# tansey/functionalmf

Measured on AMD Instinct MI355X. Metric: Gibbs sweeps/sec (full W+V update) at (512,256,64) K=5; % HBM roofline, higher is better.
Workload: dtype f64; 1 GPU; gaussian_btf c3 (512,256,64,4) nembeds=5 tf_order=2 complete data, W+V update, rng=device; burn_in_sweeps=10, step_loop=C side (btf_wv_steps: one call queues the K steps), v_sampler=spectral, likelihood_form=complete, parallelism=rows(W)/cols(V) x1

## Files before the change

### functionalmf_amd/_native.py

```python
import ctypes as C
import os
import subprocess
import sys

import numpy as np

HERE = os.path.dirname(os.path.abspath(__file__))
ROOT = os.path.dirname(HERE)
CSRC = os.path.join(HERE, "csrc")
LIB_PATH = os.environ.get("BTF_LIB_PATH") or os.path.join(HERE, "libbtf_hip.so")
SOURCES = [os.path.join(CSRC, "btf_abi.hip"), os.path.join(CSRC, "btf_criteria.hip"), os.path.join(CSRC, "btf_nmf.hip"),
           os.path.join(CSRC, "btf_gass_ep.hip"), os.path.join(CSRC, "btf_gamma_grid.hip"), os.path.join(CSRC, "btf_diag.hip"),
           os.path.join(CSRC, "btf_predict.hip"), os.path.join(CSRC, "btf_functionals.hip"), os.path.join(CSRC, "btf_fold_in.hip"),
           os.path.join(CSRC, "btf_loo.hip")]
HEADERS = sorted(os.path.join(CSRC, f) for f in os.listdir(CSRC) if f.endswith(".h")) + \
    [os.path.join(ROOT, "include", "btf.h")]

BTF_OK, BTF_EINVAL, BTF_EHIP, BTF_ENOTPD, BTF_ESTATE = 0, 1, 2, 3, 4
COMPAT = {"reference": 0, "exact": 1}
KERNEL_NAMES = ["stats", "w_accum", "w_solve", "v_accum", "v_banded", "gram", "products", "sse", "pg_draw", "nb_loglik",
                "prior_band", "gram_eig", "hyper", "ess", "criteria"]
COMM_ID_BYTES = 128
PEER_DESC_BYTES = 256
OPT_SAMPLER, OPT_NB_HISTOGRAMS, OPT_FUSE_GRAM, OPT_PG_EXACT, OPT_CURVE_COUNTS, OPT_SPLIT_ACCUM, OPT_FUSED_SWEEP, OPT_FUSED_STEP, OPT_FUSED_DATAFLOW = 0, 1, 2, 3, 4, 5, 6, 7, 8
# ... 3 lines not shown
SAMPLERS = {"banded": 0, "spectral": 1, "chain": 2, "generic": 3, "banded_nopanel": 4}

_c_dp = C.POINTER(C.c_double)
_c_ip = C.POINTER(C.c_int32)
_ctx = C.c_void_p
SIGNATURES = {
    "btf_create": (C.c_int, [C.POINTER(_ctx), C.c_int, C.c_int, C.c_int, C.c_int, C.c_int, C.c_int, C.c_void_p]),
    "btf_destroy": (None, [_ctx]),
    "btf_last_error": (C.c_char_p, [_ctx]),
    "btf_fail_index": (C.c_int, [_ctx]),
    "btf_set_shard": (C.c_int, [_ctx, C.c_int, C.c_int, C.c_int, C.c_int]),
    "btf_stream": (C.c_void_p, [_ctx]),
    "btf_dev_W": (C.c_void_p, [_ctx]),
    "btf_dev_V": (C.c_void_p, [_ctx]),
    "btf_set_data_gaussian": (C.c_int, [_ctx, _c_dp, _c_dp, C.c_int]),
    "btf_set_data_binomial": (C.c_int, [_ctx, _c_dp, _c_dp, _c_dp, _c_dp]),
    "btf_set_stale_sources": (C.c_int, [_ctx, _c_ip, _c_ip]),
    "btf_set_shard_halo": (C.c_int, [_ctx, C.c_int, C.c_int]),
    "btf_set_W": (C.c_int, [_ctx, _c_dp]),
    "btf_get_W": (C.c_int, [_ctx, _c_dp]),
    "btf_set_V": (C.c_int, [_ctx, _c_dp]),
    "btf_get_V": (C.c_int, [_ctx, _c_dp]),
    "btf_set_hyper": (C.c_int, [_ctx, _c_dp, C.c_double, C.c_double]),
    "btf_set_tau_chain": (C.c_int, [_ctx, _c_dp, _c_dp, _c_dp]),
    "btf_get_tau": (C.c_int, [_ctx, _c_dp, _c_dp, _c_dp, _c_dp]),
    "btf_resample_Tau2": (C.c_int, [_ctx, C.c_uint64, C.c_double, C.c_double, _c_dp]),
    "btf_set_nu2": (C.c_int, [_ctx, C.c_double]),
    "btf_set_omega": (C.c_int, [_ctx, _c_dp, _c_dp]),
    "btf_get_omega": (C.c_int, [_ctx, _c_dp]),
    "btf_w_accum": (C.c_int, [_ctx, C.c_int]),
    "btf_resample_W": (C.c_int, [_ctx, _c_dp, C.c_uint64, C.c_int]),
    "btf_resample_V": (C.c_int, [_ctx, _c_dp, C.c_uint64, C.c_int, C.c_double, C.c_int]),
    "btf_get_V_attempts": (C.c_int, [_ctx, _c_ip]),
    "btf_get_V_order": (C.c_int, [_ctx, _c_ip]),
    "btf_sse": (C.c_int, [_ctx, _c_dp, _c_dp]),
    "btf_sse_begin": (C.c_int, [_ctx]),
    "btf_set_data_counts": (C.c_int, [_ctx, _c_dp, C.c_int]),
    "btf_nb_loglik": (C.c_int, [_ctx, _c_dp, _c_dp, _c_ip, _c_dp]),
    "btf_nb_set_rate": (C.c_int, [_ctx, _c_dp, _c_ip]),
    "btf_nb_mh": (C.c_int, [_ctx, C.c_uint64, C.c_int, C.c_double, C.c_double, _c_ip, _c_dp]),
    "btf_nb_get_rate": (C.c_int, [_ctx, _c_dp, _c_ip]),
    "btf_dev_hyp": (C.c_void_p, [_ctx]),
    "btf_set_global_nobs": (C.c_int, [_ctx, C.c_double]),
    "btf_set_scalar_slot": (C.c_int, [_ctx, C.c_int, C.c_double]),
    "btf_device_scalars": (C.c_int, [_ctx, C.c_int]),
    "btf_set_scalars": (C.c_int, [_ctx, C.c_double, C.c_double, C.c_double, C.c_double]),
    "btf_get_scalars": (C.c_int, [_ctx, _c_dp]),
    "btf_draw_scalars": (C.c_int, [_ctx, C.c_uint64, C.c_int, C.c_double, C.c_double, C.c_double, C.c_double]),
    "btf_draw_lam2": (C.c_int, [_ctx, C.c_uint64, C.c_int]),
    "btf_sse_end": (C.c_int, [_ctx, _c_dp, _c_dp, _c_dp]),
    "btf_pg_draw": (C.c_int, [_ctx, C.c_uint64]),
    "btf_pg_batch": (C.c_int, [C.c_int, C.c_int64, _c_dp, _c_dp, C.c_uint64, _c_dp]),
    "btf_pg_batch_mode": (C.c_int, [C.c_int, C.c_int64, _c_dp, _c_dp, C.c_uint64, C.c_int, _c_dp]),
    "btf_posterior_summary": (C.c_int, [C.c_int, C.c_int, C.c_int, C.c_int, C.c_int, C.c_int, _c_dp, _c_dp, C.c_int, _c_dp,
                                        C.c_int, _c_dp, _c_dp]),
    "btf_posterior_functionals": (C.c_int, [C.c_int] * 6 + [_c_dp, _c_dp, C.c_int, _c_ip, C.c_int, _c_dp, C.c_double, C.c_double, _c_dp,
                                            C.c_int, _c_ip, C.c_int] + [_c_dp] * 7),
    "btf_collect_functionals": (C.c_int, [_ctx, C.c_int, C.c_int, _c_ip, C.c_int, _c_dp, C.c_double, C.c_double, _c_dp, C.c_int, _c_ip,
                                          C.c_int] + [_c_dp] * 7),
    "btf_fold_in_rows": (C.c_int, [C.c_int] * 7 + [_c_dp] * 7 + [C.c_uint64, C.c_int, C.c_int64, _c_dp, _c_dp, C.c_int, _c_dp, C.c_int,
                                   _c_dp, _c_dp]),
    "btf_collect_fold_in": (C.c_int, [_ctx, C.c_int, C.c_int, C.c_int] + [_c_dp] * 4 + [C.c_uint64, C.c_int, C.c_int64, _c_dp, _c_dp,
                                                                                       C.c_int, _c_dp, C.c_int, _c_dp, _c_dp]),
    "btf_diag_eval": (C.c_int, [C.c_int, C.c_int, C.c_int, C.c_int, C.c_int, C.c_int, C.c_int, C.POINTER(_c_dp), C.POINTER(_c_dp),
                                C.POINTER(_ctx), C.c_int, _c_dp]),
    "btf_collect_begin": (C.c_int, [_ctx, C.c_int]),
    "btf_collect": (C.c_int, [_ctx, C.c_int]),
    "btf_collect_schedule": (C.c_int, [_ctx, C.c_int, C.c_int, C.c_int]),
    "btf_collect_end": (C.c_int, [_ctx, C.c_int, _c_dp, _c_dp, _c_dp, _c_dp]),
    "btf_collect_summary": (C.c_int, [_ctx, C.c_int, C.c_int, _c_dp, C.c_int, _c_dp, _c_dp]),
    "btf_crit_set_data": (C.c_int, [_ctx, C.c_int, _c_dp, _c_dp, _c_dp, _c_dp]),
    "btf_crit_eval": (C.c_int, [_ctx, C.c_int, C.c_int, C.c_double, C.c_int, _c_dp, _c_dp, _c_dp, C.c_int, _c_dp, _c_dp, _c_dp]),
    "btf_crit_loo": (C.c_int, [_ctx, C.c_int, C.c_int, C.c_double, C.c_int, _c_dp, _c_dp, _c_dp, C.c_int, _c_dp, C.c_int, _c_dp, _c_dp,
                               _c_dp]),
    "btf_predict_batch": (C.c_int, [C.c_int, C.c_int, C.c_int64, _c_dp, _c_dp, C.c_uint64, _c_dp]),
    "btf_predict_eval": (C.c_int, [_ctx, C.c_int, C.c_double, C.c_int, _c_dp, _c_dp, _c_dp, C.c_int, _c_dp, _c_dp, C.c_int, C.c_int,
                                   C.c_uint64, _c_dp, C.c_int, _c_ip, C.c_int] + [_c_dp] * 11),
    "btf_nmf_create": (C.c_int, [C.POINTER(C.c_void_p), C.c_int, C.c_int, C.c_int, C.c_int, C.c_int, C.c_int, _c_dp,
                                 C.POINTER(C.c_uint8), C.c_double]),
    "btf_nmf_run": (C.c_int, [C.c_void_p, _c_dp, _c_dp, C.c_int, C.c_int, C.c_int, C.c_int, C.c_double, C.c_int, _c_ip, _c_dp,
                              _c_dp]),
    "btf_nmf_destroy": (None, [C.c_void_p]),
    "btf_nmf_pav": (C.c_int, [C.c_int, C.c_int, C.c_int, C.c_int, C.c_int, _c_dp, _c_dp]),
    "btf_sync": (C.c_int, [_ctx]),
    "btf_ess_begin": (C.c_int, [_ctx, C.c_int, _c_dp, C.c_uint64, C.c_double, C.c_int]),
    "btf_ess_eval": (C.c_int, [_ctx, C.c_int, C.c_double, C.c_int, C.c_int, _c_dp]),
    "btf_ess_run": (C.c_int, [_ctx, C.c_int, C.c_int, C.c_int, _c_dp, C.c_uint64, C.c_int, C.c_double, C.c_int]),
    "btf_ess_info": (C.c_int, [_ctx, _c_ip, _c_dp]),
    "btf_mvn_banded": (C.c_int, [C.c_int, C.c_int, C.c_int, C.c_int, _c_dp, _c_dp, _c_dp, C.c_uint64,
                                 C.c_double, C.c_int, _c_dp, _c_ip]),
    "btf_set_profiling": (C.c_int, [_ctx, C.c_int]),
    "btf_kernel_times": (C.c_int, [_ctx, _c_dp, C.POINTER(C.c_int64)]),
    "btf_set_tuning": (C.c_int, [_ctx, C.c_int, C.c_int]),
    "btf_set_option": (C.c_int, [_ctx, C.c_int, C.c_int]),
    "btf_sym_eig": (C.c_int, [C.c_int, C.c_int, C.c_int, _c_dp, _c_dp, _c_dp]),
    "btf_read_probe": (C.c_int, [C.c_int, C.c_size_t, C.c_int, _c_dp]),
    "btf_queue_Tau2": (C.c_int, [_ctx, C.c_uint64, C.c_double]),
    "btf_queue_lam2": (C.c_int, [_ctx, C.c_uint64, C.c_int]),
    "btf_gibbs_sweeps": (C.c_int, [_ctx, C.c_int, C.c_uint64, C.c_uint64, C.c_int, C.c_double, C.c_double, C.c_double,
                                   C.c_double, C.c_double, C.c_double, C.c_int]),
    "btf_wv_steps": (C.c_int, [_ctx, C.c_int, C.c_uint64, C.c_uint64, C.c_int, C.c_double, C.c_int]),
    "btf_gass_set_constraints": (C.c_int, [_ctx, _c_dp, C.c_int, _c_dp, C.c_int]),
    "btf_gass_begin": (C.c_int, [_ctx, C.c_int, C.c_int, _c_dp, _c_dp, C.c_uint64, C.c_double, C.c_int, C.c_int]),
    "btf_gass_grid": (C.c_int, [_ctx, C.c_int, _c_ip, C.POINTER(C.c_uint8), _c_dp, _c_dp]),
    "btf_gass_eval": (C.c_int, [_ctx, C.c_int, _c_dp, _c_ip, _c_dp]),
    "btf_gass_commit": (C.c_int, [_ctx, C.c_int, _c_dp, _c_ip]),
    "btf_gass_select": (C.c_int, [_ctx, C.c_int, C.c_uint64, _c_ip]),
    "btf_gass_run": (C.c_int, [_ctx, C.c_int, C.c_int, C.c_uint64, C.c_int, C.c_double, C.c_int]),
    "btf_gass_set_ep": (C.c_int, [_ctx, _c_dp, _c_dp]),
    "btf_mvn_dense": (C.c_int, [C.c_int, C.c_int, C.c_int, _c_dp, C.c_int, _c_dp, _c_dp, _c_dp, C.c_uint64, C.c_double, C.c_int,
                                _c_dp, _c_ip]),
    "btf_get_likelihood_form": (C.c_int, [_ctx, _c_ip]),
    "btf_get_draw_counters": (C.c_int, [_ctx, C.POINTER(C.c_uint64), C.POINTER(C.c_uint64)]),
    "btf_set_draw_counters": (C.c_int, [_ctx, C.c_uint64, C.c_uint64]),
    "btf_get_accum_bytes_per_cell": (C.c_int, [_ctx, _c_dp]),
    "btf_get_V_sampler": (C.c_int, [_ctx, _c_ip]),
    "btf_queue_scalars": (C.c_int, [_ctx, C.c_uint64, C.c_int, C.c_double, C.c_double, C.c_double, C.c_double, _c_ip]),
    "btf_host_selftest": (C.c_int, []),
    "btf_set_likelihood_param": (C.c_int, [_ctx, C.c_int, C.c_double]),
    "btf_set_likelihood_table": (C.c_int, [_ctx, C.c_int, _c_dp, _c_dp, _c_dp, C.c_int]),
    "btf_set_data_logsum": (C.c_int, [_ctx, _c_dp, _c_dp, C.c_int]),
    "btf_comm_fork": (C.c_int, [_ctx, C.c_void_p]),
    "btf_comm_join": (C.c_int, [_ctx, C.c_void_p]),
    "btf_comm_unique_id": (C.c_int, [C.POINTER(C.c_ubyte), C.c_int]),
    "btf_comm_block": (C.c_int, [C.c_int, C.c_int, C.c_int, _c_ip, _c_ip]),
    "btf_comm_init": (C.c_int, [_ctx, C.c_int, C.c_int, C.POINTER(C.c_ubyte), C.c_int]),
    "btf_comm_rehearse": (C.c_int, [_ctx, C.c_int, C.c_int]),
    "btf_peer_export": (C.c_int, [_ctx, C.POINTER(C.c_ubyte), C.c_int]),
    "btf_peer_init": (C.c_int, [_ctx, C.c_int, C.c_int, C.POINTER(C.c_ubyte), C.c_int]),
    "btf_comm_destroy": (C.c_int, [_ctx]),
    "btf_comm_info": (C.c_int, [_ctx, _c_ip]),
    "btf_allgather_W": (C.c_int, [_ctx]),
    "btf_allgather_V": (C.c_int, [_ctx]),
    "btf_allreduce_sse": (C.c_int, [_ctx]),
    "btf_allreduce_sum": (C.c_int, [_ctx, _c_dp, C.c_int]),
    "btf_set_gathered_W": (C.c_int, [_ctx, _c_dp]),
    "btf_set_gathered_V": (C.c_int, [_ctx, _c_dp]),
}


class BTFError(RuntimeError):
    def __init__(self, code, msg, index=-1):
        super().__init__("btf error %d: %s" % (code, msg))
        self.code = code
        self.index = index


class NotPositiveDefiniteError(BTFError, np.linalg.LinAlgError):
    """Raised where the reference raises LinAlgError (W step, factor.py:357) and
    where it would loop forever after the jitter retries (fast_mvn.py:69-72)."""


INST_SOURCE = os.path.join(CSRC, "btf_instances.hip")
INST_PARTS = 9
OBJ_DIR = os.path.join(ROOT, "build", "obj")


def build(force=False, verbose=False, jobs=None):
    deps = SOURCES + [INST_SOURCE] + HEADERS
    if not force and os.path.exists(LIB_PATH) and \
            os.path.getmtime(LIB_PATH) >= max(os.path.getmtime(p) for p in deps):
        return LIB_PATH
    from concurrent.futures import ThreadPoolExecutor
    os.makedirs(OBJ_DIR, exist_ok=True)
    tag = os.path.splitext(os.path.basename(LIB_PATH))[0]
    base = ["hipcc", "--offload-arch=gfx950", "-O3", "-std=c++17", "-fPIC", "-Wno-unused-function",
            "-mllvm", "-amdgpu-kernarg-preload-count=16",
            "-I", os.path.join(ROOT, "include")] + os.environ.get("BTF_BUILD_DEFS", "").split()
    units = [(SOURCES[0], os.path.join(OBJ_DIR, tag + "_abi.o"), []), (SOURCES[1], os.path.join(OBJ_DIR, tag + "_crit.o"), [])]
    units += [(SOURCES[2], os.path.join(OBJ_DIR, tag + "_nmf.o"), []), (SOURCES[3], os.path.join(OBJ_DIR, tag + "_gass_ep.o"), [])]
    units += [(SOURCES[4], os.path.join(OBJ_DIR, tag + "_gamma_grid.o"), []), (SOURCES[5], os.path.join(OBJ_DIR, tag + "_diag.o"), [])]
    units += [(SOURCES[6], os.path.join(OBJ_DIR, tag + "_predict.o"), []), (SOURCES[7], os.path.join(OBJ_DIR, tag + "_functionals.o"), [])]
    units += [(SOURCES[8], os.path.join(OBJ_DIR, tag + "_fold_in.o"), []), (SOURCES[9], os.path.join(OBJ_DIR, tag + "_loo.o"), [])]
    units += [(INST_SOURCE, os.path.join(OBJ_DIR, "%s_inst%d.o" % (tag, p)), ["-DBTF_INST_PART=%d" % p])
              for p in range(INST_PARTS)]

    def compile_unit(u):
        src, obj, defs = u
        cmd = base + defs + ["-c", src, "-o", obj]
        if verbose:
            print(" ".join(cmd), file=sys.stderr)
        subprocess.run(cmd, check=True, cwd=CSRC)
        return obj

    jobs = jobs or max(1, min(len(units), os.cpu_count() or 1))
    with ThreadPoolExecutor(max_workers=jobs) as pool:
        objs = list(pool.map(compile_unit, units))
    cmd = ["hipcc", "--offload-arch=gfx950", "-fPIC", "-shared", "-o", LIB_PATH] + objs + os.environ.get("BTF_LINK_FLAGS", "").split()
    if verbose:
        print(" ".join(cmd), file=sys.stderr)
    subprocess.run(cmd, check=True, cwd=CSRC)
    return LIB_PATH


_lib = None


def load():
    global _lib
    if _lib is not None:
        return _lib
    if not os.path.exists(LIB_PATH):
        raise ImportError("functionalmf_amd: %s is missing - run `python -c 'import __graft_entry__ as g; g.build()'` "
                          "(there is no CPU fallback)" % LIB_PATH)
    if "torch" not in sys.modules and os.environ.get("BTF_NO_TORCH", "0") != "1":
        try:
            import torch
        except Exception:
            pass
    lib = C.CDLL(LIB_PATH)
    for name, (res, args) in SIGNATURES.items():
        fn = getattr(lib, name)
        fn.restype = res
        fn.argtypes = args
    _lib = lib
    return lib


def check(rc, lib, handle=None, fail_index=True):
    if rc == BTF_OK:
        return
    msg = lib.btf_last_error(handle).decode()
    if rc == BTF_ENOTPD:
        raise NotPositiveDefiniteError(rc, msg, lib.btf_fail_index(handle) if fail_index else -1)
    raise BTFError(rc, msg)


def dptr(a):
    return a.ctypes.data_as(_c_dp) if a is not None else None


def as_f64(a):
    return np.ascontiguousarray(a, dtype=np.float64)


class Context:

    def __init__(self, nrows, ncols, ndepth, nembeds, tf_order, device=0, stream=None):
        self.lib = load()
        self.h = _ctx()
        check(self.lib.btf_create(C.byref(self.h), nrows, ncols, ndepth, nembeds, tf_order, device,
                                  C.c_void_p(stream) if stream else None), self.lib)
        self.dims = (nrows, ncols, ndepth, nembeds, tf_order)
        self.device = device
        self.stream_handle = self.lib.btf_stream(self.h)

    def close(self):
        if getattr(self, "h", None):
            self.lib.btf_destroy(self.h)
            self.h = None

    def __del__(self):
        try:
            self.close()
        except Exception:
            pass

    def check(self, rc):
        check(rc, self.lib, self.h)

    def call(self, name, *args):
        self.check(getattr(self.lib, name)(self.h, *args))

    def kernel_times(self):
        ms = np.zeros(len(KERNEL_NAMES))
        n = np.zeros(len(KERNEL_NAMES), dtype=np.int64)
        self.check(self.lib.btf_kernel_times(self.h, dptr(ms), n.ctypes.data_as(C.POINTER(C.c_int64))))
        return {k: (float(ms[i]), int(n[i])) for i, k in enumerate(KERNEL_NAMES)}
```

### functionalmf_amd/csrc/btf_abi.hip

```cpp
#include "../../include/btf.h"
#include "btf_kernels.h"
#include "btf_banded_fast.h"
#include "btf_banded_twist.h"
#include "btf_banded_chunk.h"
#include "btf_spectral.h"
#include "btf_gass.h"
#include "btf_gass_ep.h"
#include "btf_gamma_grid.h"
#include "btf_fused.h"
#include "btf_diag.h"
#include "btf_criteria.h"
#include "btf_loo.h"
#include "btf_predict.h"
#include "btf_functionals.h"
#include "btf_fold_in.h"
#include "btf_instances.h"
#include "btf_comm.h"
#include "btf_scratch.h"
#include <hip/hip_ext.h>
#include <unistd.h>

#include <algorithm>
#include <atomic>
#include <climits>
// ... 319 lines not shown
  }
  for (int r = 0; r < nD; ++r) {
    int lo = T, hi = -1;
    for (int t = 0; t < T; ++t)
      if (Delta[(size_t)r * T + t] != 0.0) { lo = std::min(lo, t); hi = std::max(hi, t); }
    if (hi - lo > tf + 1) return fail(c, BTF_EINVAL, "penalty row wider than the band");
  }
  int rc;
  if ((rc = dev_alloc(c, &c->st_ptr, ptr.size()))) return rc;
  if ((rc = dev_alloc(c, &c->st_row, row.size()))) return rc;
  if ((rc = dev_alloc(c, &c->st_coef, coef.size()))) return rc;
  HIPCHK(c, hipMemcpy(c->st_ptr, ptr.data(), ptr.size() * sizeof(int), hipMemcpyHostToDevice));
  HIPCHK(c, hipMemcpy(c->st_row, row.data(), row.size() * sizeof(int), hipMemcpyHostToDevice));
  HIPCHK(c, hipMemcpy(c->st_coef, coef.data(), coef.size() * sizeof(double), hipMemcpyHostToDevice));
  {
    const size_t ne = (size_t)T * D1;
    std::vector<int> drow(ne * VS_MAXE, 0);
    std::vector<double> dcoef(ne * VS_MAXE, 0.0);
    c->st_dense_ok = true;
    for (size_t e = 0; e < ne; ++e) {
      const int cnt = ptr[e + 1] - ptr[e];
      if (cnt > VS_MAXE) { c->st_dense_ok = false; break; }
      for (int u = 0; u < cnt; ++u) { drow[e * VS_MAXE + u] = row[ptr[e] + u]; dcoef[e * VS_MAXE + u] = coef[ptr[e] + u]; }
    }
    if ((rc = dev_alloc(c, &c->st_drow, drow.size()))) return rc;
    if ((rc = dev_alloc(c, &c->st_dcoef, dcoef.size()))) return rc;
    HIPCHK(c, hipMemcpy(c->st_drow, drow.data(), drow.size() * sizeof(int), hipMemcpyHostToDevice));
    HIPCHK(c, hipMemcpy(c->st_dcoef, dcoef.data(), dcoef.size() * sizeof(double), hipMemcpyHostToDevice));
  }
  return BTF_OK;
}

inline int unr3_min_rpb() {
  static const int v = [] { const char* e = std::getenv("BTF_UNR3_RPB"); return e ? std::atoi(e) : 2048; }();
  return v;
}
inline bool lean_on() {
  static const bool v = [] { const char* e = std::getenv("BTF_ACC_LEAN"); return !e || std::atoi(e) != 0; }();
  return v;
}
template <int K>
void launch_accum(btf_ctx* c, int kid, int mode, const double* X, const double* Cx, const unsigned char* C8, const double* U,
                  const int* srcmap, int Rdim, int ld, int rpb, int nch, EigSide side = EigSide{nullptr, 0, 0, nullptr},
                  EigSideCols sidec = EigSideCols{nullptr, 0, CurveLists{nullptr, nullptr, nullptr}, nullptr, 0.0, nullptr},
                  TauSide tau = TauSide{}, GramSide gram = GramSide{},
                  ChunkMap cm = ChunkMap{0, 0, INT_MAX, 0, 0, 0}, SweepSide sw = SweepSide{},
                  const FuseW* fw = nullptr, const FuseV* fv = nullptr) {
  if (cm.row_end == 0) cm.row_end = Rdim;
  {
    static const double min_mb = [] { const char* e = std::getenv("BTF_NT_MIN_MB"); return e ? std::atof(e) : 100.0; }();
    cm.nt = (double)Rdim * (double)ld * 8.0 >= min_mb * 1048576.0 ? 1 : 0;
  }
#ifdef BTF_ACC_STAMPS
  cm.stamps = c->acc_stamps;
#endif
  Prof p(c, kid);
  const int cpw = TAU_SIDE_CPW;
  cm.nside = (sw.sc.hyp ? 1 : 0) + (sw.lam.hyp ? 1 : 0) + (side.out ? 1 + eig_side_groups(sidec.ncols, acc_waves(K, mode)) : 0) +
             (tau.Tau2 ? (tau.M + cpw - 1) / cpw : 0) + (gram.gpart ? gram.nblocks : 0) + (gram.sum_src ? 1 : 0) + (fw ? fw->owners : 0);
  dim3 grid((ld / ACC_TILE) * nch + cm.nside);
  if (fw || fv) {
    const bool unr3 = rpb >= unr3_min_rpb();
    if constexpr (K == 8) {
      if (unr3 && fw) { p.launch(accum_kernel<K, 0, 16, double, double, 3, 2, FUSE_W>, grid, dim3(16 * WAVE), 0, X, Cx, U, srcmap, c->part, Rdim, ld, rpb, side, sidec, tau, gram, cm, sw, *fw); return; }
      if (unr3 && fv) { p.launch(accum_kernel<K, 0, 16, double, double, 3, 2, FUSE_V>, grid, dim3(16 * WAVE), 0, X, Cx, U, srcmap, c->part, Rdim, ld, rpb, side, sidec, tau, gram, cm, sw, *fv); return; }
    }
    if constexpr (K <= 8) {
      if (fw) p.launch(accum_kernel<K, 0, 16, double, double, 0, 2, FUSE_W>, grid, dim3(16 * WAVE), 0, X, Cx, U, srcmap, c->part, Rdim, ld, rpb, side, sidec, tau, gram, cm, sw, *fw);
      else {
        const bool df_on = c->fused_dataflow != 0;
        FuseV f2 = *fv;
        constexpr int RG = K < 4 ? 4 : (K > 6 ? 6 : K);
        f2.dataflow = (df_on && f2.a.pband && f2.pimg && !f2.cnt && !f2.hp.flag && K <= 6 &&
                       vf_df_fits(f2.a.T, K, f2.a.TF, f2.a.nD, 16, RG)) ? 1 : 0;

        if constexpr (K <= 6) {
          if (f2.dataflow) { p.launch(accum_kernel<K, 0, 16, double, double, 0, 2, FUSE_VDF>, grid, dim3(16 * WAVE), 0, X, Cx, U, srcmap, c->part, Rdim, ld, rpb, side, sidec, tau, gram, cm, sw, f2); return; }
        }
        p.launch(accum_kernel<K, 0, 16, double, double, 0, 2, FUSE_V>, grid, dim3(16 * WAVE), 0, X, Cx, U, srcmap, c->part, Rdim, ld, rpb, side, sidec, tau, gram, cm, sw, f2);
      }
    }
    return;
  }
  const signed char* A8 = (mode >= 1 && !C8 && X == c->A_wT) ? c->A8_wT : ((mode >= 1 && !C8 && X == c->A_v) ? c->A8_v : nullptr);
  if (A8) {
    if (mode == 2) p.launch(accum_kernel<K, 2, acc_waves(K, 2), double, signed char>, grid, dim3(acc_waves(K, 2) * WAVE), 0, A8, Cx, U, srcmap, c->part, Rdim, ld, rpb, side, sidec, tau, gram, cm, sw, FuseNone{});
    else p.launch(accum_kernel<K, 1, acc_waves(K, 1), double, signed char>, grid, dim3(acc_waves(K, 1) * WAVE), 0, A8, Cx, U, srcmap, c->part, Rdim, ld, rpb, side, sidec, tau, gram, cm, sw, FuseNone{});
    return;
  }
  if (mode >= 1 && C8) {
    if (mode == 2) p.launch(accum_kernel<K, 2, acc_waves(K, 2), unsigned char>, grid, dim3(acc_waves(K, 2) * WAVE), 0, X, C8, U, srcmap, c->part, Rdim, ld, rpb, side, sidec, tau, gram, cm, sw, FuseNone{});
    else p.launch(accum_kernel<K, 1, acc_waves(K, 1), unsigned char>, grid, dim3(acc_waves(K, 1) * WAVE), 0, X, C8, U, srcmap, c->part, Rdim, ld, rpb, side, sidec, tau, gram, cm, sw, FuseNone{});
  } else if (mode == 2) p.launch(accum_kernel<K, 2>, grid, dim3(acc_waves(K, 2) * WAVE), 0, X, Cx, U, srcmap, c->part, Rdim, ld, rpb, side, sidec, tau, gram, cm, sw, FuseNone{});
  else if (mode == 1) p.launch(accum_kernel<K, 1>, grid, dim3(acc_waves(K, 1) * WAVE), 0, X, Cx, U, srcmap, c->part, Rdim, ld, rpb, side, sidec, tau, gram, cm, sw, FuseNone{});
  else if (K <= 8 && acc_waves(K, 0) == 16 && rpb < unr3_min_rpb() && !tau.Tau2 && !sw.sc.hyp && !sw.lam.hyp && lean_on()) {
    if constexpr (K <= 8) p.launch(accum_kernel<K, 0, 16, double, double, 0, 2, FUSE_LEAN>, grid, dim3(16 * WAVE), 0, X, Cx, U, srcmap, c->part, Rdim, ld, rpb, side, sidec, tau, gram, cm, sw, FuseNone{});
  }
  else if (K >= 10 && ACC_WAVES != acc_waves(10, 0) && !side.out && rpb < unr3_min_rpb()) {
    if constexpr (K >= 10) p.launch(accum_kernel<K, 0, ACC_WAVES>, grid, dim3(ACC_WAVES * WAVE), 0, X, Cx, U, srcmap, c->part, Rdim, ld, rpb, side, sidec, tau, gram, cm, sw, FuseNone{});
  }
  else if (rpb >= unr3_min_rpb()) p.launch(accum_kernel<K, 0, acc_waves(K, 0), double, double, 3>, grid, dim3(acc_waves(K, 0) * WAVE), 0, X, Cx, U, srcmap, c->part, Rdim, ld, rpb, side, sidec, tau, gram, cm, sw, FuseNone{});
  else p.launch(accum_kernel<K, 0>, grid, dim3(acc_waves(K, 0) * WAVE), 0, X, Cx, U, srcmap, c->part, Rdim, ld, rpb, side, sidec, tau, gram, cm, sw, FuseNone{});
}
struct PgPasses { bool flat, series, frac; int mode; };
PgPasses pg_passes(const btf_ctx* c) {
  PgPasses p{false, false, false, c->pg_mode};
  if (c->counts && p.mode == PG_MODE_DEFAULT) p.mode = PG_MODE_SERIES_ALL;
  if (p.mode == PG_MODE_SERIES_ALL) { p.series = true; return p; }
  if (p.mode == PG_MODE_EXACT_ALL) { p.flat = c->pg_has_small || c->pg_has_big; p.frac = c->pg_has_frac; }
  else { p.flat = c->pg_has_small; p.series = c->pg_has_big || c->pg_has_frac; }
  if (!p.flat && !p.series && !p.frac) p.series = true;
  return p;
}
template <int K>
void launch_pg(btf_ctx* c, const double* B, double* out, const double* Lf, const double* Uf, int nl, int ld, int Rdim,
               unsigned long long base, unsigned long long stride_r, unsigned long long stride_l, unsigned long long seed) {
  const int gx = (nl + PG_THREADS - 1) / PG_THREADS;
  int nrb = std::max(1, std::min(Rdim, 4096 / std::max(1, gx)));
  const int rpb = (Rdim + nrb - 1) / nrb;
  nrb = (Rdim + rpb - 1) / rpb;
  const PgPasses ps = pg_passes(c);
  int fill = 1;
  if (ps.flat) {
    Prof p(c, BTF_K_PG);
    const int rpx = round_up(rpb, PGX_CPL);
    p.launch(pgx_kernel<K, PGX_CPL>, dim3(gx, (Rdim + rpx - 1) / rpx), dim3(256), pgx_rows_lds(PGX_CPL), B, out, Lf, Uf, nl, ld, Rdim,
             rpx, base, stride_r, stride_l, seed, ps.mode, fill);
    fill = 0;
  }
  if (ps.series) {
    Prof p(c, BTF_K_PG);
    p.launch(pg_kernel<K, PG_PATH_SERIES>, dim3(gx, nrb), dim3(PG_THREADS), 0, B, out, Lf, Uf, nl, ld, Rdim, rpb, base, stride_r, stride_l, seed, ps.mode, fill);
    fill = 0;
  }
  if (ps.frac) {
    Prof p(c, BTF_K_PG);
    p.launch(pg_kernel<K, PG_PATH_EXACT>, dim3(gx, nrb), dim3(PG_THREADS), 0, B, out, Lf, Uf, nl, ld, Rdim, rpb, base, stride_r, stride_l, seed, ps.mode, fill);
  }
}
template <int K>
void launch_gram(btf_ctx* c, const double* U, int Rdim) {
  Prof p(c, BTF_K_GRAM);
  c->ngp_gram = gram_blocks(Rdim);
  p.launch(gram_kernel<K>, dim3(c->ngp_gram), dim3(GRAM_THREADS), 0, U, Rdim, c->gpart);
}
template <int K>
void launch_wsolve(btf_ctx* c, const WSolveArgs& a0) {
  Prof p(c, BTF_K_W_SOLVE);
  WSolveArgs a = a0;
  const int rw = ws_rows_for(a.nl);
  a.nside = (a.lam.hyp ? 1 : 0) + (a.band.pband ? a.band.ml : 0);
  const dim3 grid((a.nl + rw - 1) / rw + a.nside);
#define WS_LAUNCH(WT, RWV) p.launch(w_solve_kernel<K, WT, RWV>, grid, dim3(WS_ROWS * ws_split_of(K, WT)), 0, a)
#define WS_PICK(WT) do { if (rw == 8) WS_LAUNCH(WT, 8); else if (rw == 16) WS_LAUNCH(WT, 16); else if (rw == 32) WS_LAUNCH(WT, 32); else WS_LAUNCH(WT, 64); } while (0)
  if (a.weighted) WS_PICK(true); else WS_PICK(false);
#undef WS_PICK
#undef WS_LAUNCH
}
template <int K>
hipError_t launch_vbanded(btf_ctx* c, const VBandArgs& a, size_t lds_bytes) {
  static std::atomic<unsigned long long> attr_set{0};
  if (!dev_flag_is_set(attr_set, c->dev)) {
    hipError_t e = hipFuncSetAttribute((const void*)v_banded_kernel<K>, hipFuncAttributeMaxDynamicSharedMemorySize, 160 * 1024);
    if (e != hipSuccess) return e;
    dev_flag_set(attr_set, c->dev);
  }
  Prof p(c, BTF_K_V_BANDED);
  p.launch(v_banded_kernel<K>, dim3(a.ml), dim3(WAVE), lds_bytes, a);
  return hipSuccess;
}
template <int NPL, bool ROW16>
hipError_t launch_vbanded_fast(btf_ctx* c, const VBandArgs& a, size_t lds_bytes) {
  static std::atomic<unsigned long long> attr_set{0};
  if (!dev_flag_is_set(attr_set, c->dev)) {
    hipError_t e = hipFuncSetAttribute((const void*)v_banded_fast_kernel<NPL, ROW16>,
                                       hipFuncAttributeMaxDynamicSharedMemorySize, 160 * 1024);
    if (e != hipSuccess) return e;
    dev_flag_set(attr_set, c->dev);
  }
  Prof p(c, BTF_K_V_BANDED);
  p.launch(v_banded_fast_kernel<NPL, ROW16>, dim3(a.ml), dim3(VB_THREADS), lds_bytes, a, c->K);
  return hipSuccess;
}
hipError_t dispatch_vbanded_fast(btf_ctx* c, const VBandArgs& a, int bw, size_t lds_bytes, bool* handled) {
  const int npairs = bw * (bw - 1) / 2;
  const int npl = std::max(1, (npairs + WAVE - 1) / WAVE);
  *handled = true;
  if (bw <= 15) {
    if (npl == 1) return launch_vbanded_fast<1, true>(c, a, lds_bytes);
    if (npl == 2) return launch_vbanded_fast<2, true>(c, a, lds_bytes);
  } else {
    switch (npl) {
      case 2: return launch_vbanded_fast<2, false>(c, a, lds_bytes);
      case 3: return launch_vbanded_fast<3, false>(c, a, lds_bytes);
      case 4: return launch_vbanded_fast<4, false>(c, a, lds_bytes);
      case 5: return launch_vbanded_fast<5, false>(c, a, lds_bytes);
      case 6: return launch_vbanded_fast<6, false>(c, a, lds_bytes);
      case 7: return launch_vbanded_fast<7, false>(c, a, lds_bytes);
      case 8: return launch_vbanded_fast<8, false>(c, a, lds_bytes);
      default: break;
    }
  }
  *handled = false;
  return hipSuccess;
}
template <int NPL>
hipError_t launch_vbanded_chunk(btf_ctx* c, const VBandArgs& a, size_t lds_bytes, int CH) {
  static std::atomic<unsigned long long> attr_set{0};
  if (!dev_flag_is_set(attr_set, c->dev)) {
    hipError_t e = hipFuncSetAttribute((const void*)v_banded_chunk_kernel<NPL>, hipFuncAttributeMaxDynamicSharedMemorySize, 160 * 1024);
    if (e != hipSuccess) return e;
    dev_flag_set(attr_set, c->dev);
  }
  Prof p(c, BTF_K_V_BANDED);
  p.launch(v_banded_chunk_kernel<NPL>, dim3(a.ml), dim3(VB_THREADS), lds_bytes, a, c->K, CH);
  return hipSuccess;
}
constexpr size_t VC_LDS_BUDGET = 158 * 1024;
inline int vc_npl(int bw) { return std::max(1, ((bw - 1) * (bw - 2) / 2 + WAVE - 1) / WAVE); }
inline int vc_chunk_for(const btf_ctx* c, bool wt) {
  const int bw = (c->TF + 1) * c->K;
  if (bw < 3 || vc_npl(bw) > 8) return 0;
  return vc_pick_chunk(c->T, c->K, c->TF, wt ? 1 : 0, VC_LDS_BUDGET);
}
hipError_t dispatch_vbanded_chunk(btf_ctx* c, const VBandArgs& a, int bw, int CH, bool wt, bool* handled) {
  const size_t lds_bytes = vc_lds_bytes(c->T, c->K, c->TF, wt ? 1 : 0, CH);
  *handled = true;
  switch (vc_npl(bw)) {
    case 1: return launch_vbanded_chunk<1>(c, a, lds_bytes, CH);
    case 2: return launch_vbanded_chunk<2>(c, a, lds_bytes, CH);
    case 3: return launch_vbanded_chunk<3>(c, a, lds_bytes, CH);
    case 4: return launch_vbanded_chunk<4>(c, a, lds_bytes, CH);
    case 5: return launch_vbanded_chunk<5>(c, a, lds_bytes, CH);
    case 6: return launch_vbanded_chunk<6>(c, a, lds_bytes, CH);
    case 7: return launch_vbanded_chunk<7>(c, a, lds_bytes, CH);
    case 8: return launch_vbanded_chunk<8>(c, a, lds_bytes, CH);
    default: break;
  }
  *handled = false;
  return hipSuccess;
}
template <int NPL, bool ROW16, int KC = 0, int TFC = 0, int TC = 0>
hipError_t launch_vbanded_twist(btf_ctx* c, const VBandArgs& a, size_t lds_bytes) {
  static std::atomic<unsigned long long> attr_set{0};
  if (!dev_flag_is_set(attr_set, c->dev)) {
    hipError_t e = hipFuncSetAttribute((const void*)v_banded_twist_kernel<NPL, ROW16, KC, TFC, TC>,
                                       hipFuncAttributeMaxDynamicSharedMemorySize, 160 * 1024);
    if (e != hipSuccess) return e;
    dev_flag_set(attr_set, c->dev);
  }
  Prof p(c, BTF_K_V_BANDED);
  p.launch(v_banded_twist_kernel<NPL, ROW16, KC, TFC, TC>, dim3(a.ml), dim3(VT_THREADS), lds_bytes, a, c->K);
  return hipSuccess;
}
void fill_table_host(int T, int K, int TF, int wmode, std::vector<int>& tab) {
  const int KK = tri(K), D1 = TF + 2, n = T * K;
  const bool weighted = wmode != 0;
  const TwLayout W = tw_layout(T, K, TF, wmode);
  auto qsrc = [&](int t, int q) { return wmode == 2 ? -2 - (q * T + t) : W.Ql + (weighted ? t * KK : 0) + q; };
  const int R1 = W.L.R1, nl = W.nl, nr = W.nr, nL = W.nL;
  tab.clear();
  auto put = [&](int dst, int src, int dia) { tab.push_back(dst); tab.push_back(src); tab.push_back(dia); tab.push_back(0); };
  for (int i = 0; i < nL; ++i) {
    const int t = i / K, k = i - t * K;
    for (int aa = 0; aa < K - k; ++aa)
      if (i + aa < nL) put(W.L.band + i * R1 + aa, qsrc(t, lidx(k + aa, k)), aa == 0 ? W.P + t * D1 : -1);
    for (int d = 1; d < D1; ++d)
      if (t + d < T && i + d * K < nL) put(W.L.band + i * R1 + d * K, W.P + t * D1 + d, -1);
  }
  for (int m = 0; m < nr; ++m) {
    const int gc = n - 1 - m, tc = gc / K, kc = gc - tc * K;
    for (int aa = 0; aa <= kc; ++aa)
      if (gc - aa >= nl) put(W.R.band + m * R1 + aa, qsrc(tc, lidx(kc, kc - aa)), aa == 0 ? W.P + tc * D1 : -1);
    for (int d = 1; d < D1; ++d)
      if (gc - d * K >= nl) put(W.R.band + m * R1 + d * K, W.P + (tc - d) * D1 + d, -1);
  }
  while ((tab.size() / 4) % VT_THREADS) put(W.L.dummy + 1, W.P, -1);
}
inline int twist_wmode(const btf_ctx* c, bool wt) {
  if (tw_lds_bytes(c->T, c->K, c->TF, wt ? 1 : 0) <= 160 * 1024) return wt ? 1 : 0;
  if (wt && tw_lds_bytes(c->T, c->K, c->TF, 2) <= 160 * 1024) return 2;
  return -1;
}
int make_fill_table(btf_ctx* c, bool weighted) {
  const int key = twist_wmode(c, weighted);
  if (c->fill_tab && c->fill_key == key) return BTF_OK;
  std::vector<int> tab;
  fill_table_host(c->T, c->K, c->TF, key, tab);
  std::vector<int> packed(tab.size() / 2);
  for (size_t e = 0; e + 3 < tab.size(); e += 4) {
    const int dst = tab[e], src = tab[e + 1], dia = tab[e + 2];
    if (dst < 0 || dst >= 0xffff || dia >= 0xffff) return fail(c, BTF_EINVAL, "band assembly program: LDS offset beyond 16 bits");
    packed[e / 2] = (int)((unsigned)dst | ((unsigned)(dia < 0 ? 0xffff : dia) << 16));
    packed[e / 2 + 1] = src;
  }
  int rc;
  if ((rc = dev_alloc(c, &c->fill_tab, packed.size()))) return rc;
  HIPCHK(c, hipMemcpy(c->fill_tab, packed.data(), packed.size() * sizeof(int), hipMemcpyHostToDevice));
  c->fill_n = (int)(tab.size() / 4);
  c->fill_key = key;
  return BTF_OK;
}
hipError_t dispatch_vbanded_twist(btf_ctx* c, const VBandArgs& a, int bw, size_t lds_bytes, bool* handled) {
  const int npairs = (bw - 1) * (bw - 2) / 2;
  const int npl = std::max(1, (npairs + WAVE - 1) / WAVE);
  *handled = true;
  if (c->TF == 2 && c->T == 64 && (c->K == 5 || c->K == 8)) {
    if (c->K == 5) return launch_vbanded_twist<tw_npl(5, 2), tw_row16(5, 2), 5, 2, 64>(c, a, lds_bytes);
    return launch_vbanded_twist<tw_npl(8, 2), tw_row16(8, 2), 8, 2, 64>(c, a, lds_bytes);
  }
// ... 136 lines not shown
  if (st[0] != 0) {
    c->fail_index = st[1];
    int zero[2] = {0, -1};
    HIPCHK(c, hipMemcpy(c->status, zero, sizeof(zero), hipMemcpyHostToDevice));
    if (st[0] == 2) return fail(c, BTF_EHIP, "a hand-off inside a fused launch timed out (btf_fused.h): its producer workgroup never published");
    if (st[0] == 3) return fail(c, BTF_EHIP, "the peer-window exchange timed out waiting for rank " + std::to_string(st[1]) + " (btf_comm.h; BTF_PEER_TIMEOUT_MS)");
    return fail(c, BTF_ENOTPD, "conditional precision not positive definite at index " + std::to_string(st[1]));
  }
  return BTF_OK;
}

int ensure_part(btf_ctx* c, size_t elems) {
  if (elems > c->part_elems) {
    int rc = dev_alloc(c, &c->part, elems);
    if (rc) return rc;
    c->part_elems = elems;
  }
  return BTF_OK;
}

int ensure_z(btf_ctx* c, size_t elems) {
  if (elems > c->z_elems) {
    int rc = dev_alloc(c, &c->zbuf, elems);
    if (rc) return rc;
    c->z_elems = elems;
  }
  return BTF_OK;
}

int pick_rpb(int Rdim, int tiles, int user, bool weighted, int slots = 0, int reserve = 0) {
  if (user > 0) return std::max(64, round_up(user, 64));
  const long long want_wgs = tiles >= 32 ? 512 : 256;
  long long rpb = ((long long)Rdim * tiles + want_wgs - 1) / want_wgs;
  rpb = std::max<long long>(rpb, weighted ? 256 : 512);
  rpb = std::min<long long>(rpb, std::max(Rdim, 1));
  rpb = std::max(128, round_up((int)rpb, 64));
  static const bool fit = [] { const char* e = std::getenv("BTF_FIT_ROUND"); return !e || std::atoi(e) != 0; }();
  if (fit && slots > 0) {
    const long long nch = (Rdim + rpb - 1) / rpb, total = nch * tiles + reserve;
    const long long rounds = (total + slots - 1) / slots;
    const long long nch1 = (slots - reserve) / std::max(tiles, 1);
    if (rounds >= 2 && rounds <= 3 && nch1 >= 1) {
      const long long r1 = round_up((int)((Rdim + nch1 - 1) / nch1), 64);
      if (r1 < rounds * rpb) rpb = r1;
    }
  }
  return (int)rpb;
}
inline int slab_rows(const btf_ctx* c) { return c->nl + (c->hrow >= 0 ? 1 : 0); }
inline int slab_cols(const btf_ctx* c) { return c->ml + (c->hcol >= 0 ? 1 : 0); }
inline int acc_slots(const btf_ctx* c, int K, int mode, bool w_launch = false) {
  const int waves = (w_launch && mode == 0 && K >= 10) ? ACC_WAVES : acc_waves(K, mode);
  return c->ncu * std::max(1, 16 / waves);
}
inline int w_side_reserve(const btf_ctx* c, bool wt) {
  const bool whole = c->nl == c->N && c->ml == c->M;
  const bool gram_side = !wt && !(whole && c->fuse_gram && c->ngp_v > 0) && !c->weighted;
  return (gram_side ? 32 : 0) + (c->tau_pending && c->dev_scalars && c->have_chain ? (c->ml + TAU_SIDE_CPW - 1) / TAU_SIDE_CPW : 0) +
         (c->sc_pending ? 1 : 0);
}
inline int v_side_reserve(const btf_ctx* c, bool wt) {
  const bool spectral = banded_choice(c) == 3;
  return (spectral ? 1 + (c->weighted && !wt ? (c->cv_ndef + 3) / 4 : 0) : 0) + (c->lam_pending ? 1 : 0);
}

struct Uploaded { const double* h = nullptr; const double* h2 = nullptr; double* d = nullptr; double* d2 = nullptr; };
int make_stats(btf_ctx* c, const double* hY, const double* hY2, int rows, int cols, int R, bool transposed,
               double** A, double** C, double** B, int ld, size_t out_rows, bool want_sums, Uploaded* keep, bool last, int sum_rows = -1) {
  const size_t cells = (size_t)rows * cols;
  double* dY = nullptr; double* dY2 = nullptr;
  int rc;
  const bool reuse = keep && keep->d && keep->h == hY && keep->h2 == hY2;
  if (reuse) { dY = keep->d; dY2 = keep->d2; }
  else {
    if ((rc = dev_alloc(c, &dY, cells * R))) return rc;
    HIPCHK(c, hipMemcpy(dY, hY, cells * R * sizeof(double), hipMemcpyHostToDevice));
    if (hY2) {
      if ((rc = dev_alloc(c, &dY2, cells))) return rc;
      HIPCHK(c, hipMemcpy(dY2, hY2, cells * sizeof(double), hipMemcpyHostToDevice));
    }
  }
  const size_t out_elems = out_rows * (size_t)ld;
  if ((rc = dev_alloc(c, A, out_elems))) return rc;
  HIPCHK(c, hipMemsetAsync(*A, 0, out_elems * sizeof(double), c->stream));
  if ((rc = dev_alloc(c, C, out_elems))) return rc;
  HIPCHK(c, hipMemsetAsync(*C, 0, out_elems * sizeof(double), c->stream));
  int* dflag = c->status + 2;
  const int blocks = (int)std::min<size_t>(4096, (cells + 255) / 256);
  if (want_sums) {
    if ((size_t)blocks * 3 > c->bsum_elems) {
      if ((rc = dev_alloc(c, &c->bsum, (size_t)blocks * 3))) return rc;
      c->bsum_elems = (size_t)blocks * 3;
    }
  }
  StatsArgs a{dY, dY2, rows, cols, R, ld, transposed ? 1 : 0, *A, *C, want_sums ? c->bsum : nullptr, dflag, sum_rows < 0 ? rows : sum_rows};
  {
    Prof p(c, BTF_K_STATS);
    p.launch(stats_kernel, dim3(blocks), dim3(256), 0, a);
  }
  HIPCHK(c, hipGetLastError());
  if (B && hY2) {
    if ((rc = dev_alloc(c, B, out_elems))) return rc;
    HIPCHK(c, hipMemcpyAsync(*B, *C, out_elems * sizeof(double), hipMemcpyDeviceToDevice, c->stream));
  }
  HIPCHK(c, hipStreamSynchronize(c->stream));
  if (want_sums) {
    std::vector<double> h((size_t)blocks * 3);
    HIPCHK(c, hipMemcpy(h.data(), c->bsum, h.size() * sizeof(double), hipMemcpyDeviceToHost));
    double ssw = 0.0, nobs = 0.0, sa2 = 0.0;
    for (int b = 0; b < blocks; ++b) { ssw += h[3 * b]; nobs += h[3 * b + 1]; sa2 += h[3 * b + 2]; }
    c->ssw = ssw;
    c->nobs = nobs;
    c->sa2 = sa2;
  }
  if (keep && !last) { keep->h = hY; keep->h2 = hY2; keep->d = dY; keep->d2 = dY2; }
  else {
    (void)hipFree(dY);
    if (dY2) (void)hipFree(dY2);
    if (keep) *keep = Uploaded{};
  }
  return BTF_OK;
}

int upload_relayout(btf_ctx* c, const double* h, int rows, int cols, double* dst, int ld, bool transposed) {
  const size_t cells = (size_t)rows * cols;
  double* d = nullptr;
  int rc;
  if ((rc = dev_alloc(c, &d, cells))) return rc;
  HIPCHK(c, hipMemcpy(d, h, cells * sizeof(double), hipMemcpyHostToDevice));
  const int blocks = (int)std::min<size_t>(4096, (cells + 255) / 256);
  hipLaunchKernelGGL(relayout_kernel, dim3(blocks), dim3(256), 0, c->stream, d, rows, cols, dst, ld, transposed ? 1 : 0, 1);
  HIPCHK(c, hipStreamSynchronize(c->stream));
  (void)hipFree(d);
  return BTF_OK;
}

}

extern "C" {

int btf_create(btf_ctx** out, int nrows, int ncols, int ndepth, int nembeds, int tf_order, int device, void* stream) {
  if (!out) return BTF_EINVAL;
  *out = nullptr;
  if (nrows < 1 || ncols < 1 || ndepth < 2 || nembeds < 1 || nembeds > MAX_K || tf_order < 0 || tf_order > 3)
    return fail(nullptr, BTF_EINVAL, "unsupported dims (need 1<=nembeds<=10, 0<=tf_order<=3, ndepth>=2)");
  if ((tf_order + 1) * nembeds > 63) return fail(nullptr, BTF_EINVAL, "half-bandwidth (tf_order+1)*nembeds must be <= 63");
  btf_ctx* c = new btf_ctx();
  c->N = nrows; c->M = ncols; c->T = ndepth; c->K = nembeds; c->TF = tf_order; c->KK = tri(nembeds);
  c->dev = device;
  c->row0 = 0; c->nl = nrows; c->col0 = 0; c->ml = ncols;
  hipError_t e = hipSetDevice(device);
  if (e != hipSuccess) { g_err = std::string("hipSetDevice: ") + hipGetErrorString(e); delete c; return BTF_EHIP; }
  { int n = 0; if (hipDeviceGetAttribute(&n, hipDeviceAttributeMultiprocessorCount, device) == hipSuccess && n > 0) c->ncu = n; }
  { const char* e = std::getenv("BTF_FUSED_STEP"); if (e) c->fused_step = std::max(0, std::min(2, std::atoi(e))); }
  { const char* e = std::getenv("BTF_LAM_IN_WSOLVE"); if (e) c->lam_in_wsolve = std::atoi(e) != 0; }
  { const char* e = std::getenv("BTF_BAND_IN_WSOLVE"); if (e) c->band_in_wsolve = std::atoi(e) != 0; }
  { const char* e = std::getenv("BTF_VF_DATAFLOW"); if (e) c->fused_dataflow = std::atoi(e) != 0 ? 1 : 0; }
  if (stream) { c->stream = (hipStream_t)stream; }
  else {
    e = hipStreamCreateWithFlags(&c->stream, hipStreamNonBlocking);
    if (e != hipSuccess) { g_err = std::string("hipStreamCreate: ") + hipGetErrorString(e); delete c; return BTF_EHIP; }
    c->own_stream = true;
  }
  int rc = BTF_OK;
  auto A = [&](int r) { if (rc == BTF_OK) rc = r; };
  A(dev_alloc(c, &c->W, (size_t)(nrows + 64) * nembeds));
  A(dev_alloc(c, &c->V, (size_t)(ncols + 64) * ndepth * nembeds));
  A(dev_alloc(c, &c->gpart, (size_t)GRAM_BLOCKS * c->KK));
  A(dev_alloc(c, &c->status, 4));
  if (rc == BTF_OK) {
    int init[4] = {0, -1, 0, 0};
    if (hipMemcpy(c->status, init, sizeof(init), hipMemcpyHostToDevice) != hipSuccess) rc = BTF_EHIP;
  }
  if (rc == BTF_OK) rc = build_stencil(c);
  A(dev_alloc(c, &c->Tau2, (size_t)ncols * c->nD));
  A(dev_alloc(c, &c->tries, (size_t)ncols));
  if (rc != BTF_OK) { std::string m = c->err; btf_destroy(c); g_err = m; return rc; }
  *out = c;
  return BTF_OK;
}

void btf_destroy(btf_ctx* c) {
  if (!c) return;
  (void)hipSetDevice(c->dev);
  if (c->stream) (void)hipStreamSynchronize(c->stream);
  void* ptrs[] = {c->A_wT, c->C_wT, c->A_v, c->C_v, c->B_wT, c->B_v, c->W, c->V, c->Tau2, c->part,
                  c->gpart, c->zbuf, c->bsum, c->gband, c->status, c->tries, c->st_ptr, c->st_row, c->st_coef,
                  c->srcmap_w, c->srcmap_v, c->pband, c->pimg, c->dbg, c->gpart_w, c->gpart_v, c->gsum_v, c->eig, c->cv_cptr, c->cv_crow, c->cv_cdef, c->cv_rptr, c->cv_rcol, c->cv_rdef, c->eig_cols, c->cv_dcols, c->A8_wT, c->A8_v, c->gs_cons, c->gs_cc, c->gs_rc, c->gs_av, c->gs_mask, c->gs_info, c->gs_thetas, c->gs_ntheta, c->gs_ll, c->gs_llp, c->gs_hh, c->gs_cur, c->gs_nacc, c->gs_u, c->st_drow, c->st_dcoef, c->essX0, c->essNu, c->ess_st, c->ess_theta, c->ess_done, c->ess_part, c->Ta, c->Tb, c->Tc, c->lsum, c->dr_ptr, c->dr_col, c->dr_val, c->sse_cols, c->vs_rec, c->vc_scratch, c->gs_cptr, c->gs_cidx, c->gs_cval,
                  c->ep_rows, c->ep_cols, c->ep_crow, c->ep_ccol, c->ep_mu, c->ep_corr, c->ep_pband, c->ep_envg, c->ep_f, c->ep_off,
                  c->gg_tab, c->gg_Lw, c->gg_Lv};
  for (void* p : ptrs) if (p) (void)hipFree(p);
  if (c->pin) (void)hipHostFree(c->pin);
  if (c->pin_lsum) (void)hipHostFree(c->pin_lsum);
  if (c->pin_hyp) (void)hipHostFree(c->pin_hyp);
  for (void* p : {(void*)c->nb_data, (void*)c->nb_S, (void*)c->nb_cnt, (void*)c->nb_R, (void*)c->nb_C, (void*)c->nb_tmp, (void*)c->nb_out, (void*)c->nb_H, (void*)c->nb_Hd, (void*)c->nb_Hs, (void*)c->nb_G, (void*)c->nb_L, (void*)c->nb_optr, (void*)c->nb_oval, (void*)c->fill_tab, (void*)c->C8_wT, (void*)c->C8_v, (void*)c->smp_W, (void*)c->smp_V, (void*)c->smp_T, (void*)c->smp_s})
    if (p) (void)hipFree(p);
  for (int sl = 0; sl < 2; ++sl)
    for (void* p : {(void*)c->crit_S1[sl], (void*)c->crit_cnt[sl], (void*)c->crit_c0[sl], (void*)c->crit_c1[sl]})
      if (p) (void)hipFree(p);
  if (c->hyp) (void)hipFree(c->hyp);
  if (c->fz_words) (void)hipFree(c->fz_words);
  if (c->fz_pub) (void)hipFree(c->fz_pub);
  for (auto& e : c->ev_pool) { (void)hipEventDestroy(e.a); (void)hipEventDestroy(e.b); }
  if (c->ev_draw) (void)hipEventDestroy(c->ev_draw);
  if (c->ev_join) (void)hipEventDestroy(c->ev_join);
  (void)btf_comm_destroy(c);

  if (c->own_stream && c->stream) (void)hipStreamDestroy(c->stream);
  delete c;
}

const char* btf_last_error(const btf_ctx* c) { return c ? c->err.c_str() : g_err.c_str(); }
int fold_fail_index();
int btf_fail_index(const btf_ctx* c) { return c ? c->fail_index : fold_fail_index(); }

int btf_set_shard(btf_ctx* c, int row0, int nrows_local, int col0, int ncols_local) {
  if (!c) return BTF_EINVAL;
  if (c->have_data) return fail(c, BTF_ESTATE, "btf_set_shard must precede btf_set_data_*");
  if (row0 < 0 || nrows_local < 0 || row0 + nrows_local > c->N || col0 < 0 || ncols_local < 0 || col0 + ncols_local > c->M)
    return fail(c, BTF_EINVAL, "shard out of range");
  c->row0 = row0; c->nl = nrows_local; c->col0 = col0; c->ml = ncols_local;
  c->hrow = c->hcol = -1;
  ++c->prior_version;
  if (c->pband) { (void)hipFree(c->pband); c->pband = nullptr; c->pband_version = 0; }
  if (c->pimg) { (void)hipFree(c->pimg); c->pimg = nullptr; c->pimg_version = 0; }
  c->v_wants_band = false;
  c->nb_bwt_written = false;
  return BTF_OK;
}
int btf_set_shard_halo(btf_ctx* c, int halo_row, int halo_col) {
  if (!c) return BTF_EINVAL;
  if (halo_row < -1 || halo_row >= c->N || halo_col < -1 || halo_col >= c->M) return fail(c, BTF_EINVAL, "halo source out of range");
  if ((halo_row >= c->row0 && halo_row < c->row0 + c->nl) || (halo_col >= c->col0 && halo_col < c->col0 + c->ml))
    return fail(c, BTF_EINVAL, "halo source inside the shard's own block");
  if (halo_row != c->hrow || halo_col != c->hcol) {
    c->have_data = false;
    c->nb_bwt_written = false;
  }
  c->hrow = halo_row; c->hcol = halo_col;
  return BTF_OK;
}
void* btf_stream(btf_ctx* c) { return c ? (void*)c->stream : nullptr; }
void* btf_dev_W(btf_ctx* c) { return c ? c->W : nullptr; }
void* btf_dev_V(btf_ctx* c) { return c ? c->V : nullptr; }

static int detect_curve_counts(btf_ctx* c) {
  c->curve = false;
  c->cv_cij.clear();
  if (!c->C8_v || c->nl != c->N || c->ml != c->M) return BTF_OK;
  const int N = c->N, M = c->M, T = c->T;
  std::vector<unsigned char> h((size_t)N * c->ldv);
  HIPCHK(c, hipMemcpy(h.data(), c->C8_v, h.size(), hipMemcpyDeviceToHost));
  std::vector<unsigned char> cij((size_t)N * M);
  for (int i = 0; i < N; ++i)
    for (int j = 0; j < M; ++j) {
      const unsigned char* p = h.data() + (size_t)i * c->ldv + (size_t)j * T;
      const unsigned char v = p[0];
      for (int t = 1; t < T; ++t) if (p[t] != v) return BTF_OK;
      cij[(size_t)i * M + j] = v;
    }
  std::vector<int> cptr(M + 1, 0), rptr(N + 1, 0);
  size_t nnz = 0;
  for (int i = 0; i < N; ++i)
    for (int j = 0; j < M; ++j) if (cij[(size_t)i * M + j] < c->R) { ++cptr[j + 1]; ++rptr[i + 1]; ++nnz; }
  if (nnz == 0 || nnz > (size_t)N * M / 4) return BTF_OK;
  for (int j = 0; j < M; ++j) cptr[j + 1] += cptr[j];
  for (int i = 0; i < N; ++i) rptr[i + 1] += rptr[i];
  std::vector<int> crow(nnz), rcol(nnz), cfill(cptr.begin(), cptr.end() - 1), rfill(rptr.begin(), rptr.end() - 1);
  std::vector<double> cdef(nnz), rdef(nnz);
  for (int i = 0; i < N; ++i)
    for (int j = 0; j < M; ++j) {
      const int v = cij[(size_t)i * M + j];
      if (v >= c->R) continue;
      const double d = (double)(c->R - v);
      crow[cfill[j]] = i; cdef[cfill[j]++] = d;
      rcol[rfill[i]] = j; rdef[rfill[i]++] = d;
    }
  int rc;
  if ((rc = dev_alloc(c, &c->cv_cptr, cptr.size()))) return rc;
  if ((rc = dev_alloc(c, &c->cv_crow, nnz))) return rc;
  if ((rc = dev_alloc(c, &c->cv_cdef, nnz))) return rc;
  if ((rc = dev_alloc(c, &c->cv_rptr, rptr.size()))) return rc;
  if ((rc = dev_alloc(c, &c->cv_rcol, nnz))) return rc;
  if ((rc = dev_alloc(c, &c->cv_rdef, nnz))) return rc;
  HIPCHK(c, hipMemcpy(c->cv_cptr, cptr.data(), cptr.size() * sizeof(int), hipMemcpyHostToDevice));
  HIPCHK(c, hipMemcpy(c->cv_crow, crow.data(), nnz * sizeof(int), hipMemcpyHostToDevice));
  HIPCHK(c, hipMemcpy(c->cv_cdef, cdef.data(), nnz * sizeof(double), hipMemcpyHostToDevice));
  HIPCHK(c, hipMemcpy(c->cv_rptr, rptr.data(), rptr.size() * sizeof(int), hipMemcpyHostToDevice));
  HIPCHK(c, hipMemcpy(c->cv_rcol, rcol.data(), nnz * sizeof(int), hipMemcpyHostToDevice));
  HIPCHK(c, hipMemcpy(c->cv_rdef, rdef.data(), nnz * sizeof(double), hipMemcpyHostToDevice));
  std::vector<int> dcols;
  for (int j = 0; j < M; ++j) if (cptr[j + 1] > cptr[j]) dcols.push_back(j);
  if ((rc = dev_alloc(c, &c->cv_dcols, dcols.size()))) return rc;
  HIPCHK(c, hipMemcpy(c->cv_dcols, dcols.data(), dcols.size() * sizeof(int), hipMemcpyHostToDevice));
  c->cv_ndef = (int)dcols.size();
  const size_t ne = (size_t)M * (c->K + c->K * c->K + 8);
  if ((rc = dev_alloc(c, &c->eig_cols, ne))) return rc;
  HIPCHK(c, hipMemset(c->eig_cols, 0, ne * sizeof(double)));
  c->cv_cij.swap(cij);
  c->curve = true;
  return BTF_OK;
}

static int finish_data(btf_ctx* c) {
  int flag = 0;
  HIPCHK(c, hipMemcpy(&flag, c->status + 2, sizeof(int), hipMemcpyDeviceToHost));
  c->weighted = c->binomial || flag != 0;
// ... 192 lines not shown
  if (!c) return BTF_EINVAL;
  HIPCHK(c, hipSetDevice(c->dev));
  if (Tau2) {
    HIPCHK(c, hipMemcpyAsync(c->Tau2, Tau2, (size_t)c->M * c->nD * sizeof(double), hipMemcpyHostToDevice, c->stream));
    HIPCHK(c, hipStreamSynchronize(c->stream));
    c->have_hyper = true;
  }
  if (Tau2 || lam2 != c->lam2) ++c->prior_version;
  c->lam2 = lam2; c->sigma2 = sigma2;
  return BTF_OK;
}
int btf_set_tau_chain(btf_ctx* c, const double* Ta, const double* Tb, const double* Tc) {
  if (!c || !Ta || !Tb || !Tc) return BTF_EINVAL;
  HIPCHK(c, hipSetDevice(c->dev));
  const size_t n = (size_t)c->M * c->nD;
  int rc;
  if (!c->Ta) {
    if ((rc = dev_alloc(c, &c->Ta, n))) return rc;
    if ((rc = dev_alloc(c, &c->Tb, n))) return rc;
    if ((rc = dev_alloc(c, &c->Tc, n))) return rc;
    if ((rc = dev_alloc(c, &c->lsum, (size_t)c->M))) return rc;
  }
  HIPCHK(c, hipMemcpyAsync(c->Ta, Ta, n * sizeof(double), hipMemcpyHostToDevice, c->stream));
  HIPCHK(c, hipMemcpyAsync(c->Tb, Tb, n * sizeof(double), hipMemcpyHostToDevice, c->stream));
  HIPCHK(c, hipMemcpyAsync(c->Tc, Tc, n * sizeof(double), hipMemcpyHostToDevice, c->stream));
  HIPCHK(c, hipStreamSynchronize(c->stream));
  c->have_chain = true;
  return BTF_OK;
}

int btf_get_tau(btf_ctx* c, double* Tau2, double* Ta, double* Tb, double* Tc) {
  if (!c || !Tau2) return BTF_EINVAL;
  HIPCHK(c, hipSetDevice(c->dev));
  const size_t n = (size_t)c->M * c->nD * sizeof(double);
  HIPCHK(c, hipMemcpyAsync(Tau2, c->Tau2, n, hipMemcpyDeviceToHost, c->stream));
  if (Ta && c->Ta) {
    HIPCHK(c, hipMemcpyAsync(Ta, c->Ta, n, hipMemcpyDeviceToHost, c->stream));
    HIPCHK(c, hipMemcpyAsync(Tb, c->Tb, n, hipMemcpyDeviceToHost, c->stream));
    HIPCHK(c, hipMemcpyAsync(Tc, c->Tc, n, hipMemcpyDeviceToHost, c->stream));
  }
  HIPCHK(c, hipStreamSynchronize(c->stream));
  return BTF_OK;
}

static TauSide tau_side_of(btf_ctx* c, uint64_t seed, double lam2, double stability) {
  TauSide t{};
  ++c->prior_version;
  t.V = c->V; t.T = c->T; t.nD = c->nD; t.M = c->M;
  t.dr_ptr = c->dr_ptr; t.dr_col = c->dr_col; t.dr_val = c->dr_val;
  t.lam2 = lam2; t.lo = stability; t.hi = 1.0 / stability;
  t.Tau2 = c->Tau2; t.Ta = c->Ta; t.Tb = c->Tb; t.Tc = c->Tc; t.lsum = c->lsum;
  t.seed = (unsigned long long)seed; t.hyp = c->dev_scalars ? c->hyp : nullptr;
  return t;
}

int btf_queue_Tau2(btf_ctx* c, uint64_t seed, double stability) {
  if (!c || !(stability > 0.0)) return fail(c, BTF_EINVAL, "bad Tau2 update arguments");
  if (!c->dev_scalars) return fail(c, BTF_ESTATE, "btf_queue_Tau2 needs device-resident scalars");
  if (!c->have_V || !c->have_hyper || !c->have_chain) return fail(c, BTF_ESTATE, "set V, Tau2 and the horseshoe+ chain first");
  c->tau_pending = true; c->tau_seed = seed; c->tau_stability = stability;
  return BTF_OK;
}

int btf_resample_Tau2(btf_ctx* c, uint64_t seed, double lam2, double stability, double* lsum_out) {
  if (!c || !(stability > 0.0)) return fail(c, BTF_EINVAL, "bad Tau2 update arguments");
  if (c->dev_scalars) lam2 = 1.0;
  if (!(lam2 > 0.0)) return fail(c, BTF_EINVAL, "bad Tau2 update arguments");
  if (!c->have_V || !c->have_hyper || !c->have_chain) return fail(c, BTF_ESTATE, "set V, Tau2 and the horseshoe+ chain first");
  HIPCHK(c, hipSetDevice(c->dev));
  c->tau_pending = false;
  {
    Prof p(c, BTF_K_HYPER);
    p.launch(tau2_kernel, dim3(c->M), dim3(256), 0, tau_side_of(c, seed, lam2, stability), c->K);
  }
  HIPCHK(c, hipGetLastError());
  if (lsum_out) {
    if (!c->pin_lsum) HIPCHK(c, hipHostMalloc((void**)&c->pin_lsum, (size_t)c->M * sizeof(double), hipHostMallocDefault));
    HIPCHK(c, hipMemcpyAsync(c->pin_lsum, c->lsum, (size_t)c->M * sizeof(double), hipMemcpyDeviceToHost, c->stream));
    HIPCHK(c, hipStreamSynchronize(c->stream));
    std::memcpy(lsum_out, c->pin_lsum, (size_t)c->M * sizeof(double));
  }
  return BTF_OK;
}

int btf_set_nu2(btf_ctx* c, double nu2) {
  if (!c || !(nu2 > 0.0)) return fail(c, BTF_EINVAL, "nu2 must be positive");
  c->nu2 = nu2;
  return BTF_OK;
}
int btf_set_omega(btf_ctx* c, const double* omega_rows, const double* omega_cols) {
  if (c) { c->w_part_valid = false; c->w_local_done = c->v_local_done = false; c->sse_cols_valid = false; }
  if (!c || !omega_rows || !omega_cols) return BTF_EINVAL;
  if (!c->have_data || !c->binomial) return fail(c, BTF_ESTATE, "btf_set_omega needs binomial data");
  HIPCHK(c, hipSetDevice(c->dev));
  int rc;
  const int MT = c->M * c->T;
  HIPCHK(c, hipMemsetAsync(c->C_wT, 0, (size_t)MT * c->ldw * sizeof(double), c->stream));
  HIPCHK(c, hipMemsetAsync(c->C_v, 0, (size_t)c->N * c->ldv * sizeof(double), c->stream));
  if ((rc = upload_relayout(c, omega_rows, slab_rows(c), MT, c->C_wT, c->ldw, true))) return rc;
  if ((rc = upload_relayout(c, omega_cols, c->N, slab_cols(c) * c->T, c->C_v, c->ldv, false))) return rc;
  hipLaunchKernelGGL(mask_kernel, dim3(1024), dim3(256), 0, c->stream, c->C_wT, c->B_wT, (size_t)MT * c->ldw);
  hipLaunchKernelGGL(mask_kernel, dim3(1024), dim3(256), 0, c->stream, c->C_v, c->B_v, (size_t)c->N * c->ldv);
  HIPCHK(c, hipStreamSynchronize(c->stream));
  return BTF_OK;
}
int btf_get_omega(btf_ctx* c, double* omega_rows) {
  if (!c || !omega_rows) return BTF_EINVAL;
  if (!c->have_data || !c->C_wT) return fail(c, BTF_ESTATE, "no weights on this context");
  HIPCHK(c, hipSetDevice(c->dev));
  const int MT = c->M * c->T;
  std::vector<double> h((size_t)MT * c->ldw);
  HIPCHK(c, hipMemcpyAsync(h.data(), c->C_wT, h.size() * sizeof(double), hipMemcpyDeviceToHost, c->stream));
  HIPCHK(c, hipStreamSynchronize(c->stream));
  for (int i = 0; i < c->nl; ++i)
    for (int jt = 0; jt < MT; ++jt) omega_rows[(size_t)i * MT + jt] = h[(size_t)jt * c->ldw + i];
  return BTF_OK;
}

namespace {
struct SplitGeom { bool ok; int lo, hi, rpb_l, nch_l, nch_r; };
SplitGeom split_geom(int lo, int hi, int Rdim, int rpb, int tiles) {
  SplitGeom g{false, lo, hi, 0, 0, 0};
  if (hi <= lo || hi - lo >= Rdim || rpb <= 0 || lo % rpb != 0) return g;
  g.ok = true;
  g.nch_r = (Rdim - (hi - lo) + rpb - 1) / rpb;
  long long rl = ((long long)(hi - lo) * tiles + 255) / 256;
  g.rpb_l = std::min(rpb, std::max(64, round_up((int)rl, 64)));
  g.nch_l = (hi - lo + g.rpb_l - 1) / g.rpb_l;
  return g;
}
bool split_applies(const btf_ctx* c) {
  return c->split_accum && !c->binomial && !c->counts && !(c->nl == c->N && c->ml == c->M) && c->nl > 0 && c->ml > 0;
}
enum { ACC_ALL = 2, ACC_LOCAL = 0 };

enum { FZ_EIG = 0, FZ_SC = 32, FZ_LAM = 64, FZ_GRAM = 96, FZ_GSUM = 128, FZ_TICKETS = 160 };
constexpr int FZ_PUB_EIG = 0, FZ_PUB_HYP = 128, FZ_PUB_GSUM = 136, FZ_PUB_GRAN = 200, FZ_PUB_DOUBLES = 224;
int ensure_fused(btf_ctx* c) {
  const int tw = c->ldw / ACC_TILE, tv = c->ldv / ACC_TILE;
  if (c->fz_words && c->fz_tiles_w == tw && c->fz_tiles_v == tv) return BTF_OK;
  int rc;
  const size_t nwords = (size_t)((FZ_TICKETS + tw + tv + 31) / 32) * 32;
  if ((rc = dev_alloc(c, &c->fz_words, nwords))) return rc;
  HIPCHK(c, hipMemsetAsync(c->fz_words, 0, nwords * sizeof(unsigned), c->stream));
  if (!c->fz_pub) {
    if ((rc = dev_alloc(c, &c->fz_pub, (size_t)FZ_PUB_DOUBLES))) return rc;
    HIPCHK(c, hipMemsetAsync(c->fz_pub, 0, (size_t)FZ_PUB_DOUBLES * sizeof(double), c->stream));
  }
  c->fz_tiles_w = tw; c->fz_tiles_v = tv;
  c->fz_gram_total = 0; c->fz_w_total = 0;
  return BTF_OK;
}
bool fuse_w_applies(const btf_ctx* c, bool wt, bool cv, int mode, int rpb) {
  if (c->fused_step < 2 || wt || cv || mode != 0 || c->nl <= 0 || c->K > 8) return false;
  if (split_applies(c)) return false;
  if (rpb >= unr3_min_rpb() && c->K != 8) return false;
  return true;
}
struct WFuseReq { const double* dz; uint64_t seed; bool done; };
int w_accum_phase(btf_ctx* c, int compat, int part = ACC_ALL, WFuseReq* wf = nullptr) {
  const int K = c->K, KK = c->KK, MT = c->M * c->T;
  const bool wt = lik_weighted(c), cv = c->weighted && !wt;
  const int mode = !wt ? 0 : (compat == BTF_COMPAT_REFERENCE && c->stale_w && c->srcmap_w ? 2 : 1);
  const int NV = wt ? K + KK : K;
  const int tiles = c->ldw / ACC_TILE;
  const int rpb = pick_rpb(MT, tiles, c->rpb_w, wt, acc_slots(c, K, mode, true), w_side_reserve(c, wt));
  const int nch = (MT + rpb - 1) / rpb;
  int rc;
  if ((rc = ensure_part(c, (size_t)round_up(nch, 32) * NV * c->ldw))) return rc;
  const SplitGeom sg = split_applies(c) ? split_geom(c->col0 * c->T, (c->col0 + c->ml) * c->T, MT, rpb, tiles) : SplitGeom{};
  if (sg.ok) { if ((rc = ensure_part(c, (size_t)(sg.nch_r + sg.nch_l) * NV * c->ldw))) return rc; }
  if (part == ACC_LOCAL) {
    c->w_local_done = false;
    if (!sg.ok || mode == 2) return BTF_OK;
    K_SWITCH(K, launch_accum<KT>(c, BTF_K_W_ACCUM, mode, c->A_wT, c->C_wT, c->C8_wT, c->V, c->srcmap_w, MT, c->ldw, sg.rpb_l, sg.nch_l,
                                 EigSide{nullptr, 0, 0, nullptr}, EigSideCols{nullptr, 0, CurveLists{nullptr, nullptr, nullptr}, nullptr, 0.0, nullptr},
                                 TauSide{}, GramSide{}, ChunkMap{sg.nch_r, sg.lo, INT_MAX, 0, sg.hi, 0}));
    HIPCHK(c, hipGetLastError());
    c->w_local_done = true; c->w_local_rpb = rpb; c->w_local_mode = mode;
    return BTF_OK;
  }
  const bool rest_only = c->w_local_done && sg.ok && c->w_local_rpb == rpb && c->w_local_mode == mode;
  c->w_local_done = false;
  const ChunkMap cm = rest_only ? ChunkMap{0, 0, sg.lo, sg.hi - sg.lo, MT, 0} : ChunkMap{0, 0, INT_MAX, 0, MT, 0};
  const int nch_launch = rest_only ? sg.nch_r : nch;
  const int nch_total = rest_only ? sg.nch_r + sg.nch_l : nch;
  const bool whole = c->nl == c->N && c->ml == c->M;
  bool use_gv = !wt && whole && c->fuse_gram && c->ngp_v > 0;
  if (cv && c->nl > 0) {
    if (c->ngp_v != c->ml) {
      if (!c->gpart_v) { if ((rc = dev_alloc(c, &c->gpart_v, (size_t)c->M * KK))) return rc; }
      Prof p(c, BTF_K_GRAM);
      K_SWITCH(K, p.launch(colgram_kernel<KT>, dim3(c->ml), dim3(WAVE), 0, (const double*)c->V, c->T, c->ml, c->gpart_v));
      c->ngp_v = c->ml;
    }
    use_gv = true;
  }
  if (c->nl > 0) {
    GramSide gram{nullptr, 0, nullptr, 0};
    if (!wt && !use_gv) {
      c->ngp_gram = std::min(gram_blocks(MT), 32);
      gram = GramSide{c->V, MT, c->gpart, c->ngp_gram, nullptr, nullptr, 0, nullptr, 0};
    }
    bool gsum = false;
    c->w_part_gsum = false;
    if (!wt && use_gv && part == ACC_ALL && c->ngp_v > 8 * std::min(32, (WS_ROWS * ws_split_of(K, false)) / KK)) {
      if (!c->gsum_v) { if ((rc = dev_alloc(c, &c->gsum_v, (size_t)tri(MAX_K)))) return rc; }
      gram.sum_src = c->gpart_v; gram.sum_n = c->ngp_v; gram.sum_out = c->gsum_v; gram.sum_threads = WS_ROWS * ws_split_of(K, false);
      gsum = true;
    }
    c->w_part_gsum = gsum;
    TauSide tau{};
    if (c->tau_pending && c->dev_scalars && c->have_chain) tau = tau_side_of(c, c->tau_seed, 1.0, c->tau_stability);
    SweepSide sw{};
    if (c->sc_pending) {
      const int h = std::min(c->K, c->N);
      const double nfree = (double)c->N * c->K - (double)h * (h - 1) / 2.0 - (double)(c->K - h) * c->N;
      sw.sc = ScalarSide{c->sse_cols, c->M, c->ssw + c->sa2, c->nobs_global >= 0.0 ? c->nobs_global : c->nobs, c->W, c->N * c->K, nfree,
                         c->sc_prior[0], c->sc_prior[1], c->sc_prior[2], c->sc_prior[3], c->sc_which, c->sc_seed, c->hyp};
      c->sc_pending = false;
    }
    FuseW fw{};
    int own_rows = 0;
    if (wf && !rest_only && fuse_w_applies(c, wt, cv, mode, rpb)) {
      const long long others = (long long)tiles * nch + (tau.Tau2 ? (tau.M + TAU_SIDE_CPW - 1) / TAU_SIDE_CPW : 0) + (gram.gpart ? gram.nblocks : 0) + (sw.sc.hyp ? 1 : 0);
      static const int min_rows = [] { const char* e = std::getenv("BTF_OWNER_ROWS"); return e ? std::atoi(e) : 32; }();
      for (int r = std::max(ws_rows_for(c->nl), min_rows); r <= ACC_TILE; r *= 2) {
        if (others + (long long)tiles * (ACC_TILE / r) <= (long long)c->ncu && w_owner_lds_doubles(K, r, nch) <= w_owner_lds_budget(K)) { own_rows = r; break; }
      }
    }
    const bool fuse = own_rows > 0;
    if (fuse) {
      if ((rc = ensure_fused(c))) return rc;
      ++c->fz_epoch;
      WSolveArgs& a = fw.a;
      a.part = c->part; a.nch = nch_total; a.ld = c->ldw; a.weighted = 0;
      a.gpart = use_gv ? c->gpart_v : c->gpart; a.ngp = use_gv ? c->ngp_v : c->ngp_gram;
      if (whole && c->fuse_gram) {
        if (!c->gpart_w) { if ((rc = dev_alloc(c, &c->gpart_w, (size_t)std::max(64, (c->N + WS_ROWS - 1) / WS_ROWS) * KK))) return rc; }
        a.gout = c->gpart_w;
      }
      a.s = c->binomial ? 1.0 : 1.0 / c->nu2;
      a.sR = a.s * c->R;
      a.inv_sigma2 = 1.0 / c->sigma2;
      a.hyp = c->dev_scalars ? c->hyp : nullptr; a.Rrep = c->R; a.hyp_noise = c->binomial ? 0 : 1;
      a.W = c->W; a.row0 = c->row0; a.nl = c->nl;
#ifdef BTF_WS_STAMPS
      a.dbg = c->dbg;
#endif
      a.z = wf->dz; a.seed = wf->seed; a.stream = 2 * c->sweep_w + 0x10000ULL;
      a.status = c->status;
      fw.cnt = c->fz_words + FZ_TICKETS;
      fw.rw = ws_rows_for(c->nl);
      if (sw.sc.hyp) {
        sw.sc.pub = c->fz_pub + FZ_PUB_HYP; sw.sc.flag = c->fz_words + FZ_SC; sw.sc.epoch = c->fz_epoch;
        fw.hp = HypPub{c->fz_pub + FZ_PUB_HYP, c->fz_words + FZ_SC, c->fz_epoch, sw.sc.which & 3};
      }
      if (gram.gpart) {
        gram.cnt = c->fz_words + FZ_GRAM;
        c->fz_gram_total += (unsigned)gram.nblocks;
        fw.gram_cnt = gram.cnt; fw.gram_expected = c->fz_gram_total;
      }
      c->fz_w_total += (unsigned)nch_total;
      fw.expected = c->fz_w_total;
      fw.rows = own_rows;
      fw.owners = tiles * (ACC_TILE / own_rows);
    }
    K_SWITCH(K, launch_accum<KT>(c, BTF_K_W_ACCUM, mode, c->A_wT, c->C_wT, c->C8_wT, c->V, c->srcmap_w, MT, c->ldw, rpb, nch_launch,
                                 EigSide{nullptr, 0, 0, nullptr}, EigSideCols{nullptr, 0, CurveLists{nullptr, nullptr, nullptr}, nullptr, 0.0, nullptr}, tau, gram, cm, sw,
                                 fuse ? &fw : nullptr));
    if (fuse) {
      wf->done = true;
      const int wrows = ws_rows_for(c->nl);
      c->ngp_w = fw.a.gout ? (c->nl + wrows - 1) / wrows : 0;
      c->ngp_v = 0;
    }
    c->tau_pending = false;
  } else if (c->tau_pending && c->dev_scalars && c->have_chain) {
    Prof p(c, BTF_K_HYPER);
    p.launch(tau2_kernel, dim3(c->M), dim3(256), 0, tau_side_of(c, c->tau_seed, 1.0, c->tau_stability), c->K);
    c->tau_pending = false;
  }
  HIPCHK(c, hipGetLastError());
  c->w_part_valid = true; c->w_part_mode = mode; c->w_part_nch = nch_total; c->w_part_rpb = rpb; c->w_part_gv = use_gv;
  c->w_part_curve = cv;
  return BTF_OK;
}
}

namespace {
int v_accum_local(btf_ctx* c, int compat);
int mark_draw(btf_ctx* c);
}

int btf_w_accum(btf_ctx* c, int compat) {
  if (!c) return BTF_EINVAL;
  if (!c->have_data || !c->have_V || !c->have_W) return fail(c, BTF_ESTATE, "set data, W and V first");
  HIPCHK(c, hipSetDevice(c->dev));
  return w_accum_phase(c, compat);
}

int btf_resample_W(btf_ctx* c, const double* z, uint64_t seed, int compat) {
  if (!c) return BTF_EINVAL;
  if (!c->have_data || !c->have_V || !c->have_W) return fail(c, BTF_ESTATE, "set data, W and V first");
  HIPCHK(c, hipSetDevice(c->dev));
  const int K = c->K, KK = c->KK;
  const bool wt = lik_weighted(c), cv = c->weighted && !wt;
  const int want_mode = !wt ? 0 : (compat == BTF_COMPAT_REFERENCE && c->stale_w && c->srcmap_w ? 2 : 1);
  int rc;
  c->v_local_done = false;
  const double* dz = nullptr;
  if (z) {
    const size_t nz = (size_t)w_z_offset(c->N, K);
    if ((rc = ensure_z(c, nz))) return rc;
    HIPCHK(c, hipMemcpyAsync(c->zbuf, z, nz * sizeof(double), hipMemcpyHostToDevice, c->stream));
    dz = c->zbuf;
  }
  WFuseReq wf{dz, seed, false};
  if (!(c->w_part_valid && c->w_part_mode == want_mode && c->w_part_curve == cv)) { if ((rc = w_accum_phase(c, compat, ACC_ALL, &wf))) return rc; }
  if (c->sc_pending) return fail(c, BTF_ESTATE, "btf_queue_scalars must be followed by the W accumulation that carries it");
  const int nch = c->w_part_nch;
  const bool use_gv = c->w_part_gv;
  c->w_part_valid = false;
  if (c->nl > 0 && !wf.done) {
    const bool whole = c->nl == c->N && c->ml == c->M;
    WSolveArgs a{};
    a.part = c->part; a.nch = nch; a.ld = c->ldw; a.weighted = wt ? 1 : 0;
    a.gsrc = (wt && want_mode == 2) ? c->srcmap_w : nullptr;
    a.gpart = use_gv ? c->gpart_v : c->gpart; a.ngp = use_gv ? c->ngp_v : c->ngp_gram;
    if (use_gv && c->w_part_gsum) { a.gpart = c->gsum_v; a.ngp = 1; }
    const int wrows = ws_rows_for(c->nl);
    const int wblocks = (c->nl + wrows - 1) / wrows;
    if (whole && c->fuse_gram) {
      if (!c->gpart_w) { if ((rc = dev_alloc(c, &c->gpart_w, (size_t)std::max(64, (c->N + WS_ROWS - 1) / WS_ROWS) * KK))) return rc; }
      a.gout = c->gpart_w;
    }
    a.s = c->binomial ? 1.0 : 1.0 / c->nu2;
    a.sR = a.s * c->R;
    a.inv_sigma2 = 1.0 / c->sigma2;
    a.hyp = c->dev_scalars ? c->hyp : nullptr; a.Rrep = c->R; a.hyp_noise = c->binomial ? 0 : 1;
    a.W = c->W; a.row0 = c->row0; a.nl = c->nl;
#ifdef BTF_WS_STAMPS
    a.dbg = c->dbg;
#endif
    a.z = dz; a.seed = seed; a.stream = 2 * c->sweep_w + 0x10000ULL;
    a.status = c->status;
    if (cv) { a.cv = CurveLists{c->cv_rptr, c->cv_rcol, c->cv_rdef}; a.cv_blocks = c->gpart_v; }
    if (c->lam_in_wsolve && c->lam_pending && c->dev_scalars && c->lsum && c->have_chain) {
      a.lam = LamSide{c->lsum, c->M, (double)c->nD * c->M * c->K + 1.0, c->lam_exact, c->lam_seed, c->hyp, nullptr, nullptr, 0u};
      c->lam_pending = false;
      ++c->prior_version;
      const int TD1 = c->T * (c->TF + 2);
      if (c->band_in_wsolve && c->v_wants_band && c->pband && (!c->band_img || c->pimg) && TD1 <= 2 * WS_ROWS * ws_split_of(K, wt) &&
          c->nD <= 2 * WS_ROWS * ws_split_of(K, wt)) {
        if ((rc = ensure_fused(c))) return rc;
        ++c->fz_epoch;
        a.lam.pub = c->fz_pub + FZ_PUB_HYP; a.lam.flag = c->fz_words + FZ_LAM; a.lam.epoch = c->fz_epoch;
        a.band = BandSide{c->Tau2, c->nD, c->st_ptr, c->st_row, c->st_coef, TD1, c->col0, c->ml, c->pband,
                          c->band_img ? c->pimg : nullptr, c->T, c->TF + 2, c->band_PB, nullptr, 0.0,
                          c->fz_pub + FZ_PUB_HYP, c->fz_words + FZ_LAM, c->fz_epoch, c->status};
        c->pband_version = c->prior_version;
        c->pimg_version = c->band_img ? c->prior_version : 0;
      }
    }
    K_SWITCH(K, launch_wsolve<KT>(c, a));
    c->ngp_w = a.gout ? wblocks : 0;
    c->ngp_v = 0;
  }
  c->sweep_w++;
  c->nb_L_valid = false;
  c->sse_cols_valid = false;
  HIPCHK(c, hipGetLastError());
  if (split_applies(c)) {
    if ((rc = mark_draw(c))) return rc;
    return v_accum_local(c, compat);
  }
  return BTF_OK;
}

static int v_banded_dispatch(btf_ctx* c, int choice, const double* dz, uint64_t seed, int nch, bool use_gw, double eps0,
                             int attempts, double* out, bool prior_only) {
  const int K = c->K, KK = c->KK, T = c->T, n = T * K;
  const bool wt = lik_weighted(c), cv = c->weighted && !wt && !prior_only;
  const bool whole = c->nl == c->N && c->ml == c->M;
  int rc;
  const int bw = (c->TF + 1) * K, R1 = bw + 1, D1 = c->TF + 2;
  size_t lds_fixed = (size_t)(3 * n + T * D1 + (wt ? T * KK : KK) + (bw * (bw + 1) / 2 + 3) / 4) * sizeof(double);
  size_t lds_band = std::max((size_t)n * R1, (size_t)(GRAM_BLOCKS + 16) * KK) * sizeof(double);
  size_t lds_bytes = lds_fixed + lds_band;
  VBandArgs a{};
  if (lds_bytes > 150 * 1024) {
    if (wt) lds_fixed -= (size_t)T * KK * sizeof(double);
    if (lds_fixed > 150 * 1024) return fail(c, BTF_EINVAL, "ndepth*nembeds too large for the on-chip vectors");
    const size_t stride = (size_t)n * R1 + (wt ? (size_t)T * KK : 0);
    if (!c->gband || c->gband_stride != stride) {
      if ((rc = dev_alloc(c, &c->gband, (size_t)c->ml * stride))) return rc;
      c->gband_stride = stride;
    }
    a.gband = c->gband; a.gband_stride = c->gband_stride;
    lds_bytes = lds_fixed;
  }
  a.part = c->part; a.nch = nch; a.ld = c->ldv; a.weighted = wt ? 1 : 0;
  a.gsrc = (wt && c->v_part_mode == 2) ? c->srcmap_v : nullptr;
  a.gpart = use_gw ? c->gpart_w : c->gpart; a.ngp = use_gw ? c->ngp_w : c->ngp_gram;
  a.s = c->binomial ? 1.0 : 1.0 / c->nu2;
  a.sR = a.s * c->R;
  a.Tau2 = c->Tau2; a.lam2 = c->lam2; a.nD = c->nD;
  a.hyp = c->dev_scalars ? c->hyp : nullptr; a.Rrep = c->R; a.hyp_noise = c->binomial ? 0 : 1;
  a.panel4 = c->sampler == BTF_SAMPLER_BANDED_NOPANEL ? 0 : 1;
  a.st_ptr = c->st_ptr; a.st_row = c->st_row; a.st_coef = c->st_coef;
  a.T = T; a.TF = c->TF; a.col0 = c->col0; a.ml = c->ml;
  a.V = c->V; a.z = dz; a.seed = seed; a.stream = 2 * c->sweep_v + 0x10001ULL;
  a.eps0 = eps0; a.attempts = attempts; a.status = c->status; a.tries = c->tries; a.dbg = c->dbg;
  if (prior_only) { a.nch = 0; a.ngp = 0; a.s = 0.0; a.sR = 0.0; a.hyp_noise = 0; }
  if (cv) { a.cv = CurveLists{c->cv_cptr, c->cv_crow, c->cv_cdef}; a.cv_W = c->W; }
  a.V = out;
  hipError_t e = hipSuccess;
  bool handled = false;
  const bool fast = choice >= 0;
  const int tw_npl = std::max(1, ((bw - 1) * (bw - 2) / 2 + WAVE - 1) / WAVE);
  const bool tw_handles = bw <= 15 ? tw_npl <= 2 : (tw_npl >= 2 && tw_npl <= 8);
  const bool own_prior = choice == 2 && tw_handles && c->st_dense_ok && c->st_drow && (c->TF + 2) * T >= c->nD;
  if (own_prior) {
    a.st_drow = c->st_drow; a.st_dcoef = c->st_dcoef; a.pband = nullptr;
    const int TD1 = T * D1;
    static const bool lazy_band = [] { const char* e = std::getenv("BTF_TWIST_PBAND"); return !e || std::atoi(e) != 0; }();
    if (!lazy_band) {  }
    else if (c->pband && c->pband_version == c->prior_version) a.pband = c->pband;
    else if (c->last_v_prior_version == c->prior_version) {
      if (!c->pband) { if ((rc = dev_alloc(c, &c->pband, (size_t)c->ml * TD1))) return rc; }
      Prof p(c, BTF_K_PRIOR);
      p.launch(prior_band_kernel, dim3((c->ml * TD1 + 255) / 256), dim3(256), 0, (const double*)c->Tau2, c->lam2, c->nD,
               (const int*)c->st_ptr, (const int*)c->st_row, (const double*)c->st_coef, TD1, c->col0, c->ml, c->pband,
               (const double*)(c->dev_scalars ? c->hyp : nullptr), 1, (double*)nullptr, 0, 0, 0);
      c->pband_version = c->prior_version;
      a.pband = c->pband;
    }
    c->last_v_prior_version = c->prior_version;
  }
  if (fast && !own_prior) {
    const int TD1 = T * D1;
    if (!c->pband) { if ((rc = dev_alloc(c, &c->pband, (size_t)c->ml * TD1))) return rc; }
    {
      Prof p(c, BTF_K_PRIOR);
      p.launch(prior_band_kernel, dim3((c->ml * TD1 + 255) / 256), dim3(256), 0, (const double*)c->Tau2, c->lam2, c->nD,
               (const int*)c->st_ptr, (const int*)c->st_row, (const double*)c->st_coef, TD1, c->col0, c->ml, c->pband,
               (const double*)(c->dev_scalars ? c->hyp : nullptr), 0, (double*)nullptr, 0, 0, 0);
    }
    c->pband_version = 0;
    a.pband = c->pband;
  }
  const bool emit_gv = !prior_only && fast && whole && c->fuse_gram && !wt &&
                       (size_t)c->ml * KK + 16 * KK <= ws_gram_stage(K, false);
  if (emit_gv) {
    if (!c->gpart_v) { if ((rc = dev_alloc(c, &c->gpart_v, (size_t)c->M * KK))) return rc; }
    a.gout = c->gpart_v;
  }
  if (!prior_only) { c->ngp_v = emit_gv ? c->ml : 0; c->ngp_w = 0; }
  if (choice == 2) {
    if ((rc = make_fill_table(c, wt))) return rc;
    a.fill = c->fill_tab; a.nfill = c->fill_n;
    a.ql_global = twist_wmode(c, wt) == 2 ? 1 : 0;
    e = dispatch_vbanded_twist(c, a, bw, tw_lds_bytes(T, K, c->TF, twist_wmode(c, wt)), &handled);
  }
  HIPCHK(c, e);
  if (fast && !handled && vb_fast_lds_bytes(T, K, c->TF, wt ? 1 : 0) <= 158 * 1024)
    e = dispatch_vbanded_fast(c, a, bw, vb_fast_lds_bytes(T, K, c->TF, wt ? 1 : 0), &handled);
  HIPCHK(c, e);
  if (fast && !handled) {
    const int CH = vc_chunk_for(c, wt);
    if (CH > 0) {
      const size_t stride = vc_scratch_stride(T, K, c->TF);
      if (!c->vc_scratch || c->vc_scratch_elems < (size_t)c->ml * stride) {
        if ((rc = dev_alloc(c, &c->vc_scratch, (size_t)c->ml * stride))) return rc;
        c->vc_scratch_elems = (size_t)c->ml * stride;
      }
      VBandArgs ac = a;
      ac.gband = c->vc_scratch; ac.gband_stride = stride;
      e = dispatch_vbanded_chunk(c, ac, bw, CH, wt, &handled);
      HIPCHK(c, e);
    }
  }
  if (!handled) { a.gout = nullptr; if (!prior_only) c->ngp_v = 0; }
  if (!handled) { K_SWITCH(K, e = launch_vbanded<KT>(c, a, lds_bytes)); }
  HIPCHK(c, e);
  return BTF_OK;
}
// ... 2237 lines not shown

int btf_mvn_banded(int device, int batch, int n, int bw, const double* band, const double* mu_part, const double* z,
                   uint64_t seed, double eps0, int attempts, double* x_out, int32_t* tries_out) {
  if (batch < 1 || n < 1 || bw < 0 || bw > 63 || !band || !x_out) return fail(nullptr, BTF_EINVAL, "bad mvn arguments");
  hipError_t e = hipSetDevice(device);
  if (e != hipSuccess) return fail(nullptr, BTF_EHIP, std::string("hipSetDevice: ") + hipGetErrorString(e));
  const int R1 = bw + 1;
  const size_t nb = (size_t)batch * n * R1, nv = (size_t)batch * n;
  const int st0[2] = {0, 0};
  Scratch s(nullptr, nullptr);
  const double* dband = s.upload(band, nb);
  const double* dmu = mu_part ? s.upload(mu_part, nv) : nullptr;
  const double* dz = z ? s.upload(z, nv) : nullptr;
  double *dx = s.alloc<double>(nv), *dwork = s.alloc<double>(nb + 2 * nv);
  int *dtries = s.alloc<int>((size_t)batch), *dstatus = s.upload(st0, 2);
  MvnArgs a{dband, dmu, dz, dx, dwork, n, bw, seed, eps0, attempts < 0 ? 0 : attempts, dtries, dstatus};
  const size_t lds = ((size_t)(bw * (bw + 1) / 2 + 3) / 4 + 1) * sizeof(double);
  s.launch(mvn_banded_kernel, dim3(batch), dim3(WAVE), lds, a);
  int st[2] = {0, 0};
  s.download(st, dstatus, 2);
  s.download(x_out, dx, nv);
  s.download(tries_out, dtries, (size_t)batch);
  const int rc = s.finish();
  if (rc) return rc;
  if (st[0]) return fail(nullptr, BTF_ENOTPD, "precision not positive definite in batch item " + std::to_string(st[1]));
  return BTF_OK;
}

int btf_mvn_dense(int device, int batch, int n, const double* A, int form, const double* mu, const double* mu_part,
                  const double* z, uint64_t seed, double eps0, int attempts, double* x_out, int32_t* tries_out) {
  if (batch < 1 || n < 1 || n > 1024 || !A || !x_out || (form & ~3) || (mu && mu_part))
    return fail(nullptr, BTF_EINVAL, "bad dense mvn arguments (1 <= n <= 1024; mu and mu_part are mutually exclusive)");
  hipError_t e = hipSetDevice(device);
  if (e != hipSuccess) return fail(nullptr, BTF_EHIP, std::string("hipSetDevice: ") + hipGetErrorString(e));
  const size_t nm = (size_t)batch * n * n, nv = (size_t)batch * n;
  const int st0[2] = {0, 0};
  Scratch s(nullptr, nullptr);
  const double* dA = s.upload(A, nm);
  const double* dmu = mu ? s.upload(mu, nv) : nullptr;
  const double* dmp = mu_part ? s.upload(mu_part, nv) : nullptr;
  const double* dz = z ? s.upload(z, nv) : nullptr;
  double *dx = s.alloc<double>(nv), *dwork = s.alloc<double>(nm);
  int *dtries = s.alloc<int>((size_t)batch), *dstatus = s.upload(st0, 2);
  MvnDenseArgs a{dA, dmu, dmp, dz, dx, dwork, n, form, (unsigned long long)seed, eps0, attempts < 0 ? 0 : attempts, dtries, dstatus};
  s.launch(mvn_dense_kernel, dim3(batch), dim3(MVD_THREADS), 2 * (size_t)n * sizeof(double), a);
  int st[2] = {0, 0};
  s.download(st, dstatus, 2);
  s.download(x_out, dx, nv);
  s.download(tries_out, dtries, (size_t)batch);
  const int rc = s.finish();
  if (rc) return rc;
  if (st[0]) return fail(nullptr, BTF_ENOTPD, "matrix not positive definite in batch item " + std::to_string(st[1]));
  return BTF_OK;
}

int btf_set_profiling(btf_ctx* c, int on) {
  if (!c) return BTF_EINVAL;
  HIPCHK(c, hipSetDevice(c->dev));
  if (on && c->ev_pool.empty()) {
    c->ev_pool.resize(MAX_EVENTS);
    for (auto& e : c->ev_pool) {
      HIPCHK(c, hipEventCreate(&e.a));
      HIPCHK(c, hipEventCreate(&e.b));
    }
  }
  c->profiling = on != 0;
  return BTF_OK;
}

int btf_kernel_times(btf_ctx* c, double* ms_total, int64_t* launches) {
  if (!c || !ms_total || !launches) return BTF_EINVAL;
  HIPCHK(c, hipSetDevice(c->dev));
  HIPCHK(c, hipStreamSynchronize(c->stream));
  int64_t timed[BTF_K_COUNT] = {0};
  for (size_t i = 0; i < c->ev_used; ++i) {
    float ms = 0.f;
    if (hipEventElapsedTime(&ms, c->ev_pool[i].a, c->ev_pool[i].b) == hipSuccess) {
      c->ms_total[c->ev_pool[i].kid] += ms;
      timed[c->ev_pool[i].kid]++;
    }
  }
  for (int k = 0; k < BTF_K_COUNT; ++k) {
    ms_total[k] = c->ms_total[k];
    launches[k] = c->profiling ? timed[k] : c->launches[k];
    c->ms_total[k] = 0.0;
    c->launches[k] = 0;
  }
  c->ev_used = 0;
  return BTF_OK;
}

extern "C" int btf_debug_eig(btf_ctx* c, double* out) {
  if (!c || !out) return BTF_EINVAL;
  if (!c->eig) return fail(c, BTF_ESTATE, "no eigen-system yet");
  HIPCHK(c, hipSetDevice(c->dev));
  HIPCHK(c, hipStreamSynchronize(c->stream));
  HIPCHK(c, hipMemcpy(out, c->eig, ((size_t)c->K + c->K * c->K + 8) * sizeof(double), hipMemcpyDeviceToHost));
  return BTF_OK;
}
#ifdef BTF_ACC_STAMPS
extern "C" int btf_debug_acc_stamps(btf_ctx* c, long long* out) {
  if (!c) return BTF_EINVAL;
  HIPCHK(c, hipSetDevice(c->dev));
  HIPCHK(c, hipStreamSynchronize(c->stream));
  if (!c->acc_stamps) {
    int rc = dev_alloc(c, &c->acc_stamps, (size_t)8192 * 8);
    if (rc) return rc;
  }
  HIPCHK(c, hipMemcpy(out, c->acc_stamps, sizeof(long long) * 8192 * 8, hipMemcpyDeviceToHost));
  HIPCHK(c, hipMemset(c->acc_stamps, 0, sizeof(long long) * 8192 * 8));
  return BTF_OK;
}
#endif
extern "C" int btf_debug_stamps(btf_ctx* c, long long* out) {
  if (!c) return BTF_EINVAL;
  HIPCHK(c, hipSetDevice(c->dev));
  if (!c->dbg) {
    int rc = dev_alloc(c, &c->dbg, (size_t)c->M * 6);
    if (rc) return rc;
    HIPCHK(c, hipMemset(c->dbg, 0, (size_t)c->M * 6 * sizeof(long long)));
    return BTF_OK;
  }
  HIPCHK(c, hipStreamSynchronize(c->stream));
  HIPCHK(c, hipMemcpy(out, c->dbg, (size_t)c->ml * 6 * sizeof(long long), hipMemcpyDeviceToHost));
  return BTF_OK;
}

int btf_set_tuning(btf_ctx* c, int rows_per_block_w, int rows_per_block_v) {
  if (!c || rows_per_block_w < 0 || rows_per_block_v < 0) return fail(c, BTF_EINVAL, "rows per workgroup must be >= 0 (0 = default)");
  c->rpb_w = rows_per_block_w; c->rpb_v = rows_per_block_v;
  return BTF_OK;
}

int btf_set_option(btf_ctx* c, int option, int value) {
  if (!c) return BTF_EINVAL;
  switch (option) {
    case BTF_OPT_SAMPLER:
      if (value < BTF_SAMPLER_BANDED || value > BTF_SAMPLER_BANDED_NOPANEL) return fail(c, BTF_EINVAL, "unknown sampler");
      c->sampler = value;
      c->ngp_v = 0;
      return BTF_OK;
    case BTF_OPT_NB_HISTOGRAMS:
      c->nb_hist = value != 0;
      return BTF_OK;
    case BTF_OPT_PG_EXACT:
      if (value < PG_MODE_DEFAULT || value > PG_MODE_SERIES_ALL) return fail(c, BTF_EINVAL, "unknown Polya-Gamma mode");
      c->pg_mode = value;
      return BTF_OK;
    case BTF_OPT_FUSE_GRAM:
      c->fuse_gram = value != 0;
      c->ngp_v = c->ngp_w = 0;
      return BTF_OK;
    case BTF_OPT_FUSED_STEP:
      if (value < 0 || value > 2) return fail(c, BTF_EINVAL, "BTF_OPT_FUSED_STEP: 0, 1 or 2");
      c->fused_step = value;
      return BTF_OK;
    case BTF_OPT_FUSED_DATAFLOW:
      c->fused_dataflow = value != 0 ? 1 : 0;
      return BTF_OK;
    case BTF_OPT_FUSED_SWEEP:
      c->fused_sweep = value != 0;
      c->sse_cols_valid = false;
      return BTF_OK;
    case BTF_OPT_SPLIT_ACCUM:
      c->split_accum = value != 0;
      c->w_local_done = c->v_local_done = false; c->sse_cols_valid = false;
      return BTF_OK;
    case BTF_OPT_CURVE_COUNTS:
      c->curve_opt = value != 0;
      c->ngp_v = c->ngp_w = 0;
      c->w_part_valid = false; c->w_local_done = c->v_local_done = false; c->sse_cols_valid = false;
      return BTF_OK;
    default:
      return fail(c, BTF_EINVAL, "unknown option");
  }
}

int btf_get_likelihood_form(btf_ctx* c, int32_t* form) {
  if (!c || !form) return BTF_EINVAL;
  if (!c->have_data) return fail(c, BTF_ESTATE, "set data first");
  *form = !c->weighted ? BTF_LIK_COMPLETE : (curve_on(c) ? BTF_LIK_CURVE_COUNTS : BTF_LIK_WEIGHTED);
  return BTF_OK;
}

int btf_get_draw_counters(btf_ctx* c, uint64_t* w, uint64_t* v) {
  if (!c || !w || !v) return BTF_EINVAL;
  *w = c->sweep_w; *v = c->sweep_v;
  return BTF_OK;
}

int btf_set_draw_counters(btf_ctx* c, uint64_t w, uint64_t v) {
  if (!c) return BTF_EINVAL;
  c->sweep_w = w; c->sweep_v = v;
  c->sse_cols_valid = false;
  HIPCHK(c, hipSetDevice(c->dev));
  const size_t rec = (size_t)c->K + (size_t)c->K * c->K + 8;
  if (c->eig) HIPCHK(c, hipMemsetAsync(c->eig, 0, rec * sizeof(double), c->stream));
  if (c->eig_cols) HIPCHK(c, hipMemsetAsync(c->eig_cols, 0, (size_t)c->M * rec * sizeof(double), c->stream));
  return BTF_OK;
}

int btf_comm_fork(btf_ctx* c, void* comm_stream) {
  if (!c || !comm_stream) return BTF_EINVAL;
  HIPCHK(c, hipSetDevice(c->dev));
  int rc;
  if (!(c->ev_draw && split_applies(c))) { if ((rc = mark_draw(c))) return rc; }
  HIPCHK(c, hipStreamWaitEvent((hipStream_t)comm_stream, c->ev_draw, 0));
  return BTF_OK;
}
int btf_comm_join(btf_ctx* c, void* comm_stream) {
  if (!c || !comm_stream) return BTF_EINVAL;
  HIPCHK(c, hipSetDevice(c->dev));
  if (!c->ev_join) HIPCHK(c, hipEventCreateWithFlags(&c->ev_join, hipEventDisableTiming));
  HIPCHK(c, hipEventRecord(c->ev_join, (hipStream_t)comm_stream));
  HIPCHK(c, hipStreamWaitEvent(c->stream, c->ev_join, 0));
  return BTF_OK;
}

namespace {
#define RCCLCHK(ctx, api, call)                                                                     \
  do {                                                                                              \
    ncclResult_t r__ = (call);                                                                      \
    if (r__ != ncclSuccess)                                                                         \
      return fail(ctx, BTF_EHIP, std::string(#call) + ": " + (api)->GetErrorString(r__));           \
  } while (0)

int comm_ready(btf_ctx* c, RcclApi** api) {
  if (!c) return BTF_EINVAL;
  *api = nullptr;
  if (c->peer_on) { HIPCHK(c, hipSetDevice(c->dev)); return BTF_OK; }
  if (!c->comm) return fail(c, BTF_ESTATE, "no communicator: btf_comm_init (or btf_peer_init) first");
  std::string why;
  if (!(*api = rccl_api(&why))) return fail(c, BTF_EHIP, why);
  HIPCHK(c, hipSetDevice(c->dev));
  return BTF_OK;
}
int comm_blocks_match(btf_ctx* c) {
  const int r = c->gather_rank, w = c->gather_world;
  if (c->row0 != comm_block_lo(c->N, r, w) || c->nl != comm_block_len(c->N, r, w) ||
      c->col0 != comm_block_lo(c->M, r, w) || c->ml != comm_block_len(c->M, r, w))
    return fail(c, BTF_ESTATE, "btf_set_shard blocks are not rank " + std::to_string(r) + " of " + std::to_string(w) +
                                   "'s equal chunks ceil(n / world) (btf_comm_block)");
  return BTF_OK;
}
int peer_collective(btf_ctx* c, int which, size_t off, size_t len, const double* red_src, double* red_dst, int red_n, hipStream_t s) {
  if (c->gather_world <= 1) {
    if (red_n && red_dst != red_src) HIPCHK(c, hipMemcpyAsync(red_dst, red_src, (size_t)red_n * sizeof(double), hipMemcpyDeviceToDevice, s));
    return BTF_OK;
  }
  PeerArgs a{};
  a.tab = c->peer_tab; a.rank = c->gather_rank; a.world = c->gather_world; a.which = which;
  static const int wpp_cap = [] { const char* e = std::getenv("BTF_PEER_WPP"); const int v = e && *e ? std::atoi(e) : 64; return std::min(64, std::max(1, v)); }();
  static const int wg_bytes = [] { const char* e = std::getenv("BTF_PEER_WG_BYTES"); const int v = e && *e ? std::atoi(e) : 16384; return std::max(4096, v); }();
  a.wpp = len ? (int)std::min<size_t>((size_t)wpp_cap, std::max<size_t>(1, (len * sizeof(double) + wg_bytes - 1) / wg_bytes)) : 1;
  a.epoch = ++c->peer_epoch; a.off = off; a.len = len;
  a.red_src = red_src; a.red_dst = red_dst; a.red_n = red_n;
  a.counters = c->peer_counters; a.status = c->status; a.timeout_ticks = c->peer_timeout_ticks;
  hipLaunchKernelGGL(peer_exchange_kernel, dim3((unsigned)((a.world - 1) * a.wpp)), dim3(PEER_THREADS), 0, s, a);
  HIPCHK(c, hipGetLastError());
  return BTF_OK;
}
int comm_gather(btf_ctx* c, RcclApi* api, double* buf, size_t chunk, hipStream_t s) {
  if (c->peer_on) {
    const bool isW = buf == c->W;
    const size_t unit = isW ? (size_t)c->K : (size_t)c->T * c->K;
    return peer_collective(c, isW ? 0 : 1, (size_t)(isW ? c->row0 : c->col0) * unit, (size_t)(isW ? c->nl : c->ml) * unit, nullptr, nullptr, 0, s);
  }
  if (c->comm_rehearse) {
    const size_t n = chunk * (size_t)c->gather_world;
    if (2 * n > c->comm_scr_elems) {
      int rc;
      HIPCHK(c, hipStreamSynchronize(c->stream));
      if (c->comm_stream) HIPCHK(c, hipStreamSynchronize(c->comm_stream));
      if ((rc = dev_alloc(c, &c->comm_scr, 2 * n))) return rc;
      c->comm_scr_elems = 2 * n;
      HIPCHK(c, hipMemsetAsync(c->comm_scr, 0, 2 * n * sizeof(double), s));
    }
    RCCLCHK(c, api, api->AllGather(c->comm_scr, c->comm_scr + n, n, ncclDouble, c->comm, s));
    return BTF_OK;
  }
  RCCLCHK(c, api, api->AllGather(buf + (size_t)c->comm_rank * chunk, buf, chunk, ncclDouble, c->comm, s));
  return BTF_OK;
}
int comm_gather_ordered(btf_ctx* c, double* buf, size_t chunk) {
  RcclApi* api;
  int rc;
  if ((rc = comm_ready(c, &api))) return rc;
  if ((rc = comm_blocks_match(c))) return rc;
  if (!c->split_accum) return comm_gather(c, api, buf, chunk, c->stream);
  if (!c->comm_stream) HIPCHK(c, hipStreamCreateWithFlags(&c->comm_stream, hipStreamNonBlocking));
  if ((rc = btf_comm_fork(c, c->comm_stream))) return rc;
  if ((rc = comm_gather(c, api, buf, chunk, c->comm_stream))) return rc;
  return btf_comm_join(c, c->comm_stream);
}
int comm_adopt(btf_ctx* c, RcclApi* api, int rank, int world, const ncclUniqueId& id) {
  if (c->comm) { int rc = btf_comm_destroy(c); if (rc) return rc; }
  HIPCHK(c, hipSetDevice(c->dev));
  RCCLCHK(c, api, api->CommInitRank(&c->comm, world, id, rank));
  c->comm_rank = rank; c->comm_world = world;
  if (!c->comm_words) { int rc = dev_alloc(c, &c->comm_words, (size_t)16); if (rc) return rc; }
  return BTF_OK;
}
}

int btf_comm_unique_id(unsigned char* id, int nbytes) {
  if (!id || nbytes < BTF_COMM_ID_BYTES) return fail(nullptr, BTF_EINVAL, "id buffer of BTF_COMM_ID_BYTES bytes expected");
  static_assert(sizeof(ncclUniqueId) == BTF_COMM_ID_BYTES, "BTF_COMM_ID_BYTES is NCCL_UNIQUE_ID_BYTES");
// ... 339 lines not shown
```

### functionalmf_amd/csrc/btf_instances.h

```cpp
#pragma once
#include "btf_kernels.h"
#include "btf_banded_twist.h"
#include "btf_spectral.h"
#include "btf_fused.h"

namespace btf {

#define BTF_ACC_ARGS_F(XT, CT, FZ) \
  (const XT*, const CT*, const double*, const int*, double*, int, int, int, EigSide, EigSideCols, TauSide, GramSide, ChunkMap, SweepSide, FZ)
#define BTF_ACC_ARGS(XT, CT) BTF_ACC_ARGS_F(XT, CT, FuseNone)
#define BTF_ACCUM_SET(P, K)                                                                              \
  P void accum_kernel<K, 0> BTF_ACC_ARGS(double, double);                                                \
  P void accum_kernel<K, 0, acc_waves(K, 0), double, double, 3> BTF_ACC_ARGS(double, double);            \
  P void accum_kernel<K, 1> BTF_ACC_ARGS(double, double);                                                \
  P void accum_kernel<K, 2> BTF_ACC_ARGS(double, double);                                                \
  P void accum_kernel<K, 1, acc_waves(K, 1), unsigned char> BTF_ACC_ARGS(double, unsigned char);         \
  P void accum_kernel<K, 2, acc_waves(K, 2), unsigned char> BTF_ACC_ARGS(double, unsigned char);         \
  P void accum_kernel<K, 1, acc_waves(K, 1), double, signed char> BTF_ACC_ARGS(signed char, double);     \
  P void accum_kernel<K, 2, acc_waves(K, 2), double, signed char> BTF_ACC_ARGS(signed char, double);

#define BTF_ACCUM_K10W_SET(P)                                                                            \
  P void accum_kernel<10, 0, ACC_WAVES> BTF_ACC_ARGS(double, double);

#define BTF_FUSED_W_SET(P, K)                                                                            \
  P void accum_kernel<K, 0, 16, double, double, 0, 2, FUSE_W> BTF_ACC_ARGS_F(double, double, FuseW);
#define BTF_FUSED_V_SET(P, K)                                                                            \
  P void accum_kernel<K, 0, 16, double, double, 0, 2, FUSE_V> BTF_ACC_ARGS_F(double, double, FuseV);
#define BTF_FUSED_VDF_SET(P, K)                                                                          \
  P void accum_kernel<K, 0, 16, double, double, 0, 2, FUSE_VDF> BTF_ACC_ARGS_F(double, double, FuseV);
#define BTF_LEAN_SET(P, K)                                                                               \
  P void accum_kernel<K, 0, 16, double, double, 0, 2, FUSE_LEAN> BTF_ACC_ARGS(double, double);
#define BTF_FUSED_UNR3_SET(P, K)                                                                         \
  P void accum_kernel<K, 0, 16, double, double, 3, 2, FUSE_W> BTF_ACC_ARGS_F(double, double, FuseW);     \
  P void accum_kernel<K, 0, 16, double, double, 3, 2, FUSE_V> BTF_ACC_ARGS_F(double, double, FuseV);
#define BTF_FUSED_SET(P)                                                                                 \
  BTF_FUSED_W_SET(P, 1) BTF_FUSED_W_SET(P, 2) BTF_FUSED_W_SET(P, 3) BTF_FUSED_W_SET(P, 4)                \
  BTF_FUSED_W_SET(P, 5) BTF_FUSED_W_SET(P, 6) BTF_FUSED_W_SET(P, 7) BTF_FUSED_W_SET(P, 8)                \
  BTF_FUSED_V_SET(P, 1) BTF_FUSED_V_SET(P, 2) BTF_FUSED_V_SET(P, 3) BTF_FUSED_V_SET(P, 4)                \
  BTF_FUSED_V_SET(P, 5) BTF_FUSED_V_SET(P, 6) BTF_FUSED_V_SET(P, 7) BTF_FUSED_V_SET(P, 8)                \
  BTF_FUSED_VDF_SET(P, 1) BTF_FUSED_VDF_SET(P, 2) BTF_FUSED_VDF_SET(P, 3) BTF_FUSED_VDF_SET(P, 4)        \
  BTF_FUSED_VDF_SET(P, 5) BTF_FUSED_VDF_SET(P, 6)                                                        \
  BTF_LEAN_SET(P, 1) BTF_LEAN_SET(P, 2) BTF_LEAN_SET(P, 3) BTF_LEAN_SET(P, 4)                            \
  BTF_LEAN_SET(P, 5) BTF_LEAN_SET(P, 6) BTF_LEAN_SET(P, 7) BTF_LEAN_SET(P, 8)                            \
  BTF_FUSED_UNR3_SET(P, 8)

#define BTF_WSOLVE_SET(P, K)                                                                             \
  P void w_solve_kernel<K, false, 8>(WSolveArgs);  P void w_solve_kernel<K, true, 8>(WSolveArgs);        \
  P void w_solve_kernel<K, false, 16>(WSolveArgs); P void w_solve_kernel<K, true, 16>(WSolveArgs);       \
  P void w_solve_kernel<K, false, 32>(WSolveArgs); P void w_solve_kernel<K, true, 32>(WSolveArgs);       \
  P void w_solve_kernel<K, false, 64>(WSolveArgs); P void w_solve_kernel<K, true, 64>(WSolveArgs);

#define BTF_PG_ARGS                                                                                      \
  (const double*, double*, const double*, const double*, int, int, int, int, unsigned long long, unsigned long long, \
   unsigned long long, unsigned long long, int, int)
#define BTF_PGT_ARGS \
  (const double*, double*, double*, const double*, const double*, int, int, int, int, unsigned long long, int, int)
#define BTF_PG_SET(P, K)                                                                                 \
  P void pg_kernel<K, PG_PATH_SERIES> BTF_PG_ARGS;       P void pg_kernel<K, PG_PATH_EXACT> BTF_PG_ARGS;  \
  P void pg_tile_kernel<K, PG_PATH_SERIES> BTF_PGT_ARGS; P void pg_tile_kernel<K, PG_PATH_EXACT> BTF_PGT_ARGS; \
  P void pgx_kernel<K, PGX_CPL> BTF_PG_ARGS;             P void pgx_tile_kernel<K, PGX_NW, PGX_CPL> BTF_PGT_ARGS;

#define BTF_NB_ARGS \
  (const double*, int, const double*, const double*, int, int, const double*, const double*, long long, long long, long long, int, double*)
#define BTF_NB_SET(P, K)                                                                                 \
  P void nb_loglik_kernel<K, 0> BTF_NB_ARGS; P void nb_loglik_kernel<K, 1> BTF_NB_ARGS;                  \
  P void nb_loglik_kernel<K, 2> BTF_NB_ARGS; P void nb_loglik_kernel<K, 3> BTF_NB_ARGS;                  \
  P void nb_loglik_kernel<K, 4> BTF_NB_ARGS;

#define BTF_TWIST_SET(P)                                                                                 \
  P void v_banded_twist_kernel<1, true>(VBandArgs, int);  P void v_banded_twist_kernel<2, true>(VBandArgs, int);  \
  P void v_banded_twist_kernel<2, false>(VBandArgs, int); P void v_banded_twist_kernel<3, false>(VBandArgs, int); \
  P void v_banded_twist_kernel<4, false>(VBandArgs, int); P void v_banded_twist_kernel<5, false>(VBandArgs, int); \
  P void v_banded_twist_kernel<6, false>(VBandArgs, int); P void v_banded_twist_kernel<7, false>(VBandArgs, int); \
  P void v_banded_twist_kernel<8, false>(VBandArgs, int);                                                \
  BTF_TWIST_FIXED(P, 1, 2) BTF_TWIST_FIXED(P, 2, 2) BTF_TWIST_FIXED(P, 3, 2) BTF_TWIST_FIXED(P, 4, 2) BTF_TWIST_FIXED(P, 5, 2) \
  BTF_TWIST_FIXED(P, 6, 2) BTF_TWIST_FIXED(P, 7, 2) BTF_TWIST_FIXED(P, 8, 2) BTF_TWIST_FIXED(P, 9, 2) BTF_TWIST_FIXED(P, 10, 2) \
  BTF_TWIST_FIXED_T(P, 5, 2, 64) BTF_TWIST_FIXED_T(P, 8, 2, 64)
#define BTF_TWIST_FIXED(P, K, TF) P void v_banded_twist_kernel<tw_npl(K, TF), tw_row16(K, TF), K, TF>(VBandArgs, int);
#define BTF_TWIST_FIXED_T(P, K, TF, T) P void v_banded_twist_kernel<tw_npl(K, TF), tw_row16(K, TF), K, TF, T>(VBandArgs, int);

#define BTF_FOR_K(SET, P) \
  SET(P, 1) SET(P, 2) SET(P, 3) SET(P, 4) SET(P, 5) SET(P, 6) SET(P, 7) SET(P, 8) SET(P, 9) SET(P, 10)

constexpr int BTF_INST_PARTS = 9;

#ifndef BTF_INST_PART
#define BTF_X extern template __global__
BTF_FOR_K(BTF_ACCUM_SET, BTF_X)
BTF_ACCUM_K10W_SET(BTF_X)
BTF_FOR_K(BTF_WSOLVE_SET, BTF_X)
BTF_FOR_K(BTF_PG_SET, BTF_X)
BTF_FOR_K(BTF_NB_SET, BTF_X)
BTF_TWIST_SET(BTF_X)
BTF_FUSED_SET(BTF_X)
#undef BTF_X
#else
#define BTF_D template __global__
#if BTF_INST_PART == 0
BTF_ACCUM_SET(BTF_D, 10) BTF_ACCUM_K10W_SET(BTF_D) BTF_ACCUM_SET(BTF_D, 4)
#elif BTF_INST_PART == 1
BTF_ACCUM_SET(BTF_D, 9) BTF_ACCUM_SET(BTF_D, 5)
#elif BTF_INST_PART == 2
BTF_ACCUM_SET(BTF_D, 8) BTF_ACCUM_SET(BTF_D, 6)
#elif BTF_INST_PART == 3
BTF_ACCUM_SET(BTF_D, 7) BTF_ACCUM_SET(BTF_D, 3) BTF_ACCUM_SET(BTF_D, 2) BTF_ACCUM_SET(BTF_D, 1)
#elif BTF_INST_PART == 4
BTF_FOR_K(BTF_WSOLVE_SET, BTF_D)
#elif BTF_INST_PART == 5
BTF_FOR_K(BTF_PG_SET, BTF_D)
#elif BTF_INST_PART == 6
BTF_FOR_K(BTF_NB_SET, BTF_D)
#elif BTF_INST_PART == 7
BTF_TWIST_SET(BTF_D)
#elif BTF_INST_PART == 8
BTF_FUSED_SET(BTF_D)
#else
#error "BTF_INST_PART out of range"
#endif
#undef BTF_D
#endif

}
```

### functionalmf_amd/csrc/btf_instances.hip

```cpp
#ifndef BTF_INST_PART
#error "compile with -DBTF_INST_PART=<0..7>"
#endif
#include "btf_instances.h"
```

### functionalmf_amd/csrc/btf_kernels.h

```cpp
#pragma once
#include <type_traits>
#include "btf_device.h"
#include "btf_eig.h"
#include "btf_pg_exact.h"

namespace btf {

#ifndef BTF_ACC_WAVES
#define BTF_ACC_WAVES 16
#endif
#ifndef BTF_DF_UNR
#define BTF_DF_UNR 4
#endif
#ifndef BTF_DF_PREFETCH
#define BTF_DF_PREFETCH 1
#endif
#ifndef BTF_DF_SHARE
#define BTF_DF_SHARE 0
#endif
#ifndef BTF_ACC_UNR
#define BTF_ACC_UNR 2
#endif
#ifndef BTF_ACC_PF_WT
#define BTF_ACC_PF_WT 0
// ... 668 lines not shown
              estate = 2;
            } else {
              eflag = __hip_atomic_load(fuse_eig_flag<FUSE>(fz), __ATOMIC_RELAXED, __HIP_MEMORY_SCOPE_AGENT);
              estate = 1;
            }
          }
          compute(rb, A);
          if (!df_band_done) { v_df_band_store<K, 3>(fz, tile, &red[0][0][0], dfpre); df_band_done = true; }
        }
        if (rb < r1) {
          Rows A;
          load_rows(rb, A, std::false_type{}, ntc);
          compute(rb, A);
        }
      }
      rb = r1;
    }
    for (; rb < full_end; rb += STEP) {
      Rows A;
      load_rows(rb, A, std::true_type{}, ntc);
      compute(rb, A);
    }
  }
  if constexpr (!ULDS) {
    if (rb < r1) {
      Rows A;
      load_rows(rb, A, std::false_type{}, ntc);
      compute(rb, A);
    }
  }

  };
  if (nt) run_stream(std::true_type{}); else run_stream(std::false_type{});
  ACC_STAMP(2);
  if constexpr (dataflow) {
    if (!df_band_done) {
      v_df_band_load<K, 3>(fz, tile, dfpre);
      v_df_band_store<K, 3>(fz, tile, &red[0][0][0], dfpre);
    }
    v_fused_df<K, 3, WAVES, ACC_RG, NV>(fz, tile, &red[0][0][0], acc, ACC_TAIL_STAMPS, df_early);
    return;
  }
  if constexpr (FUSE == FUSE_V) {
    if constexpr (ULDS) v_fused_prefetch_loads<K, 3>(fz, tile, vpre, band_early);
#if BTF_VF_BANDPRE
    if (band_early) v_fused_band_store<K, 3>(fz, tile, &red[0][0][0], vpre, UNRV == 3);
#endif
    v_fused_prefetch<K, 3>(fz, tile, &red[0][0][0] + RED_SLOTS * RED_SLOT - VF_MAILBOX_DOUBLES, vpre, band_early);
  }
  const int tv = threadIdx.x >> 7;
  const int tc = threadIdx.x & 127;
  constexpr int NFS = PLAIN ? 1 : (NV + ACC_RG - 1) / ACC_RG;
  double fsum[NFS];
#pragma unroll
  for (int r = 0; r < NFS; ++r) fsum[r] = 0.0;
#pragma unroll
  for (int g = 0; g < NV; g += ACC_RG) {
    if (MODE == 2 && !gram_any && g >= K) break;
#pragma unroll
    for (int v = 0; v < ACC_RG; ++v) {
      if (g + v < NV) {
        if constexpr (OPL == 2) *reinterpret_cast<double2*>(&red[wave][v][2 * lane]) = make_double2(acc[g + v][0], acc[g + v][1]);
        else red[wv][v][64 * half + lane] = acc[g + v][0];
      }
    }
    __syncthreads();
    if constexpr (!ULDS) { if (g == 0) ACC_STAMP(1); }
    if (tv < ACC_RG && g + tv < NV && !(MODE == 2 && !gram_on && g + tv >= K)) {
      double s = 0.0;
#pragma unroll
      for (int w = 0; w < NWR; ++w) s += red[w][tv][tc];
      if constexpr (PLAIN) {
#ifdef BTF_PART_SC1
        store_sc1(&part[((size_t)chunk * NV + (g + tv)) * ld + (size_t)tile * ACC_TILE + tc], s);
#else
        part[((size_t)chunk * NV + (g + tv)) * ld + (size_t)tile * ACC_TILE + tc] = s;
#endif
      } else {
        if (FUSE == FUSE_W || fuse_tickets<FUSE>(fz)) store_sc1(&part[((size_t)chunk * NV + (g + tv)) * ld + (size_t)tile * ACC_TILE + tc], s);
        if constexpr (FUSE == FUSE_V) fsum[g / ACC_RG] = s;
      }
    }
    __syncthreads();
  }
  ACC_STAMP(3);
  if constexpr (FUSE == FUSE_W) {
    drain_stores();
    __syncthreads();
    if (threadIdx.x == 0) __hip_atomic_fetch_add((gu32_t*)(fuse_tickets<FUSE>(fz) + tile), 1u, __ATOMIC_RELAXED, __HIP_MEMORY_SCOPE_AGENT);
  }
  if constexpr (FUSE == FUSE_V) {
    double* lds = &red[0][0][0];
    unsigned* tickets = fuse_tickets<FUSE>(fz);
    if (tickets) {
      drain_stores();
      __syncthreads();
      if (!last_arriver_of(tickets + tile, (unsigned)fuse_chunks<FUSE>(fz), reinterpret_cast<unsigned*>(lds))) return;
    }
    v_fused_tail<K, 3, WAVES, NFS>(fz, tile, lds, fsum, ACC_RG, tv, tc, ACC_TAIL_STAMPS, vpre, lds + RED_SLOTS * RED_SLOT - VF_MAILBOX_DOUBLES, band_early, UNRV == 3);
  }
}

constexpr int GRAM_BLOCKS = 64;
__host__ inline int gram_blocks(int Rdim) { int b = Rdim / 1024; return b < 16 ? 16 : (b > GRAM_BLOCKS ? GRAM_BLOCKS : b); }
constexpr int GRAM_THREADS = 256;

template <int K>
__global__ __launch_bounds__(GRAM_THREADS) void gram_kernel(const double* __restrict__ U, int Rdim,
                                                            double* __restrict__ gpart) {
  constexpr int KK = tri(K);
  __shared__ double red[GRAM_THREADS / WAVE][KK];
  double acc[KK];
#pragma unroll
  for (int q = 0; q < KK; ++q) acc[q] = 0.0;
  for (int r = blockIdx.x * GRAM_THREADS + threadIdx.x; r < Rdim; r += gridDim.x * GRAM_THREADS) {
    double u[K];
#pragma unroll
    for (int k = 0; k < K; ++k) u[k] = U[(size_t)r * K + k];
#pragma unroll
    for (int a = 0; a < K; ++a)
#pragma unroll
      for (int b = 0; b <= a; ++b) acc[lidx(a, b)] = fma(u[a], u[b], acc[lidx(a, b)]);
  }
  const int lane = threadIdx.x & 63, wave = threadIdx.x >> 6;
#pragma unroll
  for (int q = 0; q < KK; ++q) {
    double s = wave_sum(acc[q]);
    if (lane == 0) red[wave][q] = s;
  }
  __syncthreads();
  if (threadIdx.x < KK) {
    double s = 0.0;
    for (int w = 0; w < GRAM_THREADS / WAVE; ++w) s += red[w][threadIdx.x];
    gpart[blockIdx.x * KK + threadIdx.x] = s;
  }
}

__device__ __forceinline__ int gram_lanes(int KK) {
  const int l = (int)blockDim.x / KK;
  return l > 32 ? 32 : (l < 1 ? 1 : l);
}
__device__ __forceinline__ void reduce_gram_tail(double s, int KK, double scale, double* scratch, double* G) {
  const int lanes = gram_lanes(KK);
  const int l = threadIdx.x / KK, q = threadIdx.x - l * KK;
  if (l < lanes) scratch[l * KK + q] = s;
  __syncthreads();
  if ((int)threadIdx.x < KK) {
    double t = 0.0;
    for (int b = 0; b < lanes; ++b) t += scratch[b * KK + threadIdx.x];
    G[threadIdx.x] = t * scale;
  }
  __syncthreads();
}
__device__ inline void reduce_gram(const double* __restrict__ gpart, int ngp, int KK, double scale,
                                   double* scratch, double* G) {
  const int lanes = gram_lanes(KK);
  const int l = threadIdx.x / KK, q = threadIdx.x - l * KK;
  double s = 0.0;
  if (l < lanes) {
    for (int b0 = l; b0 < ngp; b0 += 8 * lanes) {
      double x[8];
#pragma unroll
      for (int u = 0; u < 8; ++u) x[u] = b0 + u * lanes < ngp ? gpart[(size_t)(b0 + u * lanes) * KK + q] : 0.0;
#pragma unroll
      for (int u = 0; u < 8; ++u) s += x[u];
    }
  }
  reduce_gram_tail(s, KK, scale, scratch, G);
}

__device__ __forceinline__ bool gram_early_ok(int ngp, int KK) { return ngp <= 8 * gram_lanes(KK); }
__device__ __forceinline__ void reduce_gram_fetch(const double* __restrict__ gpart, int ngp, int KK, double (&x)[8]) {
  const int lanes = gram_lanes(KK);
  const int l = threadIdx.x / KK, q = threadIdx.x - l * KK;
#pragma unroll
  for (int u = 0; u < 8; ++u) x[u] = (l < lanes && l + u * lanes < ngp) ? gpart[(size_t)(l + u * lanes) * KK + q] : 0.0;
}
__device__ inline void reduce_gram_finish(const double (&x)[8], int ngp, int KK, double scale, double* scratch, double* G) {
  double s = 0.0;
#pragma unroll
  for (int u = 0; u < 8; ++u) s += x[u];
  reduce_gram_tail(s, KK, scale, scratch, G);
}

template <int K>
__global__ __launch_bounds__(WAVE) void colgram_kernel(const double* __restrict__ V, int T, int ncols, double* __restrict__ out) {
  constexpr int KK = tri(K);
  const int j = blockIdx.x, lane = threadIdx.x;
  if (j >= ncols) return;
  double acc[KK];
#pragma unroll
  for (int q = 0; q < KK; ++q) acc[q] = 0.0;
  for (int t = lane; t < T; t += WAVE) {
    double v[K];
#pragma unroll
    for (int k = 0; k < K; ++k) v[k] = V[((size_t)j * T + t) * K + k];
#pragma unroll
    for (int a = 0; a < K; ++a)
#pragma unroll
      for (int b = 0; b <= a; ++b) acc[lidx(a, b)] = fma(v[a], v[b], acc[lidx(a, b)]);
  }
#pragma unroll
  for (int q = 0; q < KK; ++q) {
    const double t = wave_sum(acc[q]);
    if (lane == 0) out[(size_t)j * KK + q] = t;
  }
}

struct WSolveArgs {
  const double* part; int nch; int ld;
  const int* gsrc;
  const double* gpart; int ngp;
  int weighted;
  double s;
  double sR;
  double inv_sigma2;
  double* W; int row0; int nl;
  const double* z; unsigned long long seed; unsigned long long stream;
  int* status;
  double* gout;
  const double* hyp;
  double Rrep;
  int hyp_noise;
  CurveLists cv;
  const double* cv_blocks;
  int nside;
  LamSide lam;
  BandSide band;
#ifdef BTF_WS_STAMPS
  long long* dbg;
#endif
};
#ifdef BTF_WS_STAMPS
#define WS_STAMP(n) do { if (threadIdx.x == 0 && a.dbg) a.dbg[(size_t)blockIdx.x * 6 + (n)] = (long long)__builtin_amdgcn_s_memtime(); } while (0)
#else
#define WS_STAMP(n) do {} while (0)
#endif

enum { HYP_NU2 = 0, HYP_SIGMA2 = 1, HYP_LAM2 = 2, HYP_LAM2A = 3, HYP_SSE = 4, HYP_WSQ = 5, HYP_COUNT = 8 };
__device__ inline void band_side(const BandSide& bs, int j, double* itau, int nthreads) {
  const double* tau = bs.Tau2 + (size_t)(bs.col0 + j) * bs.nD;
  double tv[2] = {1.0, 1.0};
  int p0[2] = {0, 0}, p1[2] = {0, 0};
#pragma unroll
  for (int u = 0; u < 2; ++u) {
    const int r = threadIdx.x + u * nthreads, e0 = threadIdx.x + u * nthreads;
    if (r < bs.nD) tv[u] = tau[r];
    if (e0 < bs.TD1) { p0[u] = bs.st_ptr[e0]; p1[u] = bs.st_ptr[e0 + 1]; }
  }
  double lam2 = bs.hyp ? bs.hyp[HYP_LAM2] : bs.lam2;
  if (bs.lam_flag) {
    __shared__ int okf;
    if (threadIdx.x == 0) {
      bool seen = false;
      for (unsigned spins = 0; spins < (1u << 22); ++spins) {
        if (__hip_atomic_load((const gu32_t*)bs.lam_flag, __ATOMIC_RELAXED, __HIP_MEMORY_SCOPE_AGENT) == bs.epoch) { seen = true; break; }
        __builtin_amdgcn_s_sleep(8);
      }
      okf = seen ? 1 : 0;
      if (!seen && atomicCAS(&bs.status[0], 0, 2) == 0) bs.status[1] = -2;
    }
    __syncthreads();
    if (!okf) return;
    lam2 = load_sc1(bs.lam_pub + HYP_LAM2);
  }
#pragma unroll
  for (int u = 0; u < 2; ++u) {
    const int r = threadIdx.x + u * nthreads;
    if (r < bs.nD) itau[r] = 1.0 / __dmul_rn(lam2, tv[u]);
  }
  __syncthreads();
#pragma unroll
  for (int u = 0; u < 2; ++u) {
    const int e0 = threadIdx.x + u * nthreads;
    if (e0 < bs.TD1) {
      double s = 0.0;
      for (int e = p0[u]; e < p1[u]; ++e) s = fma(bs.st_coef[e], itau[bs.st_row[e]], s);
      bs.pband[(size_t)j * bs.TD1 + e0] = s;
      if (bs.pimg) {
        const int t = e0 / bs.img_D1, d = e0 - t * bs.img_D1;
        double* im = bs.pimg + (size_t)j * 2 * bs.img_PB;
        im[e0] = s;
        if (t + d < bs.img_T) im[bs.img_PB + (bs.img_T - 1 - t - d) * bs.img_D1 + d] = s;
      }
    }
  }
}


constexpr int WS_ROWS = 64;
__host__ __device__ constexpr int ws_split(int K) { return K <= 6 ? 8 : (K <= 8 ? 4 : 2); }
#ifndef BTF_WS_SPLIT_U
#define BTF_WS_SPLIT_U 4
#endif
__host__ __device__ constexpr int ws_split_of(int K, bool weighted) { return weighted ? ws_split(K) : (K <= 6 ? BTF_WS_SPLIT_U : ws_split(K)); }
__host__ __device__ constexpr size_t ws_gram_stage(int K, bool weighted) {
  return (size_t)ws_split_of(K, weighted) * (K + tri(K)) * WS_ROWS;
}

__host__ __device__ constexpr int ws_rows_for(int nl) { return nl > 2048 ? 64 : (nl > 1024 ? 32 : (nl > 512 ? 16 : 8)); }

constexpr int WS_CHB = 32;
template <bool SC1 = false>
__device__ __forceinline__ double chunk_sum_seq(const double* __restrict__ p, size_t cst, int nch) {
  double s = 0.0;
  int c = 0;
  for (; c + WS_CHB <= nch; c += WS_CHB) {
    double x[WS_CHB];
#pragma unroll
    for (int u = 0; u < WS_CHB; ++u) x[u] = SC1 ? load_sc1(p + (size_t)(c + u) * cst) : p[(size_t)(c + u) * cst];
#pragma unroll
    for (int u = 0; u < WS_CHB; ++u) s += x[u];
  }
  if (c < nch) {
    double x[WS_CHB];
#pragma unroll
    for (int u = 0; u < WS_CHB; ++u) x[u] = c + u < nch ? (SC1 ? load_sc1(p + (size_t)(c + u) * cst) : p[(size_t)(c + u) * cst]) : 0.0;
#pragma unroll
    for (int u = 0; u < WS_CHB; ++u) if (c + u < nch) s += x[u];
  }
  return s;
}

template <int K, bool WEIGHTED, int RW = WS_ROWS>
__global__ __launch_bounds__(WS_ROWS * ws_split_of(K, WEIGHTED)) void w_solve_kernel(WSolveArgs a) {
  constexpr int KK = tri(K);
  constexpr int SUB = WS_ROWS / RW;
  constexpr int WS_SPLIT = ws_split_of(K, WEIGHTED);
  constexpr int NVMAX = WEIGHTED ? K + KK : K;
  constexpr int NV = NVMAX;
  WS_STAMP(0);
  constexpr int UNR = WEIGHTED ? (K + KK > 24 ? 1 : 2) : 4;
  __shared__ double G[KK];
  __shared__ double red[WS_SPLIT][K + KK][WS_ROWS];
  __shared__ double zsh[K][WS_ROWS];
  __shared__ double cvq[WEIGHTED ? 1 : RW][WEIGHTED ? 1 : KK];
  const int lane = threadIdx.x & 63, grp = threadIdx.x >> 6;
  if (a.nside) {
    const int nsolve = (int)gridDim.x - a.nside;
    if ((int)blockIdx.x >= nsolve) {
      int b = (int)blockIdx.x - nsolve;
      if (a.lam.hyp) {
        if (b == 0) { sweep_lam_side<WS_ROWS * WS_SPLIT / WAVE>(a.lam, &red[0][0][0]); return; }
        --b;
      }
      if (a.band.pband && b < a.band.ml) band_side(a.band, b, &red[0][0][0], WS_ROWS * WS_SPLIT);
      return;
    }
  }
  if constexpr (!WEIGHTED) {
    if (a.cv.ptr) {
      constexpr int NT = WS_ROWS * WS_SPLIT, G = NT / KK, CAP = (WS_SPLIT * (K + KK) * WS_ROWS) / KK;
      const int i0 = a.row0 + blockIdx.x * RW, i1 = min(i0 + RW, a.row0 + a.nl);
      const int e0 = a.cv.ptr[i0], e1 = a.cv.ptr[i1];
      double* stage = &red[0][0][0];
      const int g = threadIdx.x / KK, q = threadIdx.x - g * KK;
      if (g < G)
        for (int r = g; r < RW; r += G) cvq[r][q] = 0.0;
      for (int eb = e0; eb < e1; eb += CAP) {
        const int ee = min(eb + CAP, e1);
        if (g < G) {
          for (int e = eb + g; e < ee; e += G)
            stage[(size_t)(e - eb) * KK + q] = a.cv.def[e] * a.cv_blocks[(size_t)a.cv.idx[e] * KK + q];
        }
        __syncthreads();
        if (g < G) {
          for (int r = g; r < RW && i0 + r < i1; r += G) {
            double acc = cvq[r][q];
            for (int e = max(a.cv.ptr[i0 + r], eb); e < min(a.cv.ptr[i0 + r + 1], ee); ++e) acc += stage[(size_t)(e - eb) * KK + q];
            cvq[r][q] = acc;
          }
        }
        __syncthreads();
      }
    }
  }
  if (a.hyp) {
    if (a.hyp_noise) { a.s = 1.0 / a.hyp[HYP_NU2]; a.sR = a.s * a.Rrep; }
    a.inv_sigma2 = 1.0 / a.hyp[HYP_SIGMA2];
  }
  double gx[8];
  bool g_early = false;
  if constexpr (!WEIGHTED) {
    g_early = gram_early_ok(a.ngp, KK);
    if (g_early) reduce_gram_fetch(a.gpart, a.ngp, KK, gx);
    else reduce_gram(a.gpart, a.ngp, KK, a.sR, &red[0][0][0], G);
  }
  const int rr = lane % RW, sub = lane / RW;
  const int il = blockIdx.x * RW + rr;
  constexpr int CS = WS_SPLIT * SUB;
  if constexpr (!WEIGHTED) {
    constexpr int NT = WS_ROWS * WS_SPLIT;
    const size_t cst = (size_t)NV * a.ld;
    for (int t = threadIdx.x; t < RW * K; t += NT) {
      const int v = t / RW, r = t - v * RW;
      const int ilr = blockIdx.x * RW + r;
      red[0][v][r] = ilr < a.nl ? chunk_sum_seq(a.part + (size_t)v * a.ld + ilr, cst, a.nch) : 0.0;
    }
    for (int t = NT - 1 - (int)threadIdx.x; t < RW * K; t += NT) {
      const int k = t / RW, r = t - k * RW;
      const int ilr = blockIdx.x * RW + r;
      double zv = 0.0;
      if (ilr < a.nl) {
        const int i = a.row0 + ilr;
        const long long zoff = w_z_offset(i, K);
        const int d = i + 1 < K ? i + 1 : K;
        if (k < d) zv = a.z ? a.z[zoff + k] : philox_normal(a.seed, a.stream, (unsigned long long)(zoff + k));
      }
      zsh[k][r] = zv;
    }
    if (g_early) reduce_gram_finish(gx, a.ngp, KK, a.sR, &red[1][0][0], G);
  } else {
  {
    double part[NVMAX];
#pragma unroll
    for (int v = 0; v < NVMAX; ++v) part[v] = 0.0;
    const size_t cst = (size_t)NV * a.ld;
    const bool live1 = il < a.nl;
    const ptrdiff_t goff = (a.gsrc && live1) ? (ptrdiff_t)a.gsrc[il] - (ptrdiff_t)il : 0;
    int c = grp * SUB + sub;
    double x0[UNR][NV];
    const bool first = live1 && c < a.nch;
    int nfirst = 0;
    if (first) {
      const double* p = a.part + (size_t)c * cst + il;
#pragma unroll
      for (int u = 0; u < UNR; ++u) {
        const bool has = c + u * CS < a.nch;
        nfirst += has ? 1 : 0;
#pragma unroll
        for (int v = 0; v < NV; ++v) x0[u][v] = has ? p[(ptrdiff_t)((size_t)u * CS * cst + (size_t)v * a.ld) + (v >= K ? goff : 0)] : 0.0;
      }
    }
    if (live1) {
      const int i = a.row0 + il;
      const long long zoff = w_z_offset(i, K);
      const int d = i + 1 < K ? i + 1 : K;
      for (int k = CS - 1 - (grp * SUB + sub); k < K; k += CS)
        zsh[k][rr] = k < d ? (a.z ? a.z[zoff + k] : philox_normal(a.seed, a.stream, (unsigned long long)(zoff + k))) : 0.0;
    }
    if (first) {
#pragma unroll
      for (int u = 0; u < UNR; ++u)
        if (u < nfirst) {
#pragma unroll
          for (int v = 0; v < NV; ++v) part[v] += x0[u][v];
        }
      c += nfirst * CS;
    }
    if (live1) {
      for (; c + (UNR - 1) * CS < a.nch; c += UNR * CS) {
        const double* p = a.part + (size_t)c * cst + il;
        double x[UNR][NV];
#pragma unroll
        for (int u = 0; u < UNR; ++u)
#pragma unroll
          for (int v = 0; v < NV; ++v) x[u][v] = p[(ptrdiff_t)((size_t)u * CS * cst + (size_t)v * a.ld) + (v >= K ? goff : 0)];
#pragma unroll
        for (int u = 0; u < UNR; ++u)
#pragma unroll
          for (int v = 0; v < NV; ++v) part[v] += x[u][v];
      }
      for (; c < a.nch; c += CS) {
        const double* p = a.part + (size_t)c * cst + il;
#pragma unroll
        for (int v = 0; v < NV; ++v) part[v] += p[(ptrdiff_t)((size_t)v * a.ld) + (v >= K ? goff : 0)];
      }
    }
    if constexpr (!WEIGHTED) {
      if (g_early) reduce_gram_finish(gx, a.ngp, KK, a.sR, &red[0][0][0], G);
    }
#pragma unroll
    for (int st = RW; st < WS_ROWS; st <<= 1)
#pragma unroll
      for (int v = 0; v < NVMAX; ++v) part[v] += __shfl_xor(part[v], st);
#pragma unroll
    for (int v = 0; v < NVMAX; ++v) red[grp][v][lane] = part[v];
  }
  }
  WS_STAMP(1);
  __syncthreads();
  WS_STAMP(2);
#ifndef BTF_WS_TWO_LEVEL_MIN
#define BTF_WS_TWO_LEVEL_MIN 128
#endif
  constexpr bool TWO_LEVEL = WEIGHTED && WS_SPLIT * (K + KK) > BTF_WS_TWO_LEVEL_MIN;
  if constexpr (TWO_LEVEL) {
    for (int v = grp; v < NV; v += WS_SPLIT) {
      double s2 = 0.0;
#pragma unroll
      for (int w = 0; w < WS_SPLIT; ++w) s2 += red[w][v][lane];
      red[0][v][lane] = s2;
    }
    __syncthreads();
  }
  constexpr int NSH = (TWO_LEVEL || !WEIGHTED) ? 1 : WS_SPLIT;
  if (grp != 0) return;
  WS_STAMP(3);
  const bool live = lane < RW && il < a.nl;
  const int i = a.row0 + (live ? il : 0);
  const int d = i + 1 < K ? i + 1 : K;
  double m[K], Q[KK];
#pragma unroll
  for (int k = 0; k < K; ++k) {
    double s = 0.0;
#pragma unroll
    for (int w = 0; w < NSH; ++w) s += red[w][k][rr];
    m[k] = __dmul_rn(s, a.s);
  }
#pragma unroll
  for (int q = 0; q < KK; ++q) {
    if constexpr (WEIGHTED) {
      double s = 0.0;
#pragma unroll
      for (int w = 0; w < NSH; ++w) s += red[w][K + q][rr];
      Q[q] = __dmul_rn(s, a.s);
    } else {
      Q[q] = G[q];
    }
  }
  if constexpr (!WEIGHTED) {
    if (a.cv.ptr && live) {
#pragma unroll
      for (int q = 0; q < KK; ++q) Q[q] = fma(-a.s, cvq[rr][q], Q[q]);
    }
  }
#pragma unroll
  for (int k = 0; k < K; ++k) Q[lidx(k, k)] += a.inv_sigma2;
#pragma unroll
  for (int r = 0; r < K; ++r) {
    if (r >= d) {
      m[r] = 0.0;
#pragma unroll
      for (int c = 0; c <= r; ++c) Q[lidx(r, c)] = (r == c) ? 1.0 : 0.0;
    }
  }
  bool ok = true;
  double invl[K];
#pragma unroll
  for (int c = 0; c < K; ++c) {
    double p = Q[lidx(c, c)];
#pragma unroll
    for (int q = 0; q < c; ++q) p = fma(-Q[lidx(c, q)], Q[lidx(c, q)], p);
    if (!(p > 0.0)) ok = false;
    const double inv = rsq_nr(p);
    const double l = __dmul_rn(p, inv);
    invl[c] = inv;
    Q[lidx(c, c)] = l;
#pragma unroll
    for (int r = c + 1; r < K; ++r) {
      double v = Q[lidx(r, c)];
#pragma unroll
      for (int q = 0; q < c; ++q) v = fma(-Q[lidx(r, q)], Q[lidx(c, q)], v);
      Q[lidx(r, c)] = __dmul_rn(v, inv);
    }
  }
  if (live && !ok && atomicCAS(&a.status[0], 0, 1) == 0) a.status[1] = i;
  WS_STAMP(4);
  double y[K];
#pragma unroll
  for (int r = 0; r < K; ++r) {
    double v = m[r];
#pragma unroll
    for (int c = 0; c < r; ++c) v = fma(-Q[lidx(r, c)], y[c], v);
    y[r] = __dmul_rn(v, invl[r]);
  }
#pragma unroll
  for (int r = 0; r < K; ++r)
    if (r < d) y[r] = __dadd_rn(y[r], zsh[r][rr]);
#pragma unroll
  for (int r = K - 1; r >= 0; --r) {
    double v = y[r];
#pragma unroll
    for (int c = r + 1; c < K; ++c) v = fma(-Q[lidx(c, r)], y[c], v);
    y[r] = __dmul_rn(v, invl[r]);
  }
  double wrow[K];
#pragma unroll
  for (int r = 0; r < K; ++r) {
    const bool fresh = live && ok && r < d;
    if (fresh) a.W[(size_t)i * K + r] = y[r];
    wrow[r] = fresh ? y[r] : 0.0;
  }
  if (live && (d < K || !ok)) {
#pragma unroll
    for (int r = 0; r < K; ++r)
      if (!(ok && r < d)) wrow[r] = a.W[(size_t)i * K + r];
  }
  if (a.gout) {
    typedef double v4f64_w __attribute__((ext_vector_type(4)));
    double* stg = &red[0][0][0];
#pragma unroll
    for (int r = 0; r < K; ++r) stg[r * WS_ROWS + lane] = wrow[r];
    const int kk = lane >> 4, ii = lane & 15;
    const double* src = stg + (ii < K ? ii : 0) * WS_ROWS + kk;
    v4f64_w acc = {0.0, 0.0, 0.0, 0.0};
#pragma unroll
    for (int sidx = 0; sidx < (RW + 3) / 4; ++sidx) {
      const double x = ii < K ? src[4 * sidx] : 0.0;
      acc = __builtin_amdgcn_mfma_f64_16x16x4f64(x, x, acc, 0, 0, 0);
    }
#pragma unroll
    for (int r = 0; r < 4; ++r) {
      const int row = 4 * r + kk;
      if (row < K && ii <= row) a.gout[(size_t)blockIdx.x * KK + lidx(row, ii)] = acc[r];
    }
  }
  WS_STAMP(5);
}

struct VBandArgs {
  const double* part; int nch; int ld;
  const int* gsrc;
  const double* gpart; int ngp;
  int weighted;
  double s, sR;
  const double* Tau2; double lam2; int nD;
  const int* st_ptr; const int* st_row; const double* st_coef;
  int T, TF;
  int col0, ml;
  double* V;
  const double* z; unsigned long long seed; unsigned long long stream;
  double eps0; int attempts;
  int* status;
  int* tries;
  double* gband;
  size_t gband_stride;
  long long* dbg;
  double* gout;
  const double* pband;
  const double* hyp;
  double Rrep;
  int hyp_noise;
  int panel4;
  const int* fill;
  int nfill;
  int ql_global;
  CurveLists cv;
  const double* cv_W;
  const int* st_drow; const double* st_dcoef;
};
constexpr int PB_MAXE = 16;
__device__ __forceinline__ void vband_load_hyp(VBandArgs& a) {
  if (a.hyp) {
    if (a.hyp_noise) { a.s = 1.0 / a.hyp[HYP_NU2]; a.sR = a.s * a.Rrep; }
    a.lam2 = a.hyp[HYP_LAM2];
  }
}

static __global__ void prior_band_kernel(const double* __restrict__ Tau2, double lam2, int nD,
                                  const int* __restrict__ st_ptr, const int* __restrict__ st_row,
                                  const double* __restrict__ st_coef, int TD1, int col0, int ml,
                                  double* __restrict__ pband, const double* __restrict__ hyp, int spectral_form,
                                  double* __restrict__ pimg, int img_T, int img_D1, int img_PB) {
  const int idx = blockIdx.x * blockDim.x + threadIdx.x;
  if (idx >= ml * TD1) return;
  if (hyp) lam2 = hyp[HYP_LAM2];
  const int j = idx / TD1, e0 = idx - j * TD1;
  const double* tau = Tau2 + (size_t)(col0 + j) * nD;
  double s = 0.0;
  if (spectral_form) {
    for (int e = st_ptr[e0]; e < st_ptr[e0 + 1]; ++e) {
      const double it = 1.0 / __dmul_rn(lam2, tau[st_row[e]]);
      s = fma(st_coef[e], it, s);
    }
  } else {
    for (int e = st_ptr[e0]; e < st_ptr[e0 + 1]; ++e) s += st_coef[e] / (lam2 * tau[st_row[e]]);
  }
  pband[idx] = s;
  if (pimg) {
    const int t = e0 / img_D1, d = e0 - t * img_D1;
    double* im = pimg + (size_t)j * 2 * img_PB;
    im[e0] = s;
    if (t + d < img_T) im[img_PB + (img_T - 1 - t - d) * img_D1 + d] = s;
  }
}

static __global__ __launch_bounds__(256) void prior_band_cols_kernel(const double* __restrict__ Tau2, double lam2, int nD,
                                  const int* __restrict__ st_ptr, const int* __restrict__ st_row,
                                  const double* __restrict__ st_coef, int TD1, int col0,
                                  double* __restrict__ pband, const double* __restrict__ hyp,
                                  double* __restrict__ pimg, int img_T, int img_D1, int img_PB) {
  __shared__ double itau[256];
  const int j = blockIdx.x;
  if (hyp) lam2 = hyp[HYP_LAM2];
  const double* tau = Tau2 + (size_t)(col0 + j) * nD;
  int p0[2], p1[2];
#pragma unroll
  for (int u = 0; u < 2; ++u) {
    const int e0 = threadIdx.x + u * 256;
    p0[u] = e0 < TD1 ? st_ptr[e0] : 0;
    p1[u] = e0 < TD1 ? st_ptr[e0 + 1] : 0;
  }
  for (int r = threadIdx.x; r < nD; r += 256) itau[r] = 1.0 / __dmul_rn(lam2, tau[r]);
  __syncthreads();
#pragma unroll
  for (int u = 0; u < 2; ++u) {
    const int e0 = threadIdx.x + u * 256;
    if (e0 < TD1) {
      double s = 0.0;
      for (int e = p0[u]; e < p1[u]; ++e) s = fma(st_coef[e], itau[st_row[e]], s);
      pband[(size_t)j * TD1 + e0] = s;
      if (pimg) {
        const int t = e0 / img_D1, d = e0 - t * img_D1;
        double* im = pimg + (size_t)j * 2 * img_PB;
        im[e0] = s;
        if (t + d < img_T) im[img_PB + (img_T - 1 - t - d) * img_D1 + d] = s;
      }
    }
  }
}

__device__ inline void fill_pair_table(unsigned short* ptab, int bw) {
  const int npairs = bw * (bw + 1) / 2;
  for (int q = threadIdx.x; q < npairs; q += WAVE) {
    int a = (int)((sqrt(8.0 * q + 1.0) - 1.0) * 0.5) + 1;
    while ((a - 1) * a / 2 > q) --a;
    while (a * (a + 1) / 2 <= q) ++a;
    const int b = q - (a - 1) * a / 2 + 1;
    ptab[q] = (unsigned short)((a << 8) | b);
  }
}

__device__ inline bool banded_factor_forward(double* Bc, double* rhs, double* invd, const unsigned short* ptab,
                                             int n, int bw) {
  const int lane = threadIdx.x;
  const int R1 = bw + 1;
  const int npairs = bw * (bw + 1) / 2;
  for (int nn = 0; nn < n; ++nn) {
    const int len = min(bw, n - 1 - nn);
    double* col = Bc + (size_t)nn * R1;
    double v = (lane <= len) ? col[lane] : 0.0;
    const double p = bcast_first(v);
    if (!(p > 0.0)) return false;
    const double l = sqrt(p);
    const double inv = 1.0 / l;
    double x = v * inv;
    if (lane == 0) {
      x = l;
      invd[nn] = inv;
    }
    if (lane <= len) col[lane] = x;
    const double yn = rhs[nn] * inv;
    if (lane == 0) rhs[nn] = yn;
    else if (lane <= len) rhs[nn + lane] -= x * yn;
    for (int q = lane; q < npairs; q += WAVE) {
      const int ab = ptab[q];
      const int a = ab >> 8, b = ab & 255;
      if (a <= len) {
        const double xa = col[a];
        const double xb = col[b];
        Bc[(size_t)(nn + b) * R1 + (a - b)] -= xa * xb;
      }
    }
  }
  return true;
}

__device__ inline void banded_backward(const double* Bc, double* rhs, const double* invd, int n, int bw) {
  const int lane = threadIdx.x;
  const int R1 = bw + 1;
// ... 1642 lines not shown
```

Before: 26800 sweeps/s.

## Add row-owner kernel fusing W accumulation and solve; shrink small-N solve tiles

Adds an opt-in fused kernel (fused_step=3) in which each block owns four rows of W. It streams the data and V chains to accumulate the row statistics, reduces the V gram, and performs the Cholesky solve and sampling in one launch, removing the separate accumulate/solve passes and the partial buffers between them. The per-row solve is factored into a shared helper. Separately, the solve row tile for nl ≤ 512 drops from 8 to 4. This doubles the block count and the number of gram partials that later reductions must sum.

New measurement: 26770 sweeps/s. Within noise of the previous version (-0.1%).

```diff
diff --git a/functionalmf_amd/_native.py b/functionalmf_amd/_native.py
--- a/functionalmf_amd/_native.py
+++ b/functionalmf_amd/_native.py
@@ -179,7 +179,7 @@
 
 
 INST_SOURCE = os.path.join(CSRC, "btf_instances.hip")
-INST_PARTS = 9
+INST_PARTS = 10
 OBJ_DIR = os.path.join(ROOT, "build", "obj")
 
 
diff --git a/functionalmf_amd/csrc/btf_abi.hip b/functionalmf_amd/csrc/btf_abi.hip
--- a/functionalmf_amd/csrc/btf_abi.hip
+++ b/functionalmf_amd/csrc/btf_abi.hip
@@ -495,10 +495,14 @@
   a.nside = (a.lam.hyp ? 1 : 0) + (a.band.pband ? a.band.ml : 0);
   const dim3 grid((a.nl + rw - 1) / rw + a.nside);
 #define WS_LAUNCH(WT, RWV) p.launch(w_solve_kernel<K, WT, RWV>, grid, dim3(WS_ROWS * ws_split_of(K, WT)), 0, a)
-#define WS_PICK(WT) do { if (rw == 8) WS_LAUNCH(WT, 8); else if (rw == 16) WS_LAUNCH(WT, 16); else if (rw == 32) WS_LAUNCH(WT, 32); else WS_LAUNCH(WT, 64); } while (0)
+#define WS_PICK(WT) do { if (rw == 4) WS_LAUNCH(WT, 4); else if (rw == 8) WS_LAUNCH(WT, 8); else if (rw == 16) WS_LAUNCH(WT, 16); else if (rw == 32) WS_LAUNCH(WT, 32); else WS_LAUNCH(WT, 64); } while (0)
   if (a.weighted) WS_PICK(true); else WS_PICK(false);
 #undef WS_PICK
 #undef WS_LAUNCH
+}
+template <int K>
+void launch_row_owner(Prof& p, int blocks, const RowOwnerArgs& ra) {
+  if constexpr (K <= 6) p.launch(w_row_owner_kernel<K>, dim3(blocks), dim3(RO_THREADS), 0, ra);
 }
 template <int K>
 hipError_t launch_vbanded(btf_ctx* c, const VBandArgs& a, size_t lds_bytes) {
@@ -941,7 +945,7 @@
   hipError_t e = hipSetDevice(device);
   if (e != hipSuccess) { g_err = std::string("hipSetDevice: ") + hipGetErrorString(e); delete c; return BTF_EHIP; }
   { int n = 0; if (hipDeviceGetAttribute(&n, hipDeviceAttributeMultiprocessorCount, device) == hipSuccess && n > 0) c->ncu = n; }
-  { const char* e = std::getenv("BTF_FUSED_STEP"); if (e) c->fused_step = std::max(0, std::min(2, std::atoi(e))); }
+  { const char* e = std::getenv("BTF_FUSED_STEP"); if (e) c->fused_step = std::max(0, std::min(3, std::atoi(e))); }
   { const char* e = std::getenv("BTF_LAM_IN_WSOLVE"); if (e) c->lam_in_wsolve = std::atoi(e) != 0; }
   { const char* e = std::getenv("BTF_BAND_IN_WSOLVE"); if (e) c->band_in_wsolve = std::atoi(e) != 0; }
   { const char* e = std::getenv("BTF_VF_DATAFLOW"); if (e) c->fused_dataflow = std::atoi(e) != 0 ? 1 : 0; }
@@ -1440,12 +1444,19 @@
   return BTF_OK;
 }
 bool fuse_w_applies(const btf_ctx* c, bool wt, bool cv, int mode, int rpb) {
-  if (c->fused_step < 2 || wt || cv || mode != 0 || c->nl <= 0 || c->K > 8) return false;
+  if (c->fused_step != 2 || wt || cv || mode != 0 || c->nl <= 0 || c->K > 8) return false;
   if (split_applies(c)) return false;
   if (rpb >= unr3_min_rpb() && c->K != 8) return false;
   return true;
 }
 struct WFuseReq { const double* dz; uint64_t seed; bool done; };
+bool row_owner_applies(const btf_ctx* c, bool wt, bool cv, int mode, int rpb, bool use_gv) {
+  if (c->fused_step != 3 || wt || cv || mode != 0 || c->K > 6 || !use_gv || !c->A_v) return false;
+  if (!(c->nl == c->N && c->ml == c->M) || split_applies(c) || !ro_rows_ok(c->nl)) return false;
+  if (c->sc_pending || c->lam_pending || (c->tau_pending && c->dev_scalars && c->have_chain)) return false;
+  if ((long long)c->M * c->T * c->K * 8 >= (1LL << 31) || (long long)c->ldv * 8 >= (1LL << 31)) return false;
+  return rpb % 64 == 0 && acc_waves(c->K, 0) == RO_CHAIN_WAVES;
+}
 int w_accum_phase(btf_ctx* c, int compat, int part = ACC_ALL, WFuseReq* wf = nullptr) {
   const int K = c->K, KK = c->KK, MT = c->M * c->T;
   const bool wt = lik_weighted(c), cv = c->weighted && !wt;
@@ -1484,6 +1495,38 @@
     }
     use_gv = true;
   }
+  if (c->nl > 0 && wf && !rest_only && row_owner_applies(c, wt, cv, mode, rpb, use_gv)) {
+    RowOwnerArgs ra{};
+    WSolveArgs& a = ra.a;
+    a.ld = c->ldw; a.weighted = 0;
+    a.gpart = c->gpart_v; a.ngp = c->ngp_v;
+    if (c->fuse_gram) {
+      if (!c->gpart_w) { if ((rc = dev_alloc(c, &c->gpart_w, (size_t)std::max(64, (c->N + ws_rows_for(c->N) - 1) / ws_rows_for(c->N)) * KK))) return rc; }
+      a.gout = c->gpart_w;
+    }
+    a.s = c->binomial ? 1.0 : 1.0 / c->nu2;
+    a.sR = a.s * c->R;
+    a.inv_sigma2 = 1.0 / c->sigma2;
+    a.hyp = c->dev_scalars ? c->hyp : nullptr; a.Rrep = c->R; a.hyp_noise = c->binomial ? 0 : 1;
+    a.W = c->W; a.row0 = c->row0; a.nl = c->nl;
+#ifdef BTF_WS_STAMPS
+    a.dbg = c->dbg;
+#endif
+    a.z = wf->dz; a.seed = wf->seed; a.stream = 2 * c->sweep_w + 0x10000ULL;
+    a.status = c->status;
+    ra.X = c->A_v; ra.V = c->V; ra.ld = c->ldv; ra.MT = MT; ra.rpb = rpb; ra.nch = nch;
+    {
+      Prof p(c, BTF_K_W_ACCUM);
+      K_SWITCH(K, launch_row_owner<KT>(p, (c->nl + RO_ROWS - 1) / RO_ROWS, ra));
+    }
+    HIPCHK(c, hipGetLastError());
+    wf->done = true;
+    c->ngp_w = a.gout ? (c->nl + RO_ROWS - 1) / RO_ROWS : 0;
+    c->ngp_v = 0;
+    c->w_part_valid = true; c->w_part_mode = mode; c->w_part_nch = nch; c->w_part_rpb = rpb; c->w_part_gv = use_gv;
+    c->w_part_curve = cv;
+    return BTF_OK;
+  }
   if (c->nl > 0) {
     GramSide gram{nullptr, 0, nullptr, 0};
     if (!wt && !use_gv) {
@@ -1525,7 +1568,7 @@
       a.part = c->part; a.nch = nch_total; a.ld = c->ldw; a.weighted = 0;
       a.gpart = use_gv ? c->gpart_v : c->gpart; a.ngp = use_gv ? c->ngp_v : c->ngp_gram;
       if (whole && c->fuse_gram) {
-        if (!c->gpart_w) { if ((rc = dev_alloc(c, &c->gpart_w, (size_t)std::max(64, (c->N + WS_ROWS - 1) / WS_ROWS) * KK))) return rc; }
+        if (!c->gpart_w) { if ((rc = dev_alloc(c, &c->gpart_w, (size_t)std::max(64, (c->N + ws_rows_for(c->N) - 1) / ws_rows_for(c->N)) * KK))) return rc; }
         a.gout = c->gpart_w;
       }
       a.s = c->binomial ? 1.0 : 1.0 / c->nu2;
@@ -1620,7 +1663,7 @@
     const int wrows = ws_rows_for(c->nl);
     const int wblocks = (c->nl + wrows - 1) / wrows;
     if (whole && c->fuse_gram) {
-      if (!c->gpart_w) { if ((rc = dev_alloc(c, &c->gpart_w, (size_t)std::max(64, (c->N + WS_ROWS - 1) / WS_ROWS) * KK))) return rc; }
+      if (!c->gpart_w) { if ((rc = dev_alloc(c, &c->gpart_w, (size_t)std::max(64, (c->N + ws_rows_for(c->N) - 1) / ws_rows_for(c->N)) * KK))) return rc; }
       a.gout = c->gpart_w;
     }
     a.s = c->binomial ? 1.0 : 1.0 / c->nu2;
@@ -4164,7 +4207,7 @@
       c->ngp_v = c->ngp_w = 0;
       return BTF_OK;
     case BTF_OPT_FUSED_STEP:
-      if (value < 0 || value > 2) return fail(c, BTF_EINVAL, "BTF_OPT_FUSED_STEP: 0, 1 or 2");
+      if (value < 0 || value > 3) return fail(c, BTF_EINVAL, "BTF_OPT_FUSED_STEP: 0, 1, 2 or 3");
       c->fused_step = value;
       return BTF_OK;
     case BTF_OPT_FUSED_DATAFLOW:
diff --git a/functionalmf_amd/csrc/btf_instances.h b/functionalmf_amd/csrc/btf_instances.h
--- a/functionalmf_amd/csrc/btf_instances.h
+++ b/functionalmf_amd/csrc/btf_instances.h
@@ -3,6 +3,7 @@
 #include "btf_banded_twist.h"
 #include "btf_spectral.h"
 #include "btf_fused.h"
+#include "btf_row_owner.h"
 
 namespace btf {
 
@@ -45,10 +46,16 @@
   BTF_FUSED_UNR3_SET(P, 8)
 
 #define BTF_WSOLVE_SET(P, K)                                                                             \
+  P void w_solve_kernel<K, false, 4>(WSolveArgs);  P void w_solve_kernel<K, true, 4>(WSolveArgs);        \
   P void w_solve_kernel<K, false, 8>(WSolveArgs);  P void w_solve_kernel<K, true, 8>(WSolveArgs);        \
   P void w_solve_kernel<K, false, 16>(WSolveArgs); P void w_solve_kernel<K, true, 16>(WSolveArgs);       \
   P void w_solve_kernel<K, false, 32>(WSolveArgs); P void w_solve_kernel<K, true, 32>(WSolveArgs);       \
   P void w_solve_kernel<K, false, 64>(WSolveArgs); P void w_solve_kernel<K, true, 64>(WSolveArgs);
+
+#define BTF_ROW_OWNER_SET(P)                                                                             \
+  P void w_row_owner_kernel<1>(RowOwnerArgs); P void w_row_owner_kernel<2>(RowOwnerArgs);                \
+  P void w_row_owner_kernel<3>(RowOwnerArgs); P void w_row_owner_kernel<4>(RowOwnerArgs);                \
+  P void w_row_owner_kernel<5>(RowOwnerArgs); P void w_row_owner_kernel<6>(RowOwnerArgs);
 
 #define BTF_PG_ARGS                                                                                      \
   (const double*, double*, const double*, const double*, int, int, int, int, unsigned long long, unsigned long long, \
@@ -82,7 +89,7 @@
 #define BTF_FOR_K(SET, P) \
   SET(P, 1) SET(P, 2) SET(P, 3) SET(P, 4) SET(P, 5) SET(P, 6) SET(P, 7) SET(P, 8) SET(P, 9) SET(P, 10)
 
-constexpr int BTF_INST_PARTS = 9;
+constexpr int BTF_INST_PARTS = 10;
 
 #ifndef BTF_INST_PART
 #define BTF_X extern template __global__
@@ -93,6 +100,7 @@
 BTF_FOR_K(BTF_NB_SET, BTF_X)
 BTF_TWIST_SET(BTF_X)
 BTF_FUSED_SET(BTF_X)
+BTF_ROW_OWNER_SET(BTF_X)
 #undef BTF_X
 #else
 #define BTF_D template __global__
@@ -114,6 +122,8 @@
 BTF_TWIST_SET(BTF_D)
 #elif BTF_INST_PART == 8
 BTF_FUSED_SET(BTF_D)
+#elif BTF_INST_PART == 9
+BTF_ROW_OWNER_SET(BTF_D)
 #else
 #error "BTF_INST_PART out of range"
 #endif
diff --git a/functionalmf_amd/csrc/btf_instances.hip b/functionalmf_amd/csrc/btf_instances.hip
--- a/functionalmf_amd/csrc/btf_instances.hip
+++ b/functionalmf_amd/csrc/btf_instances.hip
@@ -1,4 +1,4 @@
 #ifndef BTF_INST_PART
-#error "compile with -DBTF_INST_PART=<0..7>"
+#error "compile with -DBTF_INST_PART=<0..9>"
 #endif
 #include "btf_instances.h"
diff --git a/functionalmf_amd/csrc/btf_kernels.h b/functionalmf_amd/csrc/btf_kernels.h
--- a/functionalmf_amd/csrc/btf_kernels.h
+++ b/functionalmf_amd/csrc/btf_kernels.h
@@ -844,20 +844,22 @@
   }
   __syncthreads();
 }
+__device__ __forceinline__ double gram_lane_sum(const double* __restrict__ gpart, int ngp, int KK, int lanes, int l, int q) {
+  double s = 0.0;
+  for (int b0 = l; b0 < ngp; b0 += 8 * lanes) {
+    double x[8];
+#pragma unroll
+    for (int u = 0; u < 8; ++u) x[u] = b0 + u * lanes < ngp ? gpart[(size_t)(b0 + u * lanes) * KK + q] : 0.0;
+#pragma unroll
+    for (int u = 0; u < 8; ++u) s += x[u];
+  }
+  return s;
+}
 __device__ inline void reduce_gram(const double* __restrict__ gpart, int ngp, int KK, double scale,
                                    double* scratch, double* G) {
   const int lanes = gram_lanes(KK);
   const int l = threadIdx.x / KK, q = threadIdx.x - l * KK;
-  double s = 0.0;
-  if (l < lanes) {
-    for (int b0 = l; b0 < ngp; b0 += 8 * lanes) {
-      double x[8];
-#pragma unroll
-      for (int u = 0; u < 8; ++u) x[u] = b0 + u * lanes < ngp ? gpart[(size_t)(b0 + u * lanes) * KK + q] : 0.0;
-#pragma unroll
-      for (int u = 0; u < 8; ++u) s += x[u];
-    }
-  }
+  const double s = l < lanes ? gram_lane_sum(gpart, ngp, KK, lanes, l, q) : 0.0;
   reduce_gram_tail(s, KK, scale, scratch, G);
 }
 
@@ -990,7 +992,7 @@
   return (size_t)ws_split_of(K, weighted) * (K + tri(K)) * WS_ROWS;
 }
 
-__host__ __device__ constexpr int ws_rows_for(int nl) { return nl > 2048 ? 64 : (nl > 1024 ? 32 : (nl > 512 ? 16 : 8)); }
+__host__ __device__ constexpr int ws_rows_for(int nl) { return nl > 2048 ? 64 : (nl > 1024 ? 32 : (nl > 512 ? 16 : 4)); }
 
 constexpr int WS_CHB = 32;
 template <bool SC1 = false>
@@ -1012,6 +1014,93 @@
     for (int u = 0; u < WS_CHB; ++u) if (c + u < nch) s += x[u];
   }
   return s;
+}
+
+template <int K, int RW>
+__device__ __forceinline__ void w_solve_rows(const WSolveArgs& a, int blk, double (&m)[K], double (&Q)[tri(K)], const double* zs, int zst,
+                                             int rr, int lane, bool live, int i, int d, double* stg) {
+  constexpr int KK = tri(K);
+#pragma unroll
+  for (int k = 0; k < K; ++k) Q[lidx(k, k)] += a.inv_sigma2;
+#pragma unroll
+  for (int r = 0; r < K; ++r) {
+    if (r >= d) {
+      m[r] = 0.0;
+#pragma unroll
+      for (int c = 0; c <= r; ++c) Q[lidx(r, c)] = (r == c) ? 1.0 : 0.0;
+    }
+  }
+  bool ok = true;
+  double invl[K];
+#pragma unroll
+  for (int c = 0; c < K; ++c) {
+    double p = Q[lidx(c, c)];
+#pragma unroll
+    for (int q = 0; q < c; ++q) p = fma(-Q[lidx(c, q)], Q[lidx(c, q)], p);
+    if (!(p > 0.0)) ok = false;
+    const double inv = rsq_nr(p);
+    const double l = __dmul_rn(p, inv);
+    invl[c] = inv;
+    Q[lidx(c, c)] = l;
+#pragma unroll
+    for (int r = c + 1; r < K; ++r) {
+      double v = Q[lidx(r, c)];
+#pragma unroll
+      for (int q = 0; q < c; ++q) v = fma(-Q[lidx(r, q)], Q[lidx(c, q)], v);
+      Q[lidx(r, c)] = __dmul_rn(v, inv);
+    }
+  }
+  if (live && !ok && atomicCAS(&a.status[0], 0, 1) == 0) a.status[1] = i;
+  WS_STAMP(4);
+  double y[K];
+#pragma unroll
+  for (int r = 0; r < K; ++r) {
+    double v = m[r];
+#pragma unroll
+    for (int c = 0; c < r; ++c) v = fma(-Q[lidx(r, c)], y[c], v);
+    y[r] = __dmul_rn(v, invl[r]);
+  }
+#pragma unroll
+  for (int r = 0; r < K; ++r)
+    if (r < d) y[r] = __dadd_rn(y[r], zs[r * zst + rr]);
+#pragma unroll
+  for (int r = K - 1; r >= 0; --r) {
+    double v = y[r];
+#pragma unroll
+    for (int c = r + 1; c < K; ++c) v = fma(-Q[lidx(c, r)], y[c], v);
+    y[r] = __dmul_rn(v, invl[r]);
+  }
+  double wrow[K];
+#pragma unroll
+  for (int r = 0; r < K; ++r) {
+    const bool fresh = live && ok && r < d;
+    if (fresh) a.W[(size_t)i * K + r] = y[r];
+    wrow[r] = fresh ? y[r] : 0.0;
+  }
+  if (live && (d < K || !ok)) {
+#pragma unroll
+    for (int r = 0; r < K; ++r)
+      if (!(ok && r < d)) wrow[r] = a.W[(size_t)i * K + r];
+  }
+  if (a.gout) {
+    typedef double v4f64_w __attribute__((ext_vector_type(4)));
+#pragma unroll
+    for (int r = 0; r < K; ++r) stg[r * WS_ROWS + lane] = wrow[r];
+    const int kk = lane >> 4, ii = lane & 15;
+    const double* src = stg + (ii < K ? ii : 0) * WS_ROWS + kk;
+    v4f64_w acc = {0.0, 0.0, 0.0, 0.0};
+#pragma unroll
+    for (int sidx = 0; sidx < (RW + 3) / 4; ++sidx) {
+      const double x = ii < K ? src[4 * sidx] : 0.0;
+      acc = __builtin_amdgcn_mfma_f64_16x16x4f64(x, x, acc, 0, 0, 0);
+    }
+#pragma unroll
+    for (int r = 0; r < 4; ++r) {
+      const int row = 4 * r + kk;
+      if (row < K && ii <= row) a.gout[(size_t)blk * KK + lidx(row, ii)] = acc[r];
+    }
+  }
+  WS_STAMP(5);
 }
 
 template <int K, bool WEIGHTED, int RW = WS_ROWS>
@@ -1217,88 +1306,7 @@
       for (int q = 0; q < KK; ++q) Q[q] = fma(-a.s, cvq[rr][q], Q[q]);
     }
   }
-#pragma unroll
-  for (int k = 0; k < K; ++k) Q[lidx(k, k)] += a.inv_sigma2;
-#pragma unroll
-  for (int r = 0; r < K; ++r) {
-    if (r >= d) {
-      m[r] = 0.0;
-#pragma unroll
-      for (int c = 0; c <= r; ++c) Q[lidx(r, c)] = (r == c) ? 1.0 : 0.0;
-    }
-  }
-  bool ok = true;
-  double invl[K];
-#pragma unroll
-  for (int c = 0; c < K; ++c) {
-    double p = Q[lidx(c, c)];
-#pragma unroll
-    for (int q = 0; q < c; ++q) p = fma(-Q[lidx(c, q)], Q[lidx(c, q)], p);
-    if (!(p > 0.0)) ok = false;
-    const double inv = rsq_nr(p);
-    const double l = __dmul_rn(p, inv);
-    invl[c] = inv;
-    Q[lidx(c, c)] = l;
-#pragma unroll
-    for (int r = c + 1; r < K; ++r) {
-      double v = Q[lidx(r, c)];
-#pragma unroll
-      for (int q = 0; q < c; ++q) v = fma(-Q[lidx(r, q)], Q[lidx(c, q)], v);
-      Q[lidx(r, c)] = __dmul_rn(v, inv);
-    }
-  }
-  if (live && !ok && atomicCAS(&a.status[0], 0, 1) == 0) a.status[1] = i;
-  WS_STAMP(4);
-  double y[K];
-#pragma unroll
-  for (int r = 0; r < K; ++r) {
-    double v = m[r];
-#pragma unroll
-    for (int c = 0; c < r; ++c) v = fma(-Q[lidx(r, c)], y[c], v);
-    y[r] = __dmul_rn(v, invl[r]);
-  }
-#pragma unroll
-  for (int r = 0; r < K; ++r)
-    if (r < d) y[r] = __dadd_rn(y[r], zsh[r][rr]);
-#pragma unroll
-  for (int r = K - 1; r >= 0; --r) {
-    double v = y[r];
-#pragma unroll
-    for (int c = r + 1; c < K; ++c) v = fma(-Q[lidx(c, r)], y[c], v);
-    y[r] = __dmul_rn(v, invl[r]);
-  }
-  double wrow[K];
-#pragma unroll
-  for (int r = 0; r < K; ++r) {
-    const bool fresh = live && ok && r < d;
-    if (fresh) a.W[(size_t)i * K + r] = y[r];
-    wrow[r] = fresh ? y[r] : 0.0;
-  }
-  if (live && (d < K || !ok)) {
-#pragma unroll
-    for (int r = 0; r < K; ++r)
-      if (!(ok && r < d)) wrow[r] = a.W[(size_t)i * K + r];
-  }
-  if (a.gout) {
-    typedef double v4f64_w __attribute__((ext_vector_type(4)));
-    double* stg = &red[0][0][0];
-#pragma unroll
-    for (int r = 0; r < K; ++r) stg[r * WS_ROWS + lane] = wrow[r];
-    const int kk = lane >> 4, ii = lane & 15;
-    const double* src = stg + (ii < K ? ii : 0) * WS_ROWS + kk;
-    v4f64_w acc = {0.0, 0.0, 0.0, 0.0};
-#pragma unroll
-    for (int sidx = 0; sidx < (RW + 3) / 4; ++sidx) {
-      const double x = ii < K ? src[4 * sidx] : 0.0;
-      acc = __builtin_amdgcn_mfma_f64_16x16x4f64(x, x, acc, 0, 0, 0);
-    }
-#pragma unroll
-    for (int r = 0; r < 4; ++r) {
-      const int row = 4 * r + kk;
-      if (row < K && ii <= row) a.gout[(size_t)blockIdx.x * KK + lidx(row, ii)] = acc[r];
-    }
-  }
-  WS_STAMP(5);
+  w_solve_rows<K, RW>(a, (int)blockIdx.x, m, Q, &zsh[0][0], WS_ROWS, rr, lane, live, i, d, &red[0][0][0]);
 }
 
 struct VBandArgs {
diff --git a/functionalmf_amd/csrc/btf_row_owner.h b/functionalmf_amd/csrc/btf_row_owner.h
--- /dev/null
+++ b/functionalmf_amd/csrc/btf_row_owner.h
@@ -0,0 +1,201 @@
+#pragma once
+#include "btf_kernels.h"
+#include "btf_row_owner_map.h"
+
+namespace btf {
+
+constexpr int RO_ROWS = 4;
+constexpr int RO_THREADS = (RO_STREAM_WAVES + 1) * WAVE;
+__host__ __device__ constexpr bool ro_rows_ok(int nl) { return ws_rows_for(nl) == RO_ROWS; }
+
+__device__ __forceinline__ void ro_lds_turn() {
+  __builtin_amdgcn_fence(__ATOMIC_ACQ_REL, "wavefront");
+  __builtin_amdgcn_wave_barrier();
+}
+
+typedef double ro_v2d __attribute__((ext_vector_type(2)));
+
+struct RowOwnerArgs {
+  WSolveArgs a;
+  const double* X;
+  const double* V;
+  int ld, MT;
+  int rpb, nch;
+};
+
+template <int K>
+__global__ __launch_bounds__(RO_THREADS) void w_row_owner_kernel(RowOwnerArgs ra) {
+  constexpr int KK = tri(K), RO = RO_ROWS, KR = K * RO;
+  constexpr int NW = RO_STREAM_WAVES, CPP = NW * RO_LANE_CHUNKS;
+  constexpr int NTG = WS_ROWS * ws_split_of(K, false);
+  constexpr int GL = (NTG / KK) > 32 ? 32 : ((NTG / KK) < 1 ? 1 : (NTG / KK));
+  static_assert(RO_CHAIN_WAVES == acc_waves(K, 0), "the chains are those of the 16-wave complete-data accumulation");
+  static_assert(NW * 128 * K <= CPP * RO_CHAIN_WAVES * KR, "the staging slices lie inside the chains' meeting area");
+  WSolveArgs& a = ra.a;
+  __shared__ double red[CPP * RO_CHAIN_WAVES * KR];
+  __shared__ double csum[CPP * KR];
+  __shared__ double msum[K][RO];
+  __shared__ double zsh[K][RO];
+  __shared__ double G[KK];
+  __shared__ double gscr[GL * KK];
+  __shared__ double stg[K * WS_ROWS];
+  const int lane = threadIdx.x & 63;
+  const int wave = __builtin_amdgcn_readfirstlane(threadIdx.x >> 6);
+  WS_STAMP(0);
+  if (a.hyp) {
+    if (a.hyp_noise) { a.s = 1.0 / a.hyp[HYP_NU2]; a.sR = a.s * a.Rrep; }
+    a.inv_sigma2 = 1.0 / a.hyp[HYP_SIGMA2];
+  }
+  const int il0 = blockIdx.x * RO;
+  const int rpb = ra.rpb, nch = ra.nch, MT = ra.MT;
+  const int nsteps = ro_steps(rpb), npass = ro_passes(nch);
+  double tot = 0.0;
+
+  if (wave == NW) {
+    for (int t = lane; t < GL * KK; t += WAVE) {
+      const int l = t / KK, q = t - l * KK;
+      gscr[t] = gram_lane_sum(a.gpart, a.ngp, KK, GL, l, q);
+    }
+    for (int t = lane; t < KR; t += WAVE) {
+      const int k = t / RO, r = t - k * RO;
+      double zv = 0.0;
+      if (il0 + r < a.nl) {
+        const int i = a.row0 + il0 + r;
+        const long long zoff = w_z_offset(i, K);
+        const int d = i + 1 < K ? i + 1 : K;
+        if (k < d) zv = a.z ? a.z[zoff + k] : philox_normal(a.seed, a.stream, (unsigned long long)(zoff + k));
+      }
+      zsh[k][r] = zv;
+    }
+    wave_lds_sync();
+    if (lane < KK) {
+      double t = 0.0;
+      for (int b = 0; b < GL; ++b) t += gscr[b * KK + lane];
+      G[lane] = t * a.sR;
+    }
+  }
+
+  for (int pass = 0; pass < npass; ++pass) {
+    double acc[RO][K][2];
+    const int c = ro_lane_chunk(pass, wave, lane);
+    const int w0 = ro_lane_chain(lane);
+    if (wave < NW) {
+#pragma unroll
+      for (int r = 0; r < RO; ++r)
+#pragma unroll
+        for (int k = 0; k < K; ++k) acc[r][k][0] = acc[r][k][1] = 0.0;
+      const double* xrow[RO];
+#pragma unroll
+      for (int r = 0; r < RO; ++r) xrow[r] = ra.X + (size_t)(a.row0 + min(il0 + r, a.nl - 1)) * ra.ld;
+      auto compute = [&](const ro_v2d (&x)[RO], const double (&v)[2 * K]) __attribute__((always_inline)) {
+#pragma unroll
+        for (int r = 0; r < RO; ++r)
+#pragma unroll
+          for (int k = 0; k < K; ++k) {
+            acc[r][k][0] = fma(x[r].x, v[k], acc[r][k][0]);
+            acc[r][k][1] = fma(x[r].y, v[K + k], acc[r][k][1]);
+          }
+      };
+      if (__builtin_amdgcn_readfirstlane(ro_wave_full(pass, wave, nch, rpb, MT) ? 1 : 0)) {
+        const unsigned xoff = (unsigned)ro_chain_col(c, w0, 0, rpb) * 8u;
+        unsigned voff[K];
+        const int cw0 = ro_lane_chunk(pass, wave, 0);
+#pragma unroll
+        for (int u = 0; u < K; ++u)
+          voff[u] = ((unsigned)ro_chain_col(cw0 + ro_stage_run(u, lane, K), 0, 0, rpb) * K + ro_stage_off(u, lane, K)) * 8u;
+        double* slice = red + wave * 128 * K;
+        struct Step { ro_v2d v[K]; ro_v2d x[RO]; };
+        auto issue = [&](int n, Step& s) __attribute__((always_inline)) {
+          const char* vb = reinterpret_cast<const char*>(ra.V) + (size_t)n * (RO_CHAIN_WAVES * K * 8);
+#pragma unroll
+          for (int u = 0; u < K; ++u) s.v[u] = *reinterpret_cast<const ro_v2d*>(vb + voff[u]);
+#pragma unroll
+          for (int r = 0; r < RO; ++r)
+            s.x[r] = *reinterpret_cast<const ro_v2d*>(reinterpret_cast<const char*>(xrow[r]) + (size_t)n * (RO_CHAIN_WAVES * 8) + xoff);
+        };
+        auto finish = [&](const Step& s) __attribute__((always_inline)) {
+#pragma unroll
+          for (int u = 0; u < K; ++u) *reinterpret_cast<ro_v2d*>(slice + 128 * u + 2 * lane) = s.v[u];
+          ro_lds_turn();
+          double v[2 * K];
+#pragma unroll
+          for (int u = 0; u < K; ++u) {
+            const ro_v2d t = *reinterpret_cast<const ro_v2d*>(slice + 2 * K * lane + 2 * u);
+            v[2 * u] = t.x; v[2 * u + 1] = t.y;
+          }
+          ro_lds_turn();
+          compute(s.x, v);
+        };
+        Step A, B;
+        issue(0, A);
+        for (int n = 0; n < nsteps; n += 2) {
+          issue(n + 1, B);
+          finish(A);
+          if (n + 2 < nsteps) issue(n + 2, A);
+          finish(B);
+        }
+      } else {
+        for (int n = 0; n < nsteps; ++n) {
+          ro_v2d x[RO];
+          double v[2 * K];
+#pragma unroll
+          for (int e = 0; e < 2; ++e) {
+            const long long col = ro_chain_col(c, w0 + e, n, rpb);
+            const bool has = c < nch && col < (long long)MT;
+#pragma unroll
+            for (int k = 0; k < K; ++k) v[e * K + k] = has ? ra.V[(size_t)col * K + k] : 0.0;
+#pragma unroll
+            for (int r = 0; r < RO; ++r) x[r][e] = has ? xrow[r][col] : 0.0;
+          }
+          compute(x, v);
+        }
+      }
+    }
+    if (pass == npass - 1) WS_STAMP(1);
+    __syncthreads();
+    if (wave < NW && c < nch) {
+      double* dst = red + ((size_t)(c - pass * CPP) * RO_CHAIN_WAVES + w0) * KR;
+#pragma unroll
+      for (int e = 0; e < 2; ++e)
+#pragma unroll
+        for (int k = 0; k < K; ++k)
+#pragma unroll
+          for (int r = 0; r < RO; ++r) dst[e * KR + k * RO + r] = acc[r][k][e];
+    }
+    __syncthreads();
+    for (int e = threadIdx.x; e < CPP * KR; e += RO_THREADS) {
+      const int cl = e / KR, vr = e - cl * KR;
+      if (pass * CPP + cl < nch) {
+        double s = 0.0;
+#pragma unroll
+        for (int w = 0; w < RO_CHAIN_WAVES; ++w) s += red[((size_t)cl * RO_CHAIN_WAVES + w) * KR + vr];
+        csum[e] = s;
+      }
+    }
+    __syncthreads();
+    if ((int)threadIdx.x < KR) {
+      const int ncl = min(CPP, nch - pass * CPP);
+      for (int cl = 0; cl < ncl; ++cl) tot += csum[cl * KR + threadIdx.x];
+    }
+  }
+  if ((int)threadIdx.x < KR) msum[threadIdx.x / RO][threadIdx.x % RO] = tot;
+  __syncthreads();
+  WS_STAMP(2);
+  if (wave != 0) return;
+  const int rr = lane % RO, il = il0 + rr;
+  const bool live = lane < RO && il < a.nl;
+  const int i = a.row0 + (live ? il : 0);
+  const int d = i + 1 < K ? i + 1 : K;
+  double m[K], Q[KK];
+#pragma unroll
+  for (int k = 0; k < K; ++k) {
+    double s = 0.0;
+    s += msum[k][rr];
+    m[k] = __dmul_rn(s, a.s);
+  }
+#pragma unroll
+  for (int q = 0; q < KK; ++q) Q[q] = G[q];
+  w_solve_rows<K, RO>(a, (int)blockIdx.x, m, Q, &zsh[0][0], RO, rr, lane, live, i, d, stg);
+}
+
+}
diff --git a/functionalmf_amd/csrc/btf_row_owner_map.h b/functionalmf_amd/csrc/btf_row_owner_map.h
--- /dev/null
+++ b/functionalmf_amd/csrc/btf_row_owner_map.h
@@ -0,0 +1,32 @@
+#pragma once
+
+#if defined(__HIPCC__) || defined(__CUDACC__)
+#define BTF_RO_HD __host__ __device__
+#else
+#define BTF_RO_HD
+#endif
+
+namespace btf {
+
+constexpr int RO_CHAIN_WAVES = 16;
+constexpr int RO_LANE_CHUNKS = 8;
+constexpr int RO_STREAM_WAVES = 4;
+
+BTF_RO_HD constexpr int ro_lane_chunk(int pass, int wave, int lane) {
+  return (pass * RO_STREAM_WAVES + wave) * RO_LANE_CHUNKS + lane / (RO_CHAIN_WAVES / 2);
+}
+BTF_RO_HD constexpr int ro_lane_chain(int lane) { return 2 * (lane % (RO_CHAIN_WAVES / 2)); }
+BTF_RO_HD constexpr long long ro_chain_col(int chunk, int wave, int step, int rpb) {
+  return (long long)chunk * rpb + (long long)RO_CHAIN_WAVES * step + wave;
+}
+BTF_RO_HD constexpr int ro_steps(int rpb) { return rpb / RO_CHAIN_WAVES; }
+BTF_RO_HD constexpr int ro_passes(int nch) {
+  return (nch + RO_STREAM_WAVES * RO_LANE_CHUNKS - 1) / (RO_STREAM_WAVES * RO_LANE_CHUNKS);
+}
+BTF_RO_HD constexpr bool ro_wave_full(int pass, int wave, int nch, int rpb, long long MT) {
+  return ro_lane_chunk(pass, wave, 63) < nch && (long long)(ro_lane_chunk(pass, wave, 63) + 1) * rpb <= MT;
+}
+BTF_RO_HD constexpr int ro_stage_run(int u, int lane, int K) { return (128 * u + 2 * lane) / (RO_CHAIN_WAVES * K); }
+BTF_RO_HD constexpr int ro_stage_off(int u, int lane, int K) { return (128 * u + 2 * lane) % (RO_CHAIN_WAVES * K); }
+
+}
```
